# kursawe/OpticalFlow

Measured on AMD Instinct MI355X. Metric: frame-pairs/sec, higher is better.
Workload: dtype f64; 1 GPU; 1024x1024x256 synthetic translating texture (seed 1), speed_alpha=1, remodelling_alpha=1e4, rtol=1e-06, all 255 pairs solved to the stopping rule; frames_per_gpu=256, pairs_in_flight=255, levels=9, coarse_stencils=float8, vcycle_vectors=coarse_float32, w_cycle_level=1, w_cycle_visits=3, warm_start_stride=3, allgather=False, gather_chunks=1, converged=True

## Files before the change

include/vof.h:

```cpp
#ifndef VOF_H
#define VOF_H

#include <stddef.h>
#include <stdint.h>

#ifdef __cplusplus
extern "C" {
#endif

#define VOF_VERSION 202

typedef struct vof_ctx vof_ctx;

typedef struct vof_params {
    uint32_t struct_size;
    uint32_t abi_version;
    double speed_alpha;
    double remodelling_alpha;
    double delta_x;
    double delta_t;
    double initial_v_x;
    double initial_v_y;
    double initial_remodelling;
    double rtol;
    int32_t max_iterations;
    int32_t nu_pre;
    int32_t nu_post;
    int32_t reference_quirks;
    int32_t coarse_precision;
    int32_t vcycle_precision;
    int32_t nu_pre_coarse;
    int32_t nu_post_coarse;
    int32_t w_cycle_level;
    int32_t w_cycle_visits;
    int32_t krylov_method;
    int32_t gmres_restart;
    int32_t fallback_after;
    int32_t warm_start_stride;
    int32_t preconditioner;
    int32_t reserved0;
} vof_params;

typedef struct vof_pair_stats {
    int32_t iterations;
    int32_t converged;
    double relative_residual;
    double L1_functional;
    double speed_functional;
    double remodelling_functional;
    double batch_ms;
    int32_t batch_pairs;
    int32_t reserved;
} vof_pair_stats;

enum vof_kernel_id {
    VOF_K_RHS = 0, VOF_K_APPLY0, VOF_K_GS0, VOF_K_GS, VOF_K_RESIDUAL, VOF_K_RESTRICT, VOF_K_PROLONG,
    VOF_K_GALERKIN0, VOF_K_GALERKIN, VOF_K_COARSE_SETUP, VOF_K_COARSE_SOLVE, VOF_K_VECTOR, VOF_K_REDUCE,
    VOF_K_FINALIZE, VOF_K_FUNCTIONALS, VOF_K_COARSE_TAIL, VOF_K_COUNT
};

int vof_version(void);
size_t vof_params_size(void);
int vof_default_params(vof_params* p, size_t struct_size);


int vof_create(vof_ctx** out, int device_id, int n_i, int n_j, int max_pairs_in_flight, void* stream);
void vof_destroy(vof_ctx* ctx);
const char* vof_last_error(const vof_ctx* ctx);
size_t vof_workspace_bytes(const vof_ctx* ctx);
size_t vof_query_workspace(int n_i, int n_j, int max_pairs_in_flight);
size_t vof_query_workspace_for(int n_i, int n_j, int max_pairs_in_flight, int coarse_precision, int vcycle_precision);
int vof_device_memory(int device_id, size_t* free_bytes, size_t* total_bytes);
int vof_num_levels(const vof_ctx* ctx);

int vof_solve_stack_host(vof_ctx* ctx, const double* movie, int n_frames, const vof_params* p,
                         double* v_x, double* v_y, double* remodelling, double* speed,
                         vof_pair_stats* stats);
int vof_solve_stack_dev(vof_ctx* ctx, const double* movie, int n_frames, const vof_params* p,
                        double* v_x, double* v_y, double* remodelling, double* speed,
                        vof_pair_stats* stats);

int vof_blur_stack_dev(vof_ctx* ctx, const double* in_dev, double* out_dev, int n_frames, const double* weights, int radius);
int vof_blur_stack_host(vof_ctx* ctx, const double* in_host, double* out_host, int n_frames, const double* weights, int radius);

typedef struct vof_variation_stats {
    double speed_mean, speed_variance;
    double remodelling_mean, remodelling_variance;
    double L1_functional, speed_functional, remodelling_functional;
    double max_relative_residual;
    int32_t converged_last;
    int32_t converged_all;
    int32_t max_iterations_used;
    int32_t reserved;
} vof_variation_stats;

int vof_vary_regularisation_host(vof_ctx* ctx, const double* movie, int n_frames, const vof_params* base,
                                 const double* speed_alphas, int n_speed_alphas,
                                 const double* remodelling_alphas, int n_remodelling_alphas,
                                 const double* blur_weights, int blur_radius, vof_variation_stats* out);

int vof_field_moments_dev(vof_ctx* ctx, const double* field_dev, size_t n, double* mean, double* variance);

int vof_subsample_dev(vof_ctx* ctx, const double* field_dev, int n_fields, int box, int offset, double* out_dev);

int vof_texture_stack_dev(vof_ctx* ctx, double* out_dev, int n_frames, const double* mode_params, int n_modes,
                          const double* frame_offsets, double period, double scale);

int vof_set_fused_sweeps(vof_ctx* ctx, int on);

int vof_bench_sweeps_dev(vof_ctx* ctx, const double* movie, int n_pairs, const vof_params* p, int n_sweeps);

int vof_profile_enable(vof_ctx* ctx, int on);
int vof_profile_reset(vof_ctx* ctx);
int vof_profile_filter(vof_ctx* ctx, int kernel_id, int level);
int vof_profile_get(vof_ctx* ctx, int kernel_id, int level, int64_t* launches, double* total_ms);
int vof_profile_get_units(vof_ctx* ctx, int kernel_id, int level, int64_t* pair_launches);
int vof_profile_get_bytes(vof_ctx* ctx, int kernel_id, int level, double* algorithmic_bytes);
int vof_profile_get_moved(vof_ctx* ctx, int kernel_id, int level, double* moved_bytes);
const char* vof_kernel_name(int kernel_id);

int vof_debug_setup(vof_ctx* ctx, const double* movie_host, int n_pairs, const vof_params* p);
int vof_debug_check_canaries(vof_ctx* ctx);
int vof_debug_level_shape(vof_ctx* ctx, int level, int* n_i, int* n_j);
int vof_debug_rhs(vof_ctx* ctx, double* b_host);
int vof_debug_apply(vof_ctx* ctx, int level, const double* x_host, double* y_host);
int vof_debug_gs(vof_ctx* ctx, int level, double* x_host, const double* b_host, int colour);
int vof_debug_sweep(vof_ctx* ctx, int level, double* x_host, const double* b_host, int reverse, int from_zero);
int vof_debug_smooth(vof_ctx* ctx, int level, double* x_host, const double* b_host, int nu, int reverse, int from_zero);
int vof_debug_restrict(vof_ctx* ctx, int level, const double* fine_host, double* coarse_host);
int vof_debug_prolong_add(vof_ctx* ctx, int level, double* fine_host, const double* coarse_host);
int vof_debug_resrestrict_u(vof_ctx* ctx, int level, const double* x_new_host, const double* x_old_host, double* coarse_host);
int vof_debug_stencil(vof_ctx* ctx, int level, double* c_host);
int vof_debug_vcycle(vof_ctx* ctx, const double* r_host, double* e_host);
int vof_debug_coarse_solve(vof_ctx* ctx, const double* r_host, double* e_host);
int vof_debug_vcycle_apply(vof_ctx* ctx, const double* r_host, double* y_host, double* v_host, double* dots_host, int* fused);

#ifdef __cplusplus
}
#endif
#endif
```

opticalflow_amd/_native.py:

```python
from __future__ import annotations

import ctypes as C
import os

import numpy as np

HERE = os.path.dirname(os.path.abspath(__file__))
LIB_PATH = os.environ.get("VOF_LIB") or os.path.join(HERE, "csrc", "libvof.so")

K_NAMES = ["rhs", "apply0", "gs0", "gs", "residual", "restrict", "prolong", "galerkin0", "galerkin",
           "coarse_setup", "coarse_solve", "vector", "reduce", "finalize", "functionals", "coarse_tail"]


class VofParams(C.Structure):
    _fields_ = [("struct_size", C.c_uint32), ("abi_version", C.c_uint32),
                ("speed_alpha", C.c_double), ("remodelling_alpha", C.c_double), ("delta_x", C.c_double),
                ("delta_t", C.c_double), ("initial_v_x", C.c_double), ("initial_v_y", C.c_double),
                ("initial_remodelling", C.c_double), ("rtol", C.c_double), ("max_iterations", C.c_int32),
                ("nu_pre", C.c_int32), ("nu_post", C.c_int32), ("reference_quirks", C.c_int32),
                ("coarse_precision", C.c_int32), ("vcycle_precision", C.c_int32), ("nu_pre_coarse", C.c_int32), ("nu_post_coarse", C.c_int32),
                ("w_cycle_level", C.c_int32), ("w_cycle_visits", C.c_int32), ("krylov_method", C.c_int32),
                ("gmres_restart", C.c_int32), ("fallback_after", C.c_int32), ("warm_start_stride", C.c_int32),
                ("preconditioner", C.c_int32), ("reserved0", C.c_int32)]


class VofPairStats(C.Structure):
    _fields_ = [("iterations", C.c_int32), ("converged", C.c_int32), ("relative_residual", C.c_double),
                ("L1_functional", C.c_double), ("speed_functional", C.c_double),
                ("remodelling_functional", C.c_double), ("batch_ms", C.c_double), ("batch_pairs", C.c_int32),
                ("reserved", C.c_int32)]


STATS_DTYPE = np.dtype([("iterations", np.int32), ("converged", np.int32), ("relative_residual", np.float64),
                        ("L1_functional", np.float64), ("speed_functional", np.float64),
                        ("remodelling_functional", np.float64), ("batch_ms", np.float64), ("batch_pairs", np.int32),
                        ("reserved", np.int32)])
assert STATS_DTYPE.itemsize == C.sizeof(VofPairStats)

VARIATION_DTYPE = np.dtype([("speed_mean", np.float64), ("speed_variance", np.float64), ("remodelling_mean", np.float64),
                            ("remodelling_variance", np.float64), ("L1_functional", np.float64),
                            ("speed_functional", np.float64), ("remodelling_functional", np.float64),
                            ("max_relative_residual", np.float64), ("converged_last", np.int32),
                            ("converged_all", np.int32), ("max_iterations_used", np.int32), ("reserved", np.int32)])
assert VARIATION_DTYPE.itemsize == 80

_dp = C.POINTER(C.c_double)
_vp = C.c_void_p

SIGNATURES = {
    "vof_version": (C.c_int, []),
    "vof_params_size": (C.c_size_t, []),
    "vof_default_params": (C.c_int, [C.POINTER(VofParams), C.c_size_t]),
    "vof_create": (C.c_int, [C.POINTER(_vp), C.c_int, C.c_int, C.c_int, C.c_int, _vp]),
    "vof_destroy": (None, [_vp]),
    "vof_last_error": (C.c_char_p, [_vp]),
    "vof_workspace_bytes": (C.c_size_t, [_vp]),
    "vof_query_workspace": (C.c_size_t, [C.c_int, C.c_int, C.c_int]),
    "vof_query_workspace_for": (C.c_size_t, [C.c_int, C.c_int, C.c_int, C.c_int, C.c_int]),
    "vof_device_memory": (C.c_int, [C.c_int, C.POINTER(C.c_size_t), C.POINTER(C.c_size_t)]),
    "vof_num_levels": (C.c_int, [_vp]),
    "vof_solve_stack_host": (C.c_int, [_vp, _vp, C.c_int, C.POINTER(VofParams), _vp, _vp, _vp, _vp, _vp]),
    "vof_solve_stack_dev": (C.c_int, [_vp, _vp, C.c_int, C.POINTER(VofParams), _vp, _vp, _vp, _vp, _vp]),
    "vof_texture_stack_dev": (C.c_int, [_vp, _vp, C.c_int, _vp, C.c_int, _vp, C.c_double, C.c_double]),
    "vof_bench_sweeps_dev": (C.c_int, [_vp, _vp, C.c_int, C.POINTER(VofParams), C.c_int]),
    "vof_blur_stack_dev": (C.c_int, [_vp, _vp, _vp, C.c_int, _vp, C.c_int]),
    "vof_blur_stack_host": (C.c_int, [_vp, _vp, _vp, C.c_int, _vp, C.c_int]),
    "vof_vary_regularisation_host": (C.c_int, [_vp, _vp, C.c_int, C.POINTER(VofParams), _vp, C.c_int, _vp, C.c_int, _vp, C.c_int, _vp]),
    "vof_field_moments_dev": (C.c_int, [_vp, _vp, C.c_size_t, C.POINTER(C.c_double), C.POINTER(C.c_double)]),
    "vof_subsample_dev": (C.c_int, [_vp, _vp, C.c_int, C.c_int, C.c_int, _vp]),
    "vof_profile_enable": (C.c_int, [_vp, C.c_int]),
    "vof_profile_reset": (C.c_int, [_vp]),
    "vof_profile_filter": (C.c_int, [_vp, C.c_int, C.c_int]),
    "vof_profile_get": (C.c_int, [_vp, C.c_int, C.c_int, C.POINTER(C.c_int64), C.POINTER(C.c_double)]),
    "vof_profile_get_units": (C.c_int, [_vp, C.c_int, C.c_int, C.POINTER(C.c_int64)]),
    "vof_profile_get_bytes": (C.c_int, [_vp, C.c_int, C.c_int, C.POINTER(C.c_double)]),
    "vof_profile_get_moved": (C.c_int, [_vp, C.c_int, C.c_int, C.POINTER(C.c_double)]),
    "vof_kernel_name": (C.c_char_p, [C.c_int]),
    "vof_debug_setup": (C.c_int, [_vp, _vp, C.c_int, C.POINTER(VofParams)]),
    "vof_debug_check_canaries": (C.c_int, [_vp]),
    "vof_debug_level_shape": (C.c_int, [_vp, C.c_int, C.POINTER(C.c_int), C.POINTER(C.c_int)]),
    "vof_debug_rhs": (C.c_int, [_vp, _vp]),
    "vof_debug_apply": (C.c_int, [_vp, C.c_int, _vp, _vp]),
    "vof_debug_gs": (C.c_int, [_vp, C.c_int, _vp, _vp, C.c_int]),
    "vof_debug_sweep": (C.c_int, [_vp, C.c_int, _vp, _vp, C.c_int, C.c_int]),
    "vof_debug_smooth": (C.c_int, [_vp, C.c_int, _vp, _vp, C.c_int, C.c_int, C.c_int]),
    "vof_set_fused_sweeps": (C.c_int, [_vp, C.c_int]),
    "vof_debug_restrict": (C.c_int, [_vp, C.c_int, _vp, _vp]),
    "vof_debug_resrestrict_u": (C.c_int, [_vp, C.c_int, _vp, _vp, _vp]),
    "vof_debug_prolong_add": (C.c_int, [_vp, C.c_int, _vp, _vp]),
    "vof_debug_stencil": (C.c_int, [_vp, C.c_int, _vp]),
    "vof_debug_vcycle": (C.c_int, [_vp, _vp, _vp]),
    "vof_debug_coarse_solve": (C.c_int, [_vp, _vp, _vp]),
    "vof_debug_vcycle_apply": (C.c_int, [_vp, _vp, _vp, _vp, _vp, C.POINTER(C.c_int)]),
}

_lib = None


class VofError(RuntimeError):
    pass


def _share_hip_runtime_with_torch():
    import importlib.util
    import sys
    if "torch" in sys.modules:
        return
    try:
        spec = importlib.util.find_spec("torch")
    except (ImportError, ValueError):
        spec = None
    if spec is None or not spec.origin:
        return
    hip = os.path.join(os.path.dirname(spec.origin), "lib", "libamdhip64.so")
    if os.path.exists(hip):
        C.CDLL(hip, mode=C.RTLD_GLOBAL)


def load_library(path: str | None = None):
    global _lib
    if _lib is not None and path is None:
        return _lib
    p = path or LIB_PATH
    if not os.path.exists(p):
        raise VofError(f"native library {p} not found: build it with `python -m opticalflow_amd.build` "
                       "(hipcc, gfx950). There is no CPU fallback.")
    _share_hip_runtime_with_torch()
    lib = C.CDLL(p)
    for name, (res, args) in SIGNATURES.items():
        fn = getattr(lib, name)
        fn.restype = res
        fn.argtypes = args
    if path is None:
        _lib = lib
    return lib


def default_params(**overrides) -> VofParams:
    lib = load_library()
    p = VofParams()
    if lib.vof_default_params(C.byref(p), C.sizeof(p)) != 0:
        raise VofError(f"vof_params layout mismatch: binding {C.sizeof(p)} bytes, library {lib.vof_params_size()} bytes")
    for k, v in overrides.items():
        if not hasattr(p, k):
            raise TypeError(f"unknown solver parameter {k!r}")
        setattr(p, k, v)
    return p


def _ptr(a):
    if a is None:
        return None
    if isinstance(a, int):
        return C.c_void_p(a)
    if isinstance(a, np.ndarray):
        assert a.flags["C_CONTIGUOUS"]
        return C.c_void_p(a.ctypes.data)
    if hasattr(a, "data_ptr"):
        return C.c_void_p(a.data_ptr())
    raise TypeError(type(a))


class Solver:

    def __init__(self, n_i: int, n_j: int, max_pairs_in_flight: int, device: int = 0, stream: int | None = None):
        self.lib = load_library()
        self.n_i, self.n_j, self.max_pairs = int(n_i), int(n_j), int(max_pairs_in_flight)
        self.device = int(device)
        h = C.c_void_p()
        rc = self.lib.vof_create(C.byref(h), self.device, self.n_i, self.n_j, self.max_pairs,
                                 C.c_void_p(stream) if stream else None)
        if rc != 0:
            raise VofError("vof_create failed: " + self.lib.vof_last_error(None).decode())
        self.h = h

    def check_canaries(self):
        self._check(self.lib.vof_debug_check_canaries(self.h), "vof_debug_check_canaries")

    def close(self):
        if getattr(self, "h", None):
            h, self.h = self.h, None
            rc = self.lib.vof_debug_check_canaries(h)
            msg = self.lib.vof_last_error(h).decode() if rc != 0 else ""
            self.lib.vof_destroy(h)
            if rc != 0:
                raise VofError("device buffer guard regions damaged: " + msg)

    def __del__(self):
        try:
            self.close()
        except Exception:
            pass

    def __enter__(self):
        return self

    def __exit__(self, *a):
        self.close()

    def _check(self, rc, what):
        if rc != 0:
            raise VofError(f"{what} failed ({rc}): " + self.lib.vof_last_error(self.h).decode())

    @property
    def workspace_bytes(self):
        return int(self.lib.vof_workspace_bytes(self.h))

    @property
    def num_levels(self):
        return int(self.lib.vof_num_levels(self.h))

    def level_shape(self, level):
        a, b = C.c_int(), C.c_int()
        self._check(self.lib.vof_debug_level_shape(self.h, level, C.byref(a), C.byref(b)), "level_shape")
        return a.value, b.value

    def solve_host(self, movie: np.ndarray, params: VofParams, want_speed=True):
        movie = np.ascontiguousarray(movie, dtype=np.float64)
        T = movie.shape[0]
        assert movie.shape[1:] == (self.n_i, self.n_j)
        out = [np.empty((T - 1, self.n_i, self.n_j)) for _ in range(4 if want_speed else 3)]
        stats = np.zeros(T - 1, dtype=STATS_DTYPE)
        rc = self.lib.vof_solve_stack_host(self.h, _ptr(movie), T, C.byref(params), _ptr(out[0]), _ptr(out[1]),
                                           _ptr(out[2]), _ptr(out[3]) if want_speed else None, _ptr(stats))
        self._check(rc, "vof_solve_stack_host")
        return (*out, stats) if want_speed else (*out, None, stats)

    def solve_dev(self, movie, n_frames, params: VofParams, v_x, v_y, remodelling, speed=None, stats=True):
        st = np.zeros(n_frames - 1, dtype=STATS_DTYPE) if stats else None
        rc = self.lib.vof_solve_stack_dev(self.h, _ptr(movie), int(n_frames), C.byref(params), _ptr(v_x), _ptr(v_y),
                                          _ptr(remodelling), _ptr(speed), _ptr(st))
        self._check(rc, "vof_solve_stack_dev")
        return st

    def blur_host(self, movie: np.ndarray, weights: np.ndarray):
        movie = np.ascontiguousarray(movie, dtype=np.float64)
        weights = np.ascontiguousarray(weights, dtype=np.float64)
        assert movie.shape[1:] == (self.n_i, self.n_j) and weights.size % 2 == 1
        out = np.empty_like(movie)
        self._check(self.lib.vof_blur_stack_host(self.h, _ptr(movie), _ptr(out), movie.shape[0], _ptr(weights),
                                                 weights.size // 2), "vof_blur_stack_host")
        return out

    def blur_dev(self, movie, out, n_frames, weights: np.ndarray):
        weights = np.ascontiguousarray(weights, dtype=np.float64)
        self._check(self.lib.vof_blur_stack_dev(self.h, _ptr(movie), _ptr(out), int(n_frames), _ptr(weights),
                                                weights.size // 2), "vof_blur_stack_dev")

    def vary_regularisation_host(self, movie: np.ndarray, params: VofParams, speed_alphas, remodelling_alphas, weights=None):
        movie = np.ascontiguousarray(movie, dtype=np.float64)
        assert movie.shape[1:] == (self.n_i, self.n_j)
        sa = np.ascontiguousarray(speed_alphas, dtype=np.float64).ravel()
        ra = np.ascontiguousarray(remodelling_alphas, dtype=np.float64).ravel()
        out = np.zeros((sa.size, ra.size), dtype=VARIATION_DTYPE)
        w = None if weights is None else np.ascontiguousarray(weights, dtype=np.float64)
        rc = self.lib.vof_vary_regularisation_host(self.h, _ptr(movie), movie.shape[0], C.byref(params), _ptr(sa), sa.size,
                                                   _ptr(ra), ra.size, _ptr(w), 0 if w is None else w.size // 2, _ptr(out))
        self._check(rc, "vof_vary_regularisation_host")
        return out

    def field_moments_dev(self, field, n):
        m, v = C.c_double(), C.c_double()
        self._check(self.lib.vof_field_moments_dev(self.h, _ptr(field), int(n), C.byref(m), C.byref(v)), "vof_field_moments_dev")
        return m.value, v.value

    def subsample_dev(self, field, n_fields, box, offset, out):
        self._check(self.lib.vof_subsample_dev(self.h, _ptr(field), int(n_fields), int(box), int(offset), _ptr(out)),
                    "vof_subsample_dev")

    def texture_stack_dev(self, out, n_frames, mode_params, frame_offsets, period, scale):
        mp = np.ascontiguousarray(mode_params, dtype=np.float64)
        fo = np.ascontiguousarray(frame_offsets, dtype=np.float64)
        assert mp.ndim == 2 and mp.shape[0] == 4 and fo.shape == (n_frames, 2)
        self._check(self.lib.vof_texture_stack_dev(self.h, _ptr(out), int(n_frames), _ptr(mp), mp.shape[1], _ptr(fo),
                                                   float(period), float(scale)), "vof_texture_stack_dev")

    def bench_sweeps(self, movie, n_pairs, params, n_sweeps):
        self._check(self.lib.vof_bench_sweeps_dev(self.h, _ptr(movie), n_pairs, C.byref(params), n_sweeps),
                    "vof_bench_sweeps_dev")

    def profile_enable(self, on=True):
        self._check(self.lib.vof_profile_enable(self.h, int(bool(on))), "profile_enable")

    def profile_filter(self, kernel=-1, level=-1):
        kid = K_NAMES.index(kernel) if isinstance(kernel, str) else int(kernel)
        self._check(self.lib.vof_profile_filter(self.h, kid, level), "profile_filter")

    def profile_reset(self):
        self._check(self.lib.vof_profile_reset(self.h), "profile_reset")

    def profile_get(self, kernel: int | str, level: int = -1):
        kid = K_NAMES.index(kernel) if isinstance(kernel, str) else int(kernel)
        n, ms = C.c_int64(), C.c_double()
        self._check(self.lib.vof_profile_get(self.h, kid, level, C.byref(n), C.byref(ms)), "profile_get")
        return n.value, ms.value

    def profile_units(self, kernel: int | str, level: int = -1):
        kid = K_NAMES.index(kernel) if isinstance(kernel, str) else int(kernel)
        u = C.c_int64()
        self._check(self.lib.vof_profile_get_units(self.h, kid, level, C.byref(u)), "profile_get_units")
        return u.value

    def profile_bytes(self, kernel: int | str, level: int = -1):
        kid = K_NAMES.index(kernel) if isinstance(kernel, str) else int(kernel)
        u = C.c_double()
        self._check(self.lib.vof_profile_get_bytes(self.h, kid, level, C.byref(u)), "profile_get_bytes")
        return u.value

    def profile_moved(self, kernel: int | str, level: int = -1):
        kid = K_NAMES.index(kernel) if isinstance(kernel, str) else int(kernel)
        u = C.c_double()
        self._check(self.lib.vof_profile_get_moved(self.h, kid, level, C.byref(u)), "profile_get_moved")
        return u.value

    def profile_table(self):
        rows = []
        for kid, name in enumerate(K_NAMES):
            for lvl in range(16):
                n, ms = self.profile_get(kid, lvl)
                if n:
                    rows.append((name, lvl, n, ms))
        return rows

    def debug_setup(self, movie: np.ndarray, params: VofParams):
        movie = np.ascontiguousarray(movie, dtype=np.float64)
        self._dbg_pairs = movie.shape[0] - 1
        self._check(self.lib.vof_debug_setup(self.h, _ptr(movie), self._dbg_pairs, C.byref(params)), "debug_setup")

    def _vec(self, level):
        ni, nj = self.level_shape(level)
        return (self._dbg_pairs, 3, ni, nj)

    def debug_rhs(self):
        b = np.empty(self._vec(0))
        self._check(self.lib.vof_debug_rhs(self.h, _ptr(b)), "debug_rhs")
        return b

    def debug_apply(self, level, x):
        x = np.ascontiguousarray(x, dtype=np.float64).reshape(self._vec(level))
        y = np.empty_like(x)
        self._check(self.lib.vof_debug_apply(self.h, level, _ptr(x), _ptr(y)), "debug_apply")
        return y

    def debug_gs(self, level, x, b, colour):
        x = np.array(x, dtype=np.float64, copy=True).reshape(self._vec(level))
        b = np.ascontiguousarray(b, dtype=np.float64).reshape(self._vec(level))
        self._check(self.lib.vof_debug_gs(self.h, level, _ptr(x), _ptr(b), colour), "debug_gs")
        return x

    def debug_sweep(self, level, x, b, reverse=False, from_zero=False):
        x = np.array(x, dtype=np.float64, copy=True).reshape(self._vec(level))
        b = np.ascontiguousarray(b, dtype=np.float64).reshape(self._vec(level))
        self._check(self.lib.vof_debug_sweep(self.h, level, _ptr(x), _ptr(b), int(reverse), int(from_zero)), "debug_sweep")
        return x

    def debug_smooth(self, level, x, b, nu, reverse=False, from_zero=False):
        x = np.array(x, dtype=np.float64, copy=True).reshape(self._vec(level))
        b = np.ascontiguousarray(b, dtype=np.float64).reshape(self._vec(level))
        self._check(self.lib.vof_debug_smooth(self.h, level, _ptr(x), _ptr(b), int(nu), int(reverse), int(from_zero)), "debug_smooth")
        return x

    def set_fused_sweeps(self, on=True):
        self._check(self.lib.vof_set_fused_sweeps(self.h, int(bool(on))), "set_fused_sweeps")

    def debug_restrict(self, level, fine):
        fine = np.ascontiguousarray(fine, dtype=np.float64).reshape(self._vec(level))
        coarse = np.empty(self._vec(level + 1))
        self._check(self.lib.vof_debug_restrict(self.h, level, _ptr(fine), _ptr(coarse)), "debug_restrict")
        return coarse

    def debug_resrestrict_u(self, level, x_new, x_old=None):
        x_new = np.ascontiguousarray(x_new, dtype=np.float64).reshape(self._vec(level))
        if x_old is not None:
            x_old = np.ascontiguousarray(x_old, dtype=np.float64).reshape(self._vec(level))
        coarse = np.empty(self._vec(level + 1))
        self._check(self.lib.vof_debug_resrestrict_u(self.h, level, _ptr(x_new), _ptr(x_old) if x_old is not None else None,
                                                     _ptr(coarse)), "debug_resrestrict_u")
        return coarse

    def debug_prolong_add(self, level, fine, coarse):
        fine = np.array(fine, dtype=np.float64, copy=True).reshape(self._vec(level))
        coarse = np.ascontiguousarray(coarse, dtype=np.float64).reshape(self._vec(level + 1))
        self._check(self.lib.vof_debug_prolong_add(self.h, level, _ptr(fine), _ptr(coarse)), "debug_prolong_add")
        return fine

    def debug_stencil(self, level):
        ni, nj = self.level_shape(level)
        c = np.empty((self._dbg_pairs, 3, 3, 3, 3, ni, nj))
        self._check(self.lib.vof_debug_stencil(self.h, level, _ptr(c)), "debug_stencil")
        return c

    def debug_vcycle(self, r):
        r = np.ascontiguousarray(r, dtype=np.float64).reshape(self._vec(0))
        e = np.empty_like(r)
        self._check(self.lib.vof_debug_vcycle(self.h, _ptr(r), _ptr(e)), "debug_vcycle")
        return e

    def debug_vcycle_apply(self, r):
        r = np.ascontiguousarray(r, dtype=np.float64).reshape(self._vec(0))
        y, v = np.empty_like(r), np.empty_like(r)
        dots = np.zeros((r.shape[0], 2))
        fused = C.c_int(0)
        self._check(self.lib.vof_debug_vcycle_apply(self.h, _ptr(r), _ptr(y), _ptr(v), _ptr(dots), C.byref(fused)), "debug_vcycle_apply")
        return y, v, dots, bool(fused.value)

    def debug_coarse_solve(self, r):
        last = self.num_levels - 1
        r = np.ascontiguousarray(r, dtype=np.float64).reshape(self._vec(last))
        e = np.empty_like(r)
        self._check(self.lib.vof_debug_coarse_solve(self.h, _ptr(r), _ptr(e)), "debug_coarse_solve")
        return e


def query_workspace(n_i, n_j, pairs, coarse_precision=None, vcycle_precision=None):
    if coarse_precision is None and vcycle_precision is None:
        return int(load_library().vof_query_workspace(int(n_i), int(n_j), int(pairs)))
    return int(load_library().vof_query_workspace_for(int(n_i), int(n_j), int(pairs), 3 if coarse_precision is None else int(coarse_precision),
                                                      3 if vcycle_precision is None else int(vcycle_precision)))


def device_memory(device=0):
    f, t = C.c_size_t(), C.c_size_t()
    rc = load_library().vof_device_memory(int(device), C.byref(f), C.byref(t))
    if rc != 0:
        raise VofError("no usable HIP device %d (vof_device_memory rc=%d); this package has no CPU fallback" % (device, rc))
    return f.value, t.value
```

opticalflow_amd/csrc/vof.hip:

```cpp
#include "vof_device.hpp"
#include "vof_sweep0r.hpp"
#include "vof_sweep0p.hpp"
#include "vof_direct.hpp"
#include "../../include/vof.h"

#include <dlfcn.h>
#include <fcntl.h>
#include <unistd.h>

#include <algorithm>
#include <atomic>
#include <chrono>
#include <cmath>
#include <condition_variable>
#include <cstdio>
#include <cstdlib>
#include <cstring>
#include <mutex>
#include <string>
#include <thread>
#include <vector>

using namespace vof;

namespace {

constexpr int COARSEST_MAX = 5;
int coarsest_max() {
    if (const char* e = getenv("VOF_COARSEST_MAX")) { int v = atoi(e); if (v >= 3 && v <= 9) return v; }
    return COARSEST_MAX;
}
constexpr int MAX_PROF_RECS = 32768;
constexpr int MAX_LANES = 3;
constexpr int MAX_LANE_GROUPS = 2;
constexpr int AUTO_F64_AFTER = 8;

struct Level {
    int ni = 0, nj = 0;
    size_t npts = 0;
    void* C = nullptr;
    void* x = nullptr;
    void* b = nullptr;
    void* r = nullptr;
    void* x2 = nullptr;
};

struct ProfRec {
    hipEvent_t e0, e1;
    int kid, level, units;
    double bytes;
    double moved;
};

}

struct vof_ctx {
    int device = 0;
    hipStream_t stream = nullptr;
    bool own_stream = false;
    int Ni = 0, Nj = 0, B = 0;
    std::vector<Level> L;
    double *kx = nullptr, *kb = nullptr, *kr = nullptr, *krh = nullptr, *kp = nullptr, *kv = nullptr, *kt = nullptr;
    double* ky = nullptr;
    double* kz = nullptr;
    double* b32 = nullptr;
    bool vfloat = false;
    bool emit64 = false;
    bool vcoarse32 = false;
    bool l0_handoff = true;
    bool h32 = false;
    bool h32_bad = false;
    const PairParam* pp = nullptr;
    PairParam* pp_buf = nullptr;
    double* warm_x = nullptr;
    size_t warm_cap = 0;
    int* warm_src = nullptr;
    const int* guess_src = nullptr;
    double* partials = nullptr;
    int nblk = 0;
    PairScalars* sc = nullptr;
    int* active = nullptr;
    double* func3 = nullptr;
    double *W = nullptr, *invT = nullptr;
    int nd = 0;
    int* h_active = nullptr;
    PairScalars* h_sc = nullptr;
    double* h_func3 = nullptr;
    char* h_bounce = nullptr;
    hipEvent_t ev_batch[2] = {nullptr, nullptr};
    double* st_movie = nullptr;
    double* st_out[4] = {nullptr, nullptr, nullptr, nullptr};
    double* st_out2[4] = {nullptr, nullptr, nullptr, nullptr};
    hipStream_t copy_stream = nullptr;
    hipEvent_t ev_solved[2] = {nullptr, nullptr}, ev_copied[2] = {nullptr, nullptr}, ev_uploaded[2] = {nullptr, nullptr};
    double* st_movie2 = nullptr;
    double *blur_tmp = nullptr, *blur_w = nullptr, *blur_io = nullptr;
    double* tex_tab = nullptr;
    size_t tex_cap = 0;
    double* gm_V = nullptr;
    GmresState* gm_state = nullptr;
    double* gm_partials = nullptr;
    int* gm_cycle = nullptr;
    int gm_m = 0;
    long long gmres_pairs = 0;
    struct Alloc { void* raw; char* user; size_t bytes; const char* name; int line; };
    std::vector<Alloc> allocs;
    int c_bytes_per_point = 0;
    size_t bytes = 0;
    std::string err;
    const double* frames = nullptr;
    int npairs = 0;
    vof_params prm;
    int cfmt = 0;
    bool fused = true;
    bool geo_b_fine = false, geo_b_stored = true;
    bool fuse_prolong = true;
    bool fuse_restrict = true;
    bool sweep_st = true;
    bool skip_colour0 = true;
    bool fold_stored = false;
    bool fuse_resu = true;
    bool stream_apply = true;
    bool sweep0 = true;
    bool direct_on = false;
    int dir_cap = 0;
    double *dir_T = nullptr, *dir_tabs = nullptr, *dir_W = nullptr, *dir_r = nullptr, *dir_y = nullptr, *dir_x = nullptr, *dir_t = nullptr;
    int *dir_ipiv = nullptr, *dir_info = nullptr;
    double *dir_R = nullptr, *dir_C = nullptr, *dir_D = nullptr;
    int dir_ld = 0;
    void* roc_handle = nullptr;
    long long direct_pairs = 0;
    bool trail_enabled = true;
    bool trail_set = false, trail_done = false;
    S0Trail trail_req;
    bool fuse_rr = true;
    void* rr_out = nullptr;
    bool rr_f32 = false, rr_done = false;
    bool fuse_b = true;
    int bf_mode = 0;
    S0BSrc bf{nullptr, nullptr, nullptr, nullptr, nullptr, nullptr};
    int trail_nblk = 0;
    bool sweep0m = true;
    bool sweep0m_pairs = true;
    bool sweep0r = true;
    long sweep0r_min_blocks = 512;
    bool sweep0p = true;
    bool tail_enabled = true;
    int tail_first = -1;
    size_t tail_lds = 0;
    TailArgs tail;
    int tail_key[6] = {-9, -9, -9, -9, -9, -9};
    bool prof = false;
    int prof_kid = -1, prof_level = -1;
    std::vector<ProfRec> recs;
    std::vector<hipEvent_t> free_events;
    long long prof_dropped = 0;
    double prof_ms[VOF_K_COUNT][16];
    long long prof_n[VOF_K_COUNT][16];
    long long prof_units[VOF_K_COUNT][16];
    double prof_bytes[VOF_K_COUNT][16];
    double prof_moved[VOF_K_COUNT][16];
    int cur_units = 0;
    bool pq_hier = true, pq_smooth = true;
    int dbg_sync = 0;
    long long dbg_seq = 0;
    std::string dbg_fault;
    int dbg_fd = -1;
    bool dbg_canary = false;
    bool dbg_alloc_log = false;
    bool dbg_poison = false;
    size_t part_per_pair = 0;
    vof_ctx* lane_parent = nullptr;
    int lane_lo = 0, lane_slots = 0;
    int dir_ok = -1;
    hipStream_t lane_stream[MAX_LANES] = {};
    hipEvent_t lane_ev[MAX_LANES][2] = {};
    hipEvent_t ev_fork = nullptr;
    hipEvent_t group_ev[MAX_LANES * MAX_LANE_GROUPS] = {};
};

static std::string g_create_error;

namespace {

void dbg_sync_check(vof_ctx* c, const char* what, int level) {
    if (!c->dbg_sync) return;
    ++c->dbg_seq;
    char line[256];
    if (c->dbg_fd >= 0) {
        int n = snprintf(line, sizeof line, "in flight: scope #%lld '%s' level %d, %d pairs, grid %dx%d (%d levels)%-40s\n", c->dbg_seq, what, level,
                         c->cur_units, c->Ni, c->Nj, (int)c->L.size(), "");
        if (pwrite(c->dbg_fd, line, (size_t)n, 0) < 0) {  }
    }
    hipError_t e = hipStreamSynchronize(c->stream);
    hipError_t e2 = hipGetLastError();
    if (e == hipSuccess) e = e2;
    if (e != hipSuccess && c->dbg_fault.empty()) {
        snprintf(line, sizeof line, "VOF_DEBUG_SYNC: scope #%lld, kernel class '%s', level %d, %d pairs, image %dx%d: %s", c->dbg_seq, what, level,
                 c->cur_units, c->Ni, c->Nj, hipGetErrorString(e));
        c->dbg_fault = line;
        fprintf(stderr, "%s\n", line);
        fflush(stderr);
    }
}

struct Prof {
    vof_ctx* c;
    bool on;
    int dkid, dlevel;
    ProfRec rec;
    Prof(vof_ctx* c_, int kid, int level, double bytes_per_pair = 0.0, double moved_per_pair = -1.0) : c(c_), on(false), dkid(kid), dlevel(level) {
        if (!c->prof) return;
        if (c->prof_kid >= 0 && kid != c->prof_kid) return;
        if (c->prof_level >= 0 && level != c->prof_level) return;
        if ((int)c->recs.size() >= MAX_PROF_RECS) { c->prof_dropped++; return; }
        if (c->free_events.size() >= 2) {
            rec.e0 = c->free_events.back(); c->free_events.pop_back();
            rec.e1 = c->free_events.back(); c->free_events.pop_back();
        } else {
            if (hipEventCreate(&rec.e0) != hipSuccess || hipEventCreate(&rec.e1) != hipSuccess) return;
        }
        rec.kid = kid; rec.level = level < 0 ? 0 : (level > 15 ? 15 : level);
        rec.units = c->cur_units;
        rec.bytes = bytes_per_pair * c->cur_units;
        rec.moved = (moved_per_pair < 0.0 ? bytes_per_pair : moved_per_pair) * c->cur_units;
        on = true;
        hipEventRecord(rec.e0, c->stream);
    }
    ~Prof() {
        if (on) {
            hipEventRecord(rec.e1, c->stream);
            c->recs.push_back(rec);
        }
        if (c->dbg_sync) dbg_sync_check(c, vof_kernel_name(dkid), dlevel);
    }
};

void prof_collect(vof_ctx* c) {
    if (c->recs.empty()) return;
    hipStreamSynchronize(c->stream);
    for (auto& r : c->recs) {
        float ms = 0.f;
        if (hipEventElapsedTime(&ms, r.e0, r.e1) == hipSuccess) {
            c->prof_ms[r.kid][r.level] += ms;
            c->prof_n[r.kid][r.level] += 1;
            c->prof_units[r.kid][r.level] += r.units;
            c->prof_bytes[r.kid][r.level] += r.bytes;
            c->prof_moved[r.kid][r.level] += r.moved;
        }
        c->free_events.push_back(r.e0);
        c->free_events.push_back(r.e1);
    }
    c->recs.clear();
}

#define HIPCHK(call)                                                                               \
    do {                                                                                           \
        hipError_t e_ = (call);                                                                    \
        if (e_ != hipSuccess) {                                                                    \
            char buf_[512];                                                                        \
            snprintf(buf_, sizeof buf_, "%s failed: %s (%s:%d)", #call, hipGetErrorString(e_), __FILE__, __LINE__); \
            c->err = buf_;                                                                         \
            if (!c->dbg_fault.empty()) c->err += " [" + c->dbg_fault + "]";                        \
            return -2;                                                                             \
        }                                                                                          \
    } while (0)

constexpr size_t DBG_GUARD = 4096;
constexpr int DBG_GUARD_BYTE = 0xC5;

template <typename T>
int dev_alloc_named(vof_ctx* c, T** p, size_t n, const char* name, int line) {
    void* q = nullptr;
    size_t bytes = std::max<size_t>(n * sizeof(T), 256);
    if (c->dbg_canary) {
        HIPCHK(hipMalloc(&q, bytes + 2 * DBG_GUARD));
        HIPCHK(hipMemset(q, DBG_GUARD_BYTE, DBG_GUARD));
        HIPCHK(hipMemset((char*)q + DBG_GUARD + bytes, DBG_GUARD_BYTE, DBG_GUARD));
        c->allocs.push_back({q, (char*)q + DBG_GUARD, bytes, name, line});
        *p = (T*)((char*)q + DBG_GUARD);
    } else {
        HIPCHK(hipMalloc(&q, bytes));
        c->allocs.push_back({q, (char*)q, bytes, name, line});
        *p = (T*)q;
    }
    c->bytes += bytes;
    if (c->dbg_poison) HIPCHK(hipMemset(*p, 0xFF, bytes));
    if (c->dbg_alloc_log)
        fprintf(stderr, "vof alloc ctx=%p %s (vof.hip:%d) base=%p end=%p bytes=%zu\n", (void*)c, name, line, (void*)*p, (void*)((char*)*p + bytes), bytes);
    return 0;
}
#define dev_alloc(c, p, n) dev_alloc_named(c, p, n, #p, __LINE__)

int dev_free(vof_ctx* c, void* user) {
    if (!user) return 0;
    for (size_t i = 0; i < c->allocs.size(); ++i)
        if ((void*)c->allocs[i].user == user) {
            HIPCHK(hipFree(c->allocs[i].raw));
            c->bytes -= c->allocs[i].bytes;
            c->allocs.erase(c->allocs.begin() + (long)i);
            return 0;
        }
    c->err = "internal: dev_free of a pointer the context does not own";
    return -1;
}

constexpr int DEFAULT_COARSE_PRECISION = 3;
inline int vof_params_default_coarse_precision() { return DEFAULT_COARSE_PRECISION; }
inline int coef_bytes_per_point(int fmt) { return fmt == 3 ? 30 * 4 : (fmt == 2 ? 45 * 4 : (fmt == 1 ? 81 * 4 : 81 * 8)); }

int ensure_stencil_storage(vof_ctx* c, int fmt) {
    const int need = coef_bytes_per_point(fmt);
    if (need <= c->c_bytes_per_point || c->L.size() < 2) return 0;
    HIPCHK(hipStreamSynchronize(c->stream));
    for (size_t l = 1; l < c->L.size(); ++l) {
        Level& lv = c->L[l];
        if (int rc = dev_free(c, lv.C)) return rc;
        lv.C = nullptr;
    }
    for (size_t l = 1; l < c->L.size(); ++l) {
        Level& lv = c->L[l];
        uint32_t* C = nullptr;
        if (int rc = dev_alloc(c, &C, (size_t)c->B * (need / 4) * CLay(lv.ni, lv.nj).plane)) return rc;
        lv.C = C;
    }
    c->c_bytes_per_point = need;
    c->frames = nullptr;
    return 0;
}

int ensure_storage(vof_ctx* c) {
    if (int rc = ensure_stencil_storage(c, c->prm.coarse_precision)) return rc;
    if (c->vfloat && !c->b32)
        if (int rc = dev_alloc(c, &c->b32, (size_t)c->B * 3 * c->L[0].npts)) return rc;
    return 0;
}

int dbg_check_canaries(vof_ctx* c, std::string* report) {
    int bad = 0;
    std::vector<unsigned char> h(2 * DBG_GUARD);
    if (!c->dbg_canary) return 0;
    for (const auto& a : c->allocs) {
        if (hipMemcpy(h.data(), a.raw, DBG_GUARD, hipMemcpyDeviceToHost) != hipSuccess ||
            hipMemcpy(h.data() + DBG_GUARD, a.user + a.bytes, DBG_GUARD, hipMemcpyDeviceToHost) != hipSuccess) {
            if (report) *report += "guard pages unreadable; ";
            return -1;
        }
        long first_lo = -1, first_hi = -1;
        for (size_t i = 0; i < DBG_GUARD; ++i) if (h[DBG_GUARD - 1 - i] != DBG_GUARD_BYTE) { first_lo = (long)i + 1; break; }
        for (size_t i = 0; i < DBG_GUARD; ++i) if (h[DBG_GUARD + i] != DBG_GUARD_BYTE) { first_hi = (long)i; break; }
        if (first_lo >= 0 || first_hi >= 0) {
            ++bad;
            char line[256];
            snprintf(line, sizeof line, "buffer %s (vof.hip:%d, %zu bytes at %p): written %s%ld bytes %s; ", a.name, a.line, a.bytes, (void*)a.user,
                     first_hi >= 0 ? "" : "-", first_hi >= 0 ? first_hi : first_lo, first_hi >= 0 ? "past its end" : "before its start");
            if (report) *report += line;
        }
    }
    return bad;
}

inline dim3 grid2d(int ni, int nj, int z) { return dim3((nj + BX - 1) / BX, (ni + BY - 1) / BY, z); }
inline dim3 grid2d_colour(int ni, int nj, int colour, int z) {
    int cp = colour >> 1, cq = colour & 1;
    int mi = (ni - cp + 1) / 2, mj = (nj - cq + 1) / 2;
    return dim3(std::max(1, (mj + BX - 1) / BX), std::max(1, (mi + BY - 1) / BY), z);
}
const dim3 blk2d(BX, BY, 1);

inline size_t frame_stride(const vof_ctx* c) { return (size_t)c->Ni * c->Nj; }

#define VDISPATCH(c, ...)                                   \
    do {                                                    \
        if ((c)->vfloat) { using VT = float; __VA_ARGS__; } \
        else { using VT = double; __VA_ARGS__; }            \
    } while (0)

#define YDISPATCH(c, ...)                                                  \
    do {                                                                   \
        if ((c)->vfloat || (c)->h32) { using VT = float; __VA_ARGS__; }    \
        else { using VT = double; __VA_ARGS__; }                           \
    } while (0)

template <typename T> struct TypeTag { typedef T type; };
#define CDISPATCH(c, l, ...)                                                                        \
    do {                                                                                            \
        const int cf_ = ((l) > 0) ? (c)->cfmt : 0;                                                  \
        if (cf_ == 2) { using CT = CoefB16; using CW = uint32_t; __VA_ARGS__; }                     \
        else if (cf_ == 3) { using CT = CoefF8; using CW = uint32_t; __VA_ARGS__; }                 \
        else if (cf_ == 1) { using CT = float; using CW = float; __VA_ARGS__; }                     \
        else { using CT = double; using CW = double; __VA_ARGS__; }                                 \
    } while (0)
inline double coef_bytes(const vof_ctx* c, int l) { const int f = l > 0 ? c->cfmt : 0; return f == 3 ? 30.0 * 4 : (f == 2 ? 45.0 * 4 : (f == 1 ? 81.0 * 4 : 81.0 * 8)); }

void gs_colour(vof_ctx* c, int l, double* x, const double* b, int colour, int np, const int* active) {
    Level& lv = c->L[l];
    dim3 g = grid2d_colour(lv.ni, lv.nj, colour, np);
    if (l == 0 && c->L.size() > 1) {
        Prof p(c, VOF_K_GS0, 0, 20.0 * lv.npts);
        k_gs0<<<g, blk2d, 0, c->stream>>>(c->frames, frame_stride(c), c->Nj, lv.ni, lv.nj, c->prm.speed_alpha,
                                          c->prm.remodelling_alpha, c->prm.reference_quirks, x, b, colour, active, c->pp);
    } else {
        Prof p(c, VOF_K_GS, l, (coef_bytes(c, l) + 72.0) / 4.0 * lv.npts);
        CDISPATCH(c, l, (k_gs<CT><<<g, blk2d, 0, c->stream>>>((const CW*)lv.C, lv.ni, lv.nj, x, b, colour, active)));
    }
}

int pick_band_height(int rows, int nx, int units) {
    const long blocks128 = (long)nx * ((rows + 127) / 128) * std::max(1, units);
    const int cap = blocks128 < 768 ? 32 : (blocks128 < 1536 ? 64 : 128);
    const int nb = (rows + cap - 1) / cap;
    return std::max(2, (((rows + nb - 1) / nb + 1) / 2) * 2);
}

struct ApplyGrid { int TI, nblk; dim3 grid; };
ApplyGrid apply_grid(const vof_ctx* c, int np) {
    const Level& lv = c->L[0];
    int TI = pick_band_height(lv.ni, (lv.nj + AP_OUT - 1) / AP_OUT, c->cur_units);
    ApplyGrid g;
    g.TI = TI;
    g.grid = dim3((lv.nj + AP_OUT - 1) / AP_OUT, (lv.ni + TI - 1) / TI, np);
    g.nblk = g.grid.x * g.grid.y;
    return g;
}

template <typename XT, typename BT, typename YT>
void apply_fine_t(vof_ctx* c, const XT* x, const BT* b, YT* y, int mode, int np, const int* active,
                  const double* dotvec = nullptr, int want_yy = 0, YT* ycopy = nullptr) {
    Level& lv = c->L[0];
    const double bytes = (8.0 + 3.0 * sizeof(XT) + ((y ? 3.0 : 0.0) + (ycopy ? 3.0 : 0.0)) * sizeof(YT) + (mode ? 3.0 * sizeof(BT) : 0.0) +
                          (dotvec ? 24.0 : 0.0)) * lv.npts;
    Prof p(c, VOF_K_APPLY0, 0, bytes);
    if (c->stream_apply) {
        ApplyGrid ag = apply_grid(c, np);
        double* part = (dotvec || want_yy) ? c->partials : nullptr;
        if (mode)
            k_stream_apply0<1, XT, BT, YT><<<ag.grid, AP_THREADS, 0, c->stream>>>(
                c->frames, frame_stride(c), c->Nj, lv.ni, lv.nj, ag.TI, c->prm.speed_alpha, c->prm.remodelling_alpha,
                c->prm.reference_quirks, x, b, y, dotvec, want_yy, part, ag.nblk, active, c->pp, ycopy);
        else
            k_stream_apply0<0, XT, BT, YT><<<ag.grid, AP_THREADS, 0, c->stream>>>(
                c->frames, frame_stride(c), c->Nj, lv.ni, lv.nj, ag.TI, c->prm.speed_alpha, c->prm.remodelling_alpha,
                c->prm.reference_quirks, x, b, y, dotvec, want_yy, part, ag.nblk, active, c->pp, ycopy);
        return;
    }
    if (ycopy) { c->err = "internal: second output without the streaming operator kernel"; return; }
    dim3 g = grid2d(lv.ni, lv.nj, np);
    if (mode)
        k_apply0<1, XT, BT, YT><<<g, blk2d, 0, c->stream>>>(c->frames, frame_stride(c), c->Nj, lv.ni, lv.nj,
                                                            c->prm.speed_alpha, c->prm.remodelling_alpha,
                                                            c->prm.reference_quirks, x, b, y, active, c->pp);
    else
        k_apply0<0, XT, BT, YT><<<g, blk2d, 0, c->stream>>>(c->frames, frame_stride(c), c->Nj, lv.ni, lv.nj,
                                                            c->prm.speed_alpha, c->prm.remodelling_alpha,
                                                            c->prm.reference_quirks, x, b, y, active, c->pp);
}

template <typename VT>
void apply_stored_t(vof_ctx* c, int l, const VT* x, const VT* b, VT* y, int mode, int np, const int* active) {
    Level& lv = c->L[l];
    dim3 g = grid2d(lv.ni, lv.nj, np);
    Prof p(c, VOF_K_RESIDUAL, l, (coef_bytes(c, l) + (mode ? 9.0 : 6.0) * sizeof(VT)) * lv.npts);
    if (mode) CDISPATCH(c, l, (k_apply<CT, 1, VT><<<g, blk2d, 0, c->stream>>>((const CW*)lv.C, lv.ni, lv.nj, x, b, y, active)));
    else CDISPATCH(c, l, (k_apply<CT, 0, VT><<<g, blk2d, 0, c->stream>>>((const CW*)lv.C, lv.ni, lv.nj, x, b, y, active)));
}

template <typename VT>
void apply_level_t(vof_ctx* c, int l, const VT* x, const VT* b, VT* y, int mode, int np, const int* active) {
    if (l == 0 && c->L[0].C == nullptr) apply_fine_t<VT, VT, VT>(c, x, b, y, mode, np, active);
    else apply_stored_t<VT>(c, l, x, b, y, mode, np, active);
}

int krylov_apply(vof_ctx* c, const void* y, double* out, int np, const int* active, const double* dotvec = nullptr,
                 int want_yy = 0) {
    if (c->L[0].C) { apply_stored_t<double>(c, 0, (const double*)y, nullptr, out, 0, np, active); return 0; }
    const bool fuse = c->stream_apply && (dotvec || want_yy);
    if (c->vfloat || c->h32) apply_fine_t<float, double, double>(c, (const float*)y, nullptr, out, 0, np, active, fuse ? dotvec : nullptr, fuse ? want_yy : 0);
    else apply_fine_t<double, double, double>(c, (const double*)y, nullptr, out, 0, np, active, fuse ? dotvec : nullptr, fuse ? want_yy : 0);
    return fuse ? apply_grid(c, np).nblk : 0;
}
inline bool residual_copy_ok(const vof_ctx* c) { return c->stream_apply && !c->L[0].C; }
// ... 575 lines not shown
    if (c->gm_V) return 0;
    const size_t vec = (size_t)c->B * 3 * c->L[0].npts * sizeof(double);
    size_t free_b = 0, total_b = 0;
    HIPCHK(hipMemGetInfo(&free_b, &total_b));
    const size_t fixed = (size_t)c->B * (sizeof(GmresState) + (GM_NV + 1) * c->nblk * sizeof(double) + sizeof(int));
    const double budget = 0.5 * (double)free_b - (double)fixed;
    int fit = budget > 0 ? (int)std::min<double>(budget / (double)vec, 1e6) - 1 : 0;
    int m = std::min(want_m, fit);
    if (m < 4) { c->err = "not enough device memory for the GMRES fallback (lower max_pairs_in_flight)"; return -3; }
    if (int rc = dev_alloc(c, &c->gm_V, (size_t)(m + 1) * c->B * 3 * c->L[0].npts)) return rc;
    if (int rc = dev_alloc(c, &c->gm_state, (size_t)c->B)) return rc;
    if (int rc = dev_alloc(c, &c->gm_partials, (size_t)c->B * (GM_NV + 1) * c->nblk)) return rc;
    c->gm_m = m;
    return 0;
}

std::mutex g_lane_alloc;
int lane_gmres_attach(vof_ctx* c, bool basis, int want_m) {
    vof_ctx* p = c->lane_parent;
    std::lock_guard<std::mutex> lock(g_lane_alloc);
    int rc = 0;
    if (!p->gm_cycle) rc = dev_alloc(p, &p->gm_cycle, (size_t)p->B);
    if (!rc && basis && !p->gm_V) rc = gmres_buffers(p, want_m);
    if (rc) { c->err = p->err; p->err.clear(); return rc; }
    const size_t lo = (size_t)c->lane_lo;
    c->gm_cycle = p->gm_cycle + lo;
    if (p->gm_V) {
        c->gm_V = p->gm_V + lo * 3 * c->L[0].npts;
        c->gm_state = p->gm_state + lo;
        c->gm_partials = p->gm_partials + lo * (GM_NV + 1) * c->nblk;
        c->gm_m = p->gm_m;
    }
    return 0;
}

int gmres_phase(vof_ctx* c, int np, int* handed_over) {
    const vof_params& P = c->prm;
    hipStream_t s = c->stream;
    const size_t len = 3 * c->L[0].npts;
    const size_t vstride = (size_t)c->B * len;
    if (!c->gm_cycle) {
        if (c->lane_parent) { if (int rc = lane_gmres_attach(c, false, 0)) return rc; }
        else if (int rc = dev_alloc(c, &c->gm_cycle, (size_t)c->B)) return rc;
    }
    k_gm_begin<<<(np + 63) / 64, 64, 0, s>>>(c->sc, c->active, c->gm_cycle, np, P.max_iterations);
    dbg_sync_check(c, "gm_begin", 0);
    int nact = count_active(c, np);
    if (nact < 0) { c->err = "stream synchronize failed"; return -2; }
    if (nact == 0) return 0;
    *handed_over = nact;
    if (!c->gm_V) {
        const int want = P.gmres_restart > 0 ? P.gmres_restart : 100;
        int rc = c->lane_parent ? lane_gmres_attach(c, true, want) : gmres_buffers(c, want);
        if (rc == -3) { c->err.clear(); return 0; }
        if (rc) return rc;
    }
    c->gmres_pairs += nact;
    const int m = std::min(c->gm_m, P.gmres_restart > 0 ? P.gmres_restart : 100);
    c->vfloat = false;
    c->vcoarse32 = false;
    double* V = c->gm_V;
    double* w = c->kt;
    const dim3 rg = rgrid(c, np);
    const int coef_c = (int)(offsetof(GmresState, c) / sizeof(double)), coef_y = (int)(offsetof(GmresState, y) / sizeof(double));
    for (;;) {
        c->cur_units = nact;
        int nb = residual_d(c, c->kx, c->kb, V, np, c->gm_cycle, 1);
        if (!nb) { Prof p(c, VOF_K_REDUCE, 0); k_dot2<<<rg, RBLK, 0, s>>>(V, V, nullptr, nullptr, len, c->partials, c->gm_cycle); nb = c->nblk; }
        { Prof p(c, VOF_K_VECTOR, 0);
          k_gm_init<<<np, 64, 0, s>>>(c->gm_state, c->sc, c->partials, nb, c->active, c->gm_cycle, P.max_iterations); }
        nact = count_active(c, np);
        if (nact < 0) { c->err = "stream synchronize failed"; return -2; }
        if (nact == 0) break;
        c->cur_units = nact;
        { Prof p(c, VOF_K_VECTOR, 0, 16.0 * len); k_gm_scale<<<rg, RBLK, 0, s>>>(V, V, len, c->gm_state, c->active); }
        int jdone = 0;
        for (int j = 0; j < m; ++j) {
            const int* act = c->active;
            vcycle(c, &c->ky, V + (size_t)j * vstride, np, act);
            krylov_apply(c, c->ky, w, np, act);
            for (int pass = 0; pass < 2; ++pass) {
                for (int i0 = 0; i0 <= j; i0 += GM_NV) {
                    int cnt = std::min(GM_NV, j + 1 - i0);
                    Prof p(c, VOF_K_REDUCE, 0, 8.0 * len * (cnt + 1));
                    k_gm_multidot<<<rg, RBLK, 0, s>>>(V + (size_t)i0 * vstride, vstride, cnt, w, len, c->gm_partials, act);
                    k_gm_hcoef<<<np, 64, 0, s>>>(c->gm_state, c->gm_partials, c->nblk, i0, cnt, pass, act);
                }
                for (int i0 = 0; i0 <= j; i0 += GM_NV) {
                    int cnt = std::min(GM_NV, j + 1 - i0);
                    bool last = pass == 1 && i0 + GM_NV > j;
                    Prof p(c, VOF_K_VECTOR, 0, 8.0 * len * (cnt + 2));
                    k_gm_axpy<<<rg, RBLK, 0, s>>>(V + (size_t)i0 * vstride, vstride, i0, cnt, c->gm_state, coef_c, -1.0, w,
                                                  last ? V + (size_t)(j + 1) * vstride : w, len, act, 0,
                                                  last ? c->gm_partials : nullptr);
                }
            }
            { Prof p(c, VOF_K_VECTOR, 0, 16.0 * len);
              k_gm_givens<<<np, 64, 0, s>>>(c->gm_state, c->sc, c->gm_partials, c->nblk, j, c->active, P.max_iterations);
              k_gm_scale<<<rg, RBLK, 0, s>>>(V + (size_t)(j + 1) * vstride, V + (size_t)(j + 1) * vstride, len, c->gm_state, c->active); }
            jdone = j + 1;
            nact = count_active(c, np);
            if (nact < 0) { c->err = "stream synchronize failed"; return -2; }
            if (nact == 0) break;
            c->cur_units = nact;
        }
        { Prof p(c, VOF_K_VECTOR, 0); k_gm_solve_y<<<(np + 63) / 64, 64, 0, s>>>(c->gm_state, c->gm_cycle, np); }
        for (int i0 = 0; i0 < jdone; i0 += GM_NV) {
            int cnt = std::min(GM_NV, jdone - i0);
            Prof p(c, VOF_K_VECTOR, 0, 8.0 * len * (cnt + 2));
            k_gm_axpy<<<rg, RBLK, 0, s>>>(V + (size_t)i0 * vstride, vstride, i0, cnt, c->gm_state, coef_y, 1.0,
                                          i0 ? c->kp : nullptr, c->kp, len, c->gm_cycle, 1, nullptr);
        }
        vcycle(c, &c->ky, c->kp, np, c->gm_cycle);
        { Prof p(c, VOF_K_VECTOR, 0, 24.0 * len); k_gm_xpy<<<rg, RBLK, 0, s>>>(c->kx, c->ky, len, c->gm_cycle); }
        HIPCHK(hipGetLastError());
    }
    HIPCHK(hipGetLastError());
    return 0;
}

struct RocSolverApi {
    void* lib = nullptr;
    int (*create_handle)(void**) = nullptr;
    int (*destroy_handle)(void*) = nullptr;
    int (*set_stream)(void*, hipStream_t) = nullptr;
    int (*getrf)(void*, int, int, double*, int, long long, int*, long long, int*, int) = nullptr;
    int (*getri)(void*, int, double*, int, long long, int*, long long, int*, int) = nullptr;
    std::string err;
    bool resident() {
        if (lib) return true;
        const char* names[] = {"librocsolver.so.0", "librocsolver.so"};
        for (const char* n : names)
            if (void* h = dlopen(n, RTLD_NOLOAD | RTLD_LAZY)) { dlclose(h); return true; }
        return false;
    }
    bool load() {
        if (lib) return true;
        const char* names[] = {getenv("VOF_ROCSOLVER_LIB"), "librocsolver.so.0", "librocsolver.so", "/opt/rocm/lib/librocsolver.so.0"};
        for (const char* n : names) {
            if (!n || !*n) continue;
            lib = dlopen(n, RTLD_NOW | RTLD_GLOBAL);
            if (lib) break;
        }
        if (!lib) {
            const char* e = dlerror();
            err = std::string("cannot load rocSOLVER: ") + (e ? e : "not found");
            return false;
        }
        create_handle = (int (*)(void**))dlsym(lib, "rocblas_create_handle");
        destroy_handle = (int (*)(void*))dlsym(lib, "rocblas_destroy_handle");
        set_stream = (int (*)(void*, hipStream_t))dlsym(lib, "rocblas_set_stream");
        getrf = (int (*)(void*, int, int, double*, int, long long, int*, long long, int*, int))dlsym(lib, "rocsolver_dgetrf_strided_batched");
        getri = (int (*)(void*, int, double*, int, long long, int*, long long, int*, int))dlsym(lib, "rocsolver_dgetri_strided_batched");
        if (!create_handle || !destroy_handle || !set_stream || !getrf || !getri) {
            err = "rocSOLVER / rocBLAS symbols missing";
            dlclose(lib);
            lib = nullptr;
            return false;
        }
        return true;
    }
};
RocSolverApi g_roc;

constexpr int DIRECT_OWN_MAX = 192;
bool direct_uses_rocsolver(const vof_ctx*) {
    const char* e = getenv("VOF_DIRECT_LU");
    return e && e[0] == 'r';
}
bool direct_uses_blocked(const vof_ctx* c) {
    if (const char* e = getenv("VOF_DIRECT_LU")) return e[0] == 'b';
    return 3 * c->L[0].nj > DIRECT_OWN_MAX;
}
int direct_ld(const vof_ctx* c) {
    const int m = 3 * c->L[0].nj;
    return direct_uses_blocked(c) ? ((m + DNB - 1) / DNB) * DNB : m;
}

int direct_capacity(vof_ctx* c, int want);
bool direct_ok_for_fallback(vof_ctx* c) { return c->dir_ok >= 0 ? c->dir_ok != 0 : direct_capacity(c, 1) >= 1; }

size_t direct_bytes_per_pair(const vof_ctx* c) {
    const size_t ni = c->L[0].ni, nj = c->L[0].nj, m = 3 * nj, ld = (size_t)direct_ld(c);
    const size_t panels = direct_uses_blocked(c) ? (2 * ld + DNB) * DNB : 0;
    return (ni * ld * ld + ld * ld + panels + ni * nj * DIR_TAB + (3 * ni + 1) * m) * sizeof(double) + (m + 1) * sizeof(int);
}

int direct_capacity(vof_ctx* c, int want) {
    if (c->dir_cap > 0) return c->dir_cap;
    if (c->L.size() < 2 || c->L[0].C != nullptr) return 0;
    if ((size_t)3 * c->L[0].nj > 8192) return 0;
    size_t free_b = 0, total_b = 0;
    if (hipMemGetInfo(&free_b, &total_b) != hipSuccess) return 0;
    const double per = (double)direct_bytes_per_pair(c);
    int fit = (int)std::min<double>(0.6 * (double)free_b / per, 1e6);
    return std::max(0, std::min(fit, want));
}

int direct_alloc(vof_ctx* c, int pairs) {
    if (c->dir_cap >= pairs) return 0;
    if (c->dir_cap > 0) { c->err = "direct preconditioner buffers already allocated for a smaller batch"; return -3; }
    const bool trace = getenv("VOF_TRACE") != nullptr;
    const size_t ni = c->L[0].ni, nj = c->L[0].nj, m = 3 * nj, P = (size_t)pairs, ld = (size_t)direct_ld(c);
    c->dir_ld = (int)ld;
    if (direct_uses_rocsolver(c)) {
        if (trace) { fprintf(stderr, "[vof] direct_alloc: loading rocSOLVER\n"); fflush(stderr); }
        if (!g_roc.load()) { c->err = g_roc.err; return -3; }
        if (trace) { fprintf(stderr, "[vof] direct_alloc: rocSOLVER loaded, allocating for %d pairs\n", pairs); fflush(stderr); }
    }
    if (int rc = dev_alloc(c, &c->dir_T, P * ni * ld * ld)) return rc;
    if (int rc = dev_alloc(c, &c->dir_W, P * ld * ld)) return rc;
    if (direct_uses_blocked(c)) {
        if (int rc = dev_alloc(c, &c->dir_R, P * ld * DNB)) return rc;
        if (int rc = dev_alloc(c, &c->dir_C, P * ld * DNB)) return rc;
        if (int rc = dev_alloc(c, &c->dir_D, P * DNB * DNB)) return rc;
        const int lds = (DNB * DNB + DNB * DNB_LDB) * (int)sizeof(double);
        HIPCHK(hipFuncSetAttribute((const void*)k_dir_bgj_panel, hipFuncAttributeMaxDynamicSharedMemorySize, lds));
        HIPCHK(hipFuncSetAttribute((const void*)k_dir_bgj_update, hipFuncAttributeMaxDynamicSharedMemorySize, lds));
    }
    if (int rc = dev_alloc(c, &c->dir_tabs, P * ni * nj * DIR_TAB)) return rc;
    if (int rc = dev_alloc(c, &c->dir_r, P * ni * m)) return rc;
    if (int rc = dev_alloc(c, &c->dir_y, P * ni * m)) return rc;
    if (int rc = dev_alloc(c, &c->dir_x, P * ni * m)) return rc;
    if (int rc = dev_alloc(c, &c->dir_t, P * m)) return rc;
    if (int rc = dev_alloc(c, &c->dir_ipiv, P * m)) return rc;
    if (int rc = dev_alloc(c, &c->dir_info, P)) return rc;
    if (direct_uses_rocsolver(c) && !c->roc_handle) {
        if (trace) { fprintf(stderr, "[vof] direct_alloc: rocblas_create_handle\n"); fflush(stderr); }
        if (g_roc.create_handle(&c->roc_handle) != 0) { c->err = "rocblas_create_handle failed"; return -2; }
        if (g_roc.set_stream(c->roc_handle, c->stream) != 0) { c->err = "rocblas_set_stream failed"; return -2; }
        if (trace) { fprintf(stderr, "[vof] direct_alloc: handle ready\n"); fflush(stderr); }
    }
    c->dir_cap = pairs;
    return 0;
}

int direct_setup(vof_ctx* c, int np) {
    const vof_params& P = c->prm;
    const int ni = c->L[0].ni, nj = c->L[0].nj, m = 3 * nj, ld = c->dir_ld;
    const size_t sT = (size_t)ni * ld * ld, sW = (size_t)ld * ld, sTab = (size_t)ni * nj * DIR_TAB, rowTab = (size_t)nj * DIR_TAB;
    hipStream_t s = c->stream;
    Prof pr(c, VOF_K_COARSE_SETUP, 0);
    HIPCHK(hipMemsetAsync(c->dir_info, 0, (size_t)np * sizeof(int), s));
    k_dir_tables<<<dim3((nj + 255) / 256, ni, np), 256, 0, s>>>(c->frames, frame_stride(c), c->Nj, P.speed_alpha, P.remodelling_alpha,
                                                               P.reference_quirks, ni, nj, c->dir_tabs, c->pp);
    const dim3 gm((m + 255) / 256, m, np), gs((ld + 255) / 256, ld, np);
    const bool trace = getenv("VOF_TRACE") != nullptr;
    const bool blocked = direct_uses_blocked(c);
    const int nt = ld / DNB;
    const size_t bgj_lds = (size_t)(DNB * DNB + DNB * DNB_LDB) * sizeof(double);
    for (int p = 0; p < ni; ++p) {
        if (trace && (p < 2 || p == ni - 1)) { HIPCHK(hipStreamSynchronize(s)); fprintf(stderr, "[vof] direct_setup: row %d of %d (m = %d, %d pairs)\n", p, ni, m, np); fflush(stderr); }
        double* Tp = c->dir_T + (size_t)p * ld * ld;
        if (p > 0) k_dir_W<<<gm, 256, 0, s>>>(Tp - (size_t)ld * ld, sT, c->dir_tabs + (size_t)(p - 1) * rowTab, sTab, nj, c->dir_W, sW, ld);
        k_dir_schur<<<gs, 256, 0, s>>>(c->dir_tabs + (size_t)p * rowTab, sTab, nj, p > 0 ? c->dir_W : nullptr, sW, Tp, sT, ld);
        if (blocked) {
            for (int kt = 0; kt < nt; ++kt) {
                k_dir_bgj_panel<<<dim3(nt, 2, np), 256, bgj_lds, s>>>(Tp, sT, ld, kt, c->dir_R, c->dir_C, c->dir_D, c->dir_info);
                k_dir_bgj_update<<<dim3(nt, nt, np), 256, bgj_lds, s>>>(Tp, sT, ld, kt, c->dir_R, c->dir_C, c->dir_D);
            }
        } else if (direct_uses_rocsolver(c)) {
            if (g_roc.getrf(c->roc_handle, m, m, Tp, m, (long long)sT, c->dir_ipiv, (long long)m, c->dir_info, np) != 0 ||
                g_roc.getri(c->roc_handle, m, Tp, m, (long long)sT, c->dir_ipiv, (long long)m, c->dir_info, np) != 0) {
                c->err = "rocSOLVER getrf / getri failed";
                return -2;
            }
        } else {
            k_dir_invert<<<np, 1024, 2 * (size_t)m * sizeof(double), s>>>(Tp, sT, m, c->dir_ipiv, c->dir_info);
        }
    }
    HIPCHK(hipGetLastError());
    if (!direct_uses_rocsolver(c)) {
        std::vector<int> info((size_t)np);
        HIPCHK(hipMemcpyAsync(info.data(), c->dir_info, (size_t)np * sizeof(int), hipMemcpyDeviceToHost, s));
        HIPCHK(hipStreamSynchronize(s));
        for (int k = 0; k < np; ++k)
            if (info[k] != 0) { c->err = "direct preconditioner: a Schur block of pair " + std::to_string(k) + " of the batch is singular"; return -2; }
    }
    return 0;
}

template <typename VT>
int direct_apply_t(vof_ctx* c, VT* z, const VT* r, int np) {
    const int ni = c->L[0].ni, nj = c->L[0].nj, m = 3 * nj, ld = c->dir_ld;
    const size_t sT = (size_t)ni * ld * ld, sTab = (size_t)ni * nj * DIR_TAB, rowTab = (size_t)nj * DIR_TAB, sV = (size_t)ni * m;
    hipStream_t s = c->stream;
    Prof pr(c, VOF_K_COARSE_SOLVE, 0);
    const dim3 gp(64, np), gv((m + 255) / 256, np), gg((m + 63) / 64, np);
    k_dir_permute<const VT, true><<<gp, 256, 0, s>>>(r, c->dir_r, ni, nj);
    for (int p = 0; p < ni; ++p) {
        if (p > 0) k_dir_gemv<<<gg, 256, 0, s>>>(c->dir_T + (size_t)(p - 1) * ld * ld, sT, m, c->dir_y + (size_t)(p - 1) * m, sV, c->dir_t, (size_t)m, ld);
        k_dir_rowupdate<<<gv, 256, 0, s>>>(c->dir_tabs + (size_t)p * rowTab, sTab, nj, -1, c->dir_r + (size_t)p * m, sV,
                                          p > 0 ? c->dir_t : nullptr, (size_t)m, c->dir_y + (size_t)p * m, sV);
    }
    for (int p = ni - 1; p >= 0; --p) {
        k_dir_rowupdate<<<gv, 256, 0, s>>>(c->dir_tabs + (size_t)p * rowTab, sTab, nj, +1, c->dir_y + (size_t)p * m, sV,
                                          p + 1 < ni ? c->dir_x + (size_t)(p + 1) * m : nullptr, sV, c->dir_t, (size_t)m);
        k_dir_gemv<<<gg, 256, 0, s>>>(c->dir_T + (size_t)p * ld * ld, sT, m, c->dir_t, (size_t)m, c->dir_x + (size_t)p * m, sV, ld);
    }
    k_dir_permute<VT, false><<<gp, 256, 0, s>>>(z, c->dir_x, ni, nj);
    return 0;
}

int solve_batch(vof_ctx* c, const double* frames_dev, int np, double* vx, double* vy, double* gm, double* speed,
                vof_pair_stats* stats) {
    const vof_params& P = c->prm;
    struct MaxItGuard { vof_params& p; int saved; ~MaxItGuard() { p.max_iterations = saved; } } max_it_guard{c->prm, c->prm.max_iterations};
    constexpr int MG_ATTEMPT_CAP = 150;
    if (P.preconditioner == 2 && !c->direct_on && c->L.size() > 1 && P.max_iterations > MG_ATTEMPT_CAP && 3 * c->L[0].nj <= 3100 &&
        direct_ok_for_fallback(c))
        c->prm.max_iterations = MG_ATTEMPT_CAP;
    if (stats) HIPCHK(hipEventRecord(c->ev_batch[0], c->stream));
    c->vfloat = (P.vcycle_precision == 1 || P.vcycle_precision == 2) && c->fused && c->L.size() > 1 && !c->direct_on;
    c->vcoarse32 = P.vcycle_precision == 3 && !c->direct_on;
    c->h32 = c->h32_bad = false;
    if (c->direct_on) {
        if (np > c->dir_cap) { c->err = "batch larger than the direct preconditioner's buffers"; return -1; }
        c->frames = frames_dev;
        c->npairs = np;
        c->cur_units = np;
        if (int rc = direct_setup(c, np)) return rc;
        c->direct_pairs += np;
    } else if (int rc = setup_batch(c, frames_dev, np)) return rc;
    Level& f = c->L[0];
    const size_t len = 3 * f.npts;
    hipStream_t s = c->stream;
    double sx = P.delta_t / P.delta_x;
    const bool zero_guess = !c->guess_src && (P.initial_v_x == 0.0 && P.initial_v_y == 0.0 && P.initial_remodelling == 0.0);
    double* rh = c->krh;
    {
        Prof p(c, VOF_K_RHS, 0);
        k_rhs_norm<<<rgrid(c, np), RBLK, 0, s>>>(frames_dev, frame_stride(c), c->Nj, f.ni, f.nj, c->kb, zero_guess ? c->kr : nullptr,
                                                c->partials, c->pp);
    }
    { Prof p(c, VOF_K_VECTOR, 0); k_scalar<S_BNORM><<<np, 64, 0, s>>>(c->sc, c->partials, c->nblk, c->active, P.rtol, P.max_iterations); }
    int nb0 = c->nblk;
    if (zero_guess) {
        HIPCHK(hipMemsetAsync(c->kx, 0, (size_t)np * len * sizeof(double), s));
        rh = c->kb;
    } else {
        if (c->guess_src) {
            Prof p(c, VOF_K_VECTOR, 0, 16.0 * len);
            k_gather_guess<<<rgrid(c, np), RBLK, 0, s>>>(c->kx, c->warm_x, c->guess_src, len, f.npts, P.initial_v_x * sx, P.initial_v_y * sx,
                                                        P.initial_remodelling);
        } else {
            Prof p(c, VOF_K_VECTOR, 0); k_fill<<<dim3(c->nblk, np), 256, 0, s>>>(c->kx, f.npts, P.initial_v_x * sx, P.initial_v_y * sx, P.initial_remodelling);
        }
        const bool two = residual_copy_ok(c);
        nb0 = residual_d(c, c->kx, c->kb, c->kr, np, nullptr, 1, two ? c->krh : nullptr);
        if (!two) HIPCHK(hipMemcpyAsync(c->krh, c->kr, (size_t)np * len * sizeof(double), hipMemcpyDeviceToDevice, s));
    }
    if (!nb0) {
        Prof p(c, VOF_K_REDUCE, 0); k_dot2<<<rgrid(c, np), RBLK, 0, s>>>(c->kr, c->kr, nullptr, nullptr, len, c->partials, nullptr);
        nb0 = c->nblk;
    }
    { Prof p(c, VOF_K_VECTOR, 0); k_scalar<S_R0><<<np, 64, 0, s>>>(c->sc, c->partials, nb0, c->active, P.rtol, P.max_iterations); }

    const int bicg_limit = P.krylov_method == 1 ? 0 : (P.krylov_method == 2 ? std::min(P.max_iterations, P.fallback_after) : P.max_iterations);
    int it_total = 0;
    auto bicg_loop = [&](int limit) -> int {
    bool ran_on_r = false;
    for (int it = 0; it < limit; ++it, ++it_total) {
        HIPCHK(hipMemcpyAsync(c->h_active, c->active, np * sizeof(int), hipMemcpyDeviceToHost, s));
        HIPCHK(hipStreamSynchronize(s));
        int nact = 0;
        for (int k = 0; k < np; ++k) nact += c->h_active[k] != 0;
        if (nact == 0) break;
        if (it_total == AUTO_F64_AFTER) { if (P.vcycle_precision == 2) c->vfloat = false; c->vcoarse32 = false; }
        c->cur_units = nact;
        c->h32 = handoff32_ok(c);
        const int* act = c->active;
        void* vrhs_p = c->vfloat ? (void*)c->b32 : (void*)c->kp;
        void* vrhs_s = c->vfloat ? (void*)c->b32 : (void*)c->kr;
        const double vsz = (c->vfloat || c->h32) ? 4.0 : 8.0;
        const bool on_r = it == 0 && !c->vfloat;
        const bool fold_b = fold_b_usable(c);
        if (on_r) vrhs_p = (void*)c->kr;
        else if (fold_b && it > 0) {
            const double* p_old = (it == 1 && ran_on_r) ? rh : c->kp;
            c->bf = S0BSrc{c->kr, c->kv, p_old, c->kt, c->sc, nullptr};
            c->bf_mode = 2;
            std::swap(c->kp, c->kt);
            vrhs_p = (void*)c->kp;
        } else {
            Prof p(c, VOF_K_VECTOR, 0, 8.0 * len * (it == 0 ? 2 : 4) + (c->vfloat ? 4.0 * len : 0.0));
            const double* p_old = (it == 1 && ran_on_r) ? rh : c->kp;
            VDISPATCH(c, (k_update_p<VT><<<rgrid(c, np), RBLK, 0, s>>>(c->kp, p_old, c->kr, c->kv, len, c->sc, act,
                                                                     c->vfloat ? (VT*)c->b32 : (VT*)nullptr, it == 0 ? 1 : 0)));
        }
        if (it == 0) ran_on_r = on_r;
        c->trail_req = S0Trail{c->kv, rh, 0, c->partials};
        c->trail_set = true; c->trail_done = false;
        vcycle(c, &c->ky, vrhs_p, np, act);
        c->trail_set = false;
        if (c->bf_mode) { if (c->err.empty()) c->err = "folded vector update (p): not consumed by the cycle"; c->bf_mode = 0; return -1; }
        if (c->h32_bad) { c->h32_bad = c->h32 = false; return -1; }
        int nb1 = c->trail_done ? c->trail_nblk : krylov_apply(c, c->ky, c->kv, np, act, rh, 0);
        if (!nb1) { Prof p(c, VOF_K_REDUCE, 0, 16.0 * len); k_dot2<<<rgrid(c, np), RBLK, 0, s>>>(rh, c->kv, nullptr, nullptr, len, c->partials, act); nb1 = c->nblk; }
        { Prof p(c, VOF_K_VECTOR, 0); k_scalar<S_ALPHA><<<np, 64, 0, s>>>(c->sc, c->partials, nb1, c->active, P.rtol, P.max_iterations); }
        if (fold_b) {
            c->bf = S0BSrc{c->kr, c->kv, nullptr, c->kt, c->sc, c->partials};
            c->bf_mode = 1;
            std::swap(c->kr, c->kt);
            vrhs_s = (void*)c->kr;
        } else {
        { Prof p(c, VOF_K_VECTOR, 0, 8.0 * len * 3 + (c->vfloat ? 4.0 * len : 0.0));
          VDISPATCH(c, (k_update_s<VT><<<rgrid(c, np), RBLK, 0, s>>>(c->kr, c->kv, len, c->sc, c->partials, act, c->vfloat ? (VT*)c->b32 : (VT*)nullptr))); }
        { Prof p(c, VOF_K_VECTOR, 0); k_scalar<S_S><<<np, 64, 0, s>>>(c->sc, c->partials, c->nblk, c->active, P.rtol, P.max_iterations); }
        { Prof p(c, VOF_K_VECTOR, 0);
          YDISPATCH(c, (k_fix_half<VT><<<dim3(64, np), RBLK, 0, s>>>(c->kx, (const VT*)c->ky, len, c->sc)));
          k_clear_half<<<(np + 255) / 256, 256, 0, s>>>(c->sc, np); }
        }
        c->trail_req = S0Trail{c->kt, c->kr, 1, c->partials};
        c->trail_set = true; c->trail_done = false;
        vcycle(c, &c->kz, vrhs_s, np, act);
        c->trail_set = false;
        if (c->bf_mode) { if (c->err.empty()) c->err = "folded vector update (s): not consumed by the cycle"; c->bf_mode = 0; return -1; }
        if (c->h32_bad) { c->h32_bad = c->h32 = false; return -1; }
        int nb2 = c->trail_done ? c->trail_nblk : krylov_apply(c, c->kz, c->kt, np, act, c->kr, 1);
        if (!nb2) { Prof p(c, VOF_K_REDUCE, 0, 16.0 * len); k_dot2<<<rgrid(c, np), RBLK, 0, s>>>(c->kt, c->kr, c->kt, c->kt, len, c->partials, act); nb2 = c->nblk; }
        { Prof p(c, VOF_K_VECTOR, 0); k_scalar<S_OMEGA><<<np, 64, 0, s>>>(c->sc, c->partials, nb2, c->active, P.rtol, P.max_iterations); }
        { Prof p(c, VOF_K_VECTOR, 0, 8.0 * len * 6 + 2.0 * vsz * len);
          YDISPATCH(c, (k_update_xr<VT><<<rgrid(c, np), RBLK, 0, s>>>(c->kx, (const VT*)c->ky, (const VT*)c->kz, c->kr, c->kt, rh, len, c->sc, c->partials, act))); }
        { Prof p(c, VOF_K_VECTOR, 0); k_scalar<S_R><<<np, 64, 0, s>>>(c->sc, c->partials, c->nblk, c->active, P.rtol, P.max_iterations); }
    }
    c->h32 = false;
    return 0;
    };
    if (int rc = bicg_loop(bicg_limit)) return rc;
    auto independent_residual = [&](bool keep) -> int {
        c->cur_units = np;
        int nb3 = keep ? 0 : residual_d(c, c->kx, c->kb, nullptr, np, nullptr, 1);
        if (!nb3) nb3 = residual_d(c, c->kx, c->kb, c->kt, np, nullptr, 1);
        if (!nb3) { Prof p(c, VOF_K_REDUCE, 0); k_dot2<<<rgrid(c, np), RBLK, 0, s>>>(c->kt, c->kt, nullptr, nullptr, len, c->partials, nullptr); nb3 = c->nblk; }
        { Prof p(c, VOF_K_VECTOR, 0); k_scalar<S_FINAL><<<np, 64, 0, s>>>(c->sc, c->partials, nb3, c->active, P.rtol, P.max_iterations); }
        HIPCHK(hipGetLastError());
        return 0;
    };
    if (int rc = independent_residual(false)) return rc;
    if (bicg_limit > 0) {
        for (int round = 0; round < 3; ++round) {
            { Prof p(c, VOF_K_VECTOR, 0); k_bicg_restart<<<(np + 63) / 64, 64, 0, s>>>(c->sc, c->active, np, P.max_iterations); }
            int nact = count_active(c, np);
            if (nact < 0) { c->err = "stream synchronize failed"; return -2; }
            if (nact == 0) break;
            if (int rc = independent_residual(true)) return rc;
            c->cur_units = nact;
            rh = c->krh;
            { Prof p(c, VOF_K_VECTOR, 0, 8.0 * len * 3);
              k_restart_vectors<<<rgrid(c, np), RBLK, 0, s>>>(c->kr, rh, c->kt, len, c->active); }
            if (int rc = bicg_loop(std::min(bicg_limit, 8))) return rc;
            if (int rc = independent_residual(false)) return rc;
        }
    }
    if (P.krylov_method != 0) {
        int handed_over = 0;
        if (int rc = gmres_phase(c, np, &handed_over)) return rc;
        if (handed_over)
            if (int rc = independent_residual(false)) return rc;
    }
    { Prof p(c, VOF_K_FINALIZE, 0);
      k_finalize_functionals<<<rgrid(c, np), RBLK, 0, s>>>(frames_dev, frame_stride(c), f.ni, f.nj, P.speed_alpha, P.remodelling_alpha,
                                                           P.reference_quirks, c->kx, P.delta_x / P.delta_t, vx, vy, gm, speed,
                                                           c->partials, c->pp);
      k_sum3<<<np, 64, 0, s>>>(c->partials, c->nblk, c->func3); }
    HIPCHK(hipGetLastError());
    if (stats) {
        HIPCHK(hipMemcpyAsync(c->h_sc, c->sc, np * sizeof(PairScalars), hipMemcpyDeviceToHost, s));
        HIPCHK(hipMemcpyAsync(c->h_func3, c->func3, np * 3 * sizeof(double), hipMemcpyDeviceToHost, s));
        HIPCHK(hipEventRecord(c->ev_batch[1], s));
        HIPCHK(hipStreamSynchronize(s));
        float batch_ms = 0.f;
        HIPCHK(hipEventElapsedTime(&batch_ms, c->ev_batch[0], c->ev_batch[1]));
        for (int k = 0; k < np; ++k) {
            const PairScalars& q = c->h_sc[k];
            stats[k].iterations = q.iterations;
            stats[k].relative_residual = q.bnorm2 > 0 ? std::sqrt(q.rnorm2 / q.bnorm2) : 0.0;
            stats[k].converged = (q.rnorm2 <= q.tol2) ? 1 : 0;
            stats[k].L1_functional = c->h_func3[3 * k];
            stats[k].speed_functional = c->h_func3[3 * k + 1];
            stats[k].remodelling_functional = c->h_func3[3 * k + 2];
            stats[k].batch_ms = batch_ms;
            stats[k].batch_pairs = np;
            stats[k].reserved = 0;
        }
    }
    return 0;
}

int check_params(vof_ctx* c, const vof_params* p) {
    if (!p) { c->err = "params is NULL"; return -1; }
    if (p->struct_size != sizeof(vof_params) || p->abi_version != VOF_VERSION) {
        char buf[256];
        snprintf(buf, sizeof buf, "vof_params ABI mismatch: caller has struct_size %u / version %u, library has %zu / %d "
                 "(fill the struct with vof_default_params(p, sizeof *p) of the matching include/vof.h)",
                 p->struct_size, p->abi_version, sizeof(vof_params), VOF_VERSION);
        c->err = buf;
        return -4;
    }
    if (!(p->delta_x != 0.0) || !(p->delta_t != 0.0)) { c->err = "delta_x and delta_t must be non-zero"; return -1; }
    if (p->nu_pre < 0 || p->nu_post < 0 || p->nu_pre + p->nu_post == 0) { c->err = "nu_pre + nu_post must be > 0"; return -1; }
    if (p->nu_pre_coarse < 0 || p->nu_post_coarse < 0) { c->err = "nu_*_coarse must be >= 0"; return -1; }
    if (p->w_cycle_level < -1 || p->w_cycle_level > 15) { c->err = "w_cycle_level must be -1 or a level index"; return -1; }
    if (p->w_cycle_visits < 0 || p->w_cycle_visits > 8) { c->err = "w_cycle_visits must be in [0, 8]"; return -1; }
    if (!(p->rtol > 0.0)) { c->err = "rtol must be > 0"; return -1; }
    if (p->coarse_precision < 0 || p->coarse_precision > 3) { c->err = "coarse_precision must be 0, 1, 2 or 3"; return -1; }
    if (p->vcycle_precision < 0 || p->vcycle_precision > 3) { c->err = "vcycle_precision must be 0, 1, 2 or 3"; return -1; }
    if (p->krylov_method < 0 || p->krylov_method > 2) { c->err = "krylov_method must be 0, 1 or 2"; return -1; }
    if (p->gmres_restart < 0 || p->gmres_restart > GM_MAXM) { c->err = "gmres_restart must be in [0, 128]"; return -1; }
    if (p->fallback_after < 0) { c->err = "fallback_after must be >= 0"; return -1; }
    if (p->warm_start_stride < 0) { c->err = "warm_start_stride must be >= 0"; return -1; }
    if (p->preconditioner < 0 || p->preconditioner > 2) { c->err = "preconditioner must be 0, 1 or 2"; return -1; }
    c->prm = *p;
    c->vfloat = (p->vcycle_precision == 1 || p->vcycle_precision == 2) && c->fused && c->L.size() > 1;
    c->vcoarse32 = false;
    return ensure_storage(c);
}

}

extern "C" {

int vof_version(void) { return VOF_VERSION; }

size_t vof_params_size(void) { return sizeof(vof_params); }

int vof_default_params(vof_params* p, size_t struct_size) {
    if (!p || struct_size != sizeof(vof_params)) return -1;
    memset(p, 0, sizeof *p);
    p->struct_size = (uint32_t)sizeof(vof_params);
    p->abi_version = VOF_VERSION;
    p->speed_alpha = 1.0;
    p->remodelling_alpha = 1000.0;
    p->delta_x = 1.0;
    p->delta_t = 1.0;
    p->rtol = 1e-6;
    p->max_iterations = 1000;
    p->nu_pre = 2;
    p->nu_post = 2;
    p->nu_pre_coarse = 1;
    p->nu_post_coarse = 1;
    p->w_cycle_level = 1;
    p->w_cycle_visits = 3;
    p->reference_quirks = 1;
    p->coarse_precision = 3;
    p->vcycle_precision = 3;
    p->krylov_method = 2;
    p->gmres_restart = 100;
    p->warm_start_stride = 3;
    p->fallback_after = 25;
    p->preconditioner = 2;
    return 0;
}

const char* vof_last_error(const vof_ctx* ctx) { return ctx ? ctx->err.c_str() : g_create_error.c_str(); }
size_t vof_workspace_bytes(const vof_ctx* ctx) { return ctx ? ctx->bytes : 0; }
int vof_num_levels(const vof_ctx* ctx) { return ctx ? (int)ctx->L.size() : 0; }

size_t vof_query_workspace(int n_i, int n_j, int B) { return vof_query_workspace_for(n_i, n_j, B, DEFAULT_COARSE_PRECISION, 3); }

size_t vof_query_workspace_for(int n_i, int n_j, int B, int coarse_precision, int vcycle_precision) {
    if (n_i < 4 || n_j < 4 || B < 1 || coarse_precision < 0 || coarse_precision > 3) return 0;
    size_t ni = n_i - 2, nj = n_j - 2, total = 0, b = (size_t)B;
    std::vector<std::pair<size_t, size_t>> lv{{ni, nj}};
    while (std::max(lv.back().first, lv.back().second) > (size_t)coarsest_max())
        lv.push_back({(lv.back().first + 1) / 2, (lv.back().second + 1) / 2});
    size_t words = 0;
    total += (9 + ((vcycle_precision == 1 || vcycle_precision == 2) && lv.size() > 1 ? 1 : 0)) * b * 3 * ni * nj;
    for (size_t l = 0; l < lv.size(); ++l) {
        size_t npts = lv[l].first * lv[l].second;
        if (l + 1 < lv.size()) total += (l > 0 ? 2 : 1) * b * 3 * npts;
        if (l > 0) total += 2 * b * 3 * npts;
        const size_t plane = CLay((int)lv[l].first, (int)lv[l].second).plane;
        if (lv.size() == 1) total += b * 81 * plane;
        else if (l > 0) words += b * (size_t)(coef_bytes_per_point(coarse_precision) / 4) * plane;
    }
    size_t nd = 3 * lv.back().first * lv.back().second;
    total += b * nd * 2 * nd + b * nd * nd;
    return total * sizeof(double) + words * 4 + (size_t)B * 3 * 256 * sizeof(double) + 4096;
}

int vof_device_memory(int device_id, size_t* free_bytes, size_t* total_bytes) {
    size_t f = 0, t = 0;
    if (hipSetDevice(device_id) != hipSuccess) return -1;
    if (hipMemGetInfo(&f, &t) != hipSuccess) return -2;
    if (free_bytes) *free_bytes = f;
    if (total_bytes) *total_bytes = t;
    return 0;
}

const char* vof_kernel_name(int k) {
    static const char* names[VOF_K_COUNT] = {"rhs", "apply0", "gs0", "gs", "residual", "restrict", "prolong",
                                             "galerkin0", "galerkin", "coarse_setup", "coarse_solve", "vector",
                                             "reduce", "finalize", "functionals", "coarse_tail"};
    return (k >= 0 && k < VOF_K_COUNT) ? names[k] : "?";
}

void vof_destroy(vof_ctx* c) {
    if (!c) return;
    hipSetDevice(c->device);
    if (c->stream) {
        const hipError_t e = hipStreamSynchronize(c->stream);
        if (e != hipSuccess && (c->dbg_sync || c->dbg_canary))
            fprintf(stderr, "vof_destroy: the context's stream ends with an error: %s\n", hipGetErrorString(e));
    }
    if (c->dbg_canary) {
        std::string rep;
        if (dbg_check_canaries(c, &rep) != 0) { fprintf(stderr, "vof_destroy: VOF_DEBUG_CANARY: %s\n", rep.c_str()); fflush(stderr); }
    }
    if (c->dbg_fd >= 0) close(c->dbg_fd);
    prof_collect(c);
    for (auto e : c->free_events) hipEventDestroy(e);
    for (const auto& a : c->allocs) hipFree(a.raw);
    if (c->h_active) hipHostFree(c->h_active);
    if (c->h_sc) hipHostFree(c->h_sc);
    if (c->h_func3) hipHostFree(c->h_func3);
    if (c->h_bounce) hipHostFree(c->h_bounce);
    for (int i = 0; i < 2; ++i) if (c->ev_batch[i]) hipEventDestroy(c->ev_batch[i]);
    for (int i = 0; i < 2; ++i) {
        if (c->ev_solved[i]) hipEventDestroy(c->ev_solved[i]);
        if (c->ev_copied[i]) hipEventDestroy(c->ev_copied[i]);
        if (c->ev_uploaded[i]) hipEventDestroy(c->ev_uploaded[i]);
    }
    if (c->copy_stream) hipStreamDestroy(c->copy_stream);
    for (int i = 0; i < MAX_LANES; ++i) {
        if (c->lane_stream[i]) hipStreamDestroy(c->lane_stream[i]);
        for (int j = 0; j < 2; ++j) if (c->lane_ev[i][j]) hipEventDestroy(c->lane_ev[i][j]);
    }
    if (c->ev_fork) hipEventDestroy(c->ev_fork);
    for (hipEvent_t e : c->group_ev) if (e) hipEventDestroy(e);
    if (c->own_stream && c->stream) hipStreamDestroy(c->stream);
    delete c;
}

static int create_impl(vof_ctx* c, int device_id, int n_i, int n_j, int B, void* stream) {
    if (n_i < 4 || n_j < 4) { c->err = "image must be at least 4x4 (the mirror boundary rows need N >= 4)"; return -1; }
    if (B < 1) { c->err = "max_pairs_in_flight must be >= 1"; return -1; }
    int ndev = 0;
    HIPCHK(hipGetDeviceCount(&ndev));
    if (device_id < 0 || device_id >= ndev) { c->err = "no such HIP device"; return -1; }
    HIPCHK(hipSetDevice(device_id));
    c->device = device_id;
    c->Ni = n_i; c->Nj = n_j; c->B = B;
    if (stream) { c->stream = (hipStream_t)stream; c->own_stream = false; }
    else { HIPCHK(hipStreamCreate(&c->stream)); c->own_stream = true; }
    memset(c->prof_ms, 0, sizeof c->prof_ms);
    memset(c->prof_n, 0, sizeof c->prof_n);
    memset(c->prof_units, 0, sizeof c->prof_units);
    memset(c->prof_bytes, 0, sizeof c->prof_bytes);
    memset(c->prof_moved, 0, sizeof c->prof_moved);
    vof_default_params(&c->prm, sizeof c->prm);
    if (const char* e = getenv("VOF_DEBUG_SYNC")) c->dbg_sync = atoi(e);
    if (const char* e = getenv("VOF_DEBUG_CANARY")) c->dbg_canary = e[0] != '0';
    if (const char* e = getenv("VOF_DEBUG_ALLOC_LOG")) c->dbg_alloc_log = e[0] != '0';
    if (const char* e = getenv("VOF_DEBUG_POISON")) c->dbg_poison = e[0] != '0';
    if (c->dbg_sync)
        if (const char* e = getenv("VOF_DEBUG_SYNC_FILE")) c->dbg_fd = open(e, O_WRONLY | O_CREAT, 0644);
    if (const char* e = getenv("VOF_PRECOND_QUIRKS")) { c->pq_hier = e[0] != '0'; c->pq_smooth = e[0] && e[1] != '0'; }
    if (!c->pq_smooth) c->trail_enabled = false;
    if (const char* e = getenv("VOF_SWEEP_GEO")) {
        c->geo_b_fine = e[0] == 'B';
        c->geo_b_stored = e[0] && e[1] == 'B';
    }
    if (const char* e = getenv("VOF_STREAM_APPLY")) c->stream_apply = e[0] != '0';
    if (const char* e = getenv("VOF_FUSE_RESTRICT")) c->fuse_restrict = e[0] != '0';
    if (const char* e = getenv("VOF_FUSE_PROLONG")) c->fuse_prolong = e[0] != '0';
    if (const char* e = getenv("VOF_FUSE_RESU")) c->fuse_resu = e[0] != '0';
    if (const char* e = getenv("VOF_SWEEP_ST")) c->sweep_st = e[0] != '0';
    if (const char* e = getenv("VOF_FOLD_STORED")) c->fold_stored = e[0] != '0';
    if (const char* e = getenv("VOF_SKIP_COLOUR0")) c->skip_colour0 = e[0] != '0';
    if (const char* e = getenv("VOF_COARSE_TAIL")) c->tail_enabled = e[0] != '0';
    if (const char* e = getenv("VOF_SWEEP0")) c->sweep0 = e[0] != '0';
    if (const char* e = getenv("VOF_FUSE_APPLY")) c->trail_enabled = e[0] != '0';
    if (const char* e = getenv("VOF_SWEEP0R")) c->sweep0r = e[0] != '0';
    if (const char* e = getenv("VOF_L0_HANDOFF")) c->l0_handoff = e[0] != '0';
    if (const char* e = getenv("VOF_SWEEP0P")) c->sweep0p = e[0] != '0';
    if (const char* e = getenv("VOF_SWEEP0R_MIN_BLOCKS")) c->sweep0r_min_blocks = atol(e);
    if (const char* e = getenv("VOF_FUSE_B")) c->fuse_b = e[0] != '0';
    if (const char* e = getenv("VOF_FUSE_RR")) c->fuse_rr = e[0] != '0';
    if (const char* e = getenv("VOF_SWEEP0M")) { c->sweep0m = e[0] != '0'; c->sweep0m_pairs = e[0] != '0' && e[0] != '1'; }
    Level l0; l0.ni = n_i - 2; l0.nj = n_j - 2; l0.npts = (size_t)l0.ni * l0.nj;
    c->L.push_back(l0);
    while (std::max(c->L.back().ni, c->L.back().nj) > coarsest_max()) {
        Level k; k.ni = (c->L.back().ni + 1) / 2; k.nj = (c->L.back().nj + 1) / 2; k.npts = (size_t)k.ni * k.nj;
        c->L.push_back(k);
    }
    int nl = (int)c->L.size();
    if (nl > 16) { c->err = "too many levels"; return -1; }
    size_t len0 = 3 * l0.npts;
    for (double** v : {&c->kx, &c->kb, &c->kr, &c->krh, &c->kp, &c->kv, &c->kt, &c->ky, &c->kz})
        if (int rc = dev_alloc(c, v, (size_t)B * len0)) return rc;
    for (int l = 0; l < nl; ++l) {
        Level& lv = c->L[l];
        auto valloc = [&](void** q) { double* t = nullptr; int rc = dev_alloc(c, &t, (size_t)B * 3 * lv.npts); *q = t; return rc; };
        if (l + 1 < nl && (l > 0 || !(c->stream_apply && c->fuse_restrict))) if (int rc = valloc(&lv.r)) return rc;
        if (l + 1 < nl) if (int rc = valloc(&lv.x2)) return rc;
        if (l > 0) {
            if (int rc = valloc(&lv.x)) return rc;
            if (int rc = valloc(&lv.b)) return rc;
        }
        if (nl == 1) {
            double* C = nullptr;
            if (int rc = dev_alloc(c, &C, (size_t)B * 81 * CLay(lv.ni, lv.nj).plane)) return rc;
            lv.C = C;
        }
    }
    if (int rc = ensure_stencil_storage(c, vof_params_default_coarse_precision())) return rc;
    c->nd = 3 * (int)c->L.back().npts;
    {
        int first = -1;
        for (int l = 1; l < nl; ++l) {
            const CLay lay(c->L[l].ni, c->L[l].nj);
            if (c->L[l].npts <= (size_t)TAIL_MAX_PTS && lay.sub <= (size_t)TAIL_MAX_SUB) { first = l; break; }
        }
        if (first >= 0) first = std::max(first, nl - TAIL_MAX_LEVELS);
        if (first >= 1 && first < nl - 1) {
            memset(&c->tail, 0, sizeof c->tail);
            int off = 0;
            for (int l = first; l < nl; ++l) {
                TailLevel& t = c->tail.L[l - first];
                const CLay lay(c->L[l].ni, c->L[l].nj);
                t.ni = c->L[l].ni; t.nj = c->L[l].nj; t.hj = lay.hj; t.sub = (int)lay.sub; t.plane = lay.plane;
                t.xo = off; off += 3 * (t.ni + 2) * (t.nj + 2);
                t.bo = off; off += 3 * t.ni * t.nj;
            }
            c->tail.ro = off; off += 3 * (int)c->L[first].npts;
            c->tail.nl = nl - first;
            c->tail.nd = c->nd;
            c->tail.n_ops = 0;
            c->tail_lds = (size_t)off * sizeof(double);
            if (c->tail_lds <= (size_t)150 * 1024) {
                c->tail_first = first;
                const int lds = (int)c->tail_lds;
                HIPCHK(hipFuncSetAttribute((const void*)k_tail_cycle<CoefB16, double>, hipFuncAttributeMaxDynamicSharedMemorySize, lds));
                HIPCHK(hipFuncSetAttribute((const void*)k_tail_cycle<CoefB16, float>, hipFuncAttributeMaxDynamicSharedMemorySize, lds));
                HIPCHK(hipFuncSetAttribute((const void*)k_tail_cycle<CoefF8, double>, hipFuncAttributeMaxDynamicSharedMemorySize, lds));
                HIPCHK(hipFuncSetAttribute((const void*)k_tail_cycle<CoefF8, float>, hipFuncAttributeMaxDynamicSharedMemorySize, lds));
                HIPCHK(hipFuncSetAttribute((const void*)k_tail_cycle<float, double>, hipFuncAttributeMaxDynamicSharedMemorySize, lds));
                HIPCHK(hipFuncSetAttribute((const void*)k_tail_cycle<float, float>, hipFuncAttributeMaxDynamicSharedMemorySize, lds));
                HIPCHK(hipFuncSetAttribute((const void*)k_tail_cycle<double, double>, hipFuncAttributeMaxDynamicSharedMemorySize, lds));
                HIPCHK(hipFuncSetAttribute((const void*)k_tail_cycle<double, float>, hipFuncAttributeMaxDynamicSharedMemorySize, lds));
            }
        }
    }
    if (int rc = dev_alloc(c, &c->W, (size_t)B * c->nd * 2 * c->nd)) return rc;
    if (int rc = dev_alloc(c, &c->invT, (size_t)B * c->nd * c->nd)) return rc;
    {
        const int lds = 18 * s0_row_bytes(8) + 9 * (S0_W / 2 + 2) * 8;
        HIPCHK(hipFuncSetAttribute((const void*)k_sweep0m<2, true, false, 1>, hipFuncAttributeMaxDynamicSharedMemorySize, lds));
        HIPCHK(hipFuncSetAttribute((const void*)k_sweep0m<2, false, false, 1>, hipFuncAttributeMaxDynamicSharedMemorySize, lds));
        HIPCHK(hipFuncSetAttribute((const void*)k_sweep0m<1, true, false, 1>, hipFuncAttributeMaxDynamicSharedMemorySize, lds));
        HIPCHK(hipFuncSetAttribute((const void*)k_sweep0m<1, false, false, 1>, hipFuncAttributeMaxDynamicSharedMemorySize, lds));
    }
    c->nblk = (int)std::min<size_t>(256, std::max<size_t>(1, (len0 + 4 * RBLK - 1) / (4 * RBLK)));
    {
        int nblk_apply = ((l0.nj + AP_OUT - 1) / AP_OUT) * ((l0.ni + 31) / 32 + 1);
        nblk_apply = std::max(nblk_apply, ((l0.nj + 99) / 100) * ((l0.ni + 1 + 31) / 32 + 1));
        c->part_per_pair = (size_t)3 * std::max(c->nblk, nblk_apply);
        if (int rc = dev_alloc(c, &c->partials, (size_t)B * c->part_per_pair)) return rc;
    }
    if (int rc = dev_alloc(c, &c->sc, (size_t)B)) return rc;
    if (int rc = dev_alloc(c, &c->active, (size_t)B)) return rc;
    if (int rc = dev_alloc(c, &c->func3, (size_t)B * 3)) return rc;
    HIPCHK(hipHostMalloc((void**)&c->h_active, B * sizeof(int)));
    HIPCHK(hipHostMalloc((void**)&c->h_sc, B * sizeof(PairScalars)));
    HIPCHK(hipHostMalloc((void**)&c->h_func3, B * 3 * sizeof(double)));
    for (int i = 0; i < 2; ++i) HIPCHK(hipEventCreate(&c->ev_batch[i]));
    return 0;
}

int vof_create(vof_ctx** out, int device_id, int n_i, int n_j, int max_pairs_in_flight, void* stream) {
    if (!out) { g_create_error = "out is NULL"; return -1; }
    *out = nullptr;
    vof_ctx* c = new (std::nothrow) vof_ctx();
    if (!c) { g_create_error = "out of host memory"; return -1; }
    int rc = create_impl(c, device_id, n_i, n_j, max_pairs_in_flight, stream);
    if (rc) {
        g_create_error = c->err;
        vof_destroy(c);
        return rc;
    }
    *out = c;
    return 0;
}

}

namespace {

double lanes_min_pixels() {
    double mpix = 16.0;
    if (const char* e = getenv("VOF_LANES_MIN_MPIX")) { const double v = atof(e); if (v >= 0.0) mpix = v; }
    return mpix * 1e6;
}

int lanes_for(const vof_ctx* c, int pairs_per_phase) {
    if (c->prof || c->dbg_sync) return 1;
    int n = 3;
    if (const char* e = getenv("VOF_LANES")) { const int v = atoi(e); if (v >= 1 && v <= MAX_LANES) n = v; }
    const double minpix = lanes_min_pixels();
    n = std::min(n, c->B);
    while (n > 1 && (pairs_per_phase < n || (double)pairs_per_phase / n * c->Ni * c->Nj < minpix)) --n;
    return n;
}

struct LaneGroup { int lo, hi, lane; };

int lane_groups_wanted() {
    int g = 1;
    if (const char* e = getenv("VOF_LANE_GROUPS")) { const int v = atoi(e); if (v >= 1 && v <= MAX_LANE_GROUPS) g = v; }
    return g;
}

std::vector<LaneGroup> plan_groups(const vof_ctx* c, int n1, int L, int G) {
    const int min_pairs = std::max(1, (int)std::ceil(lanes_min_pixels() / ((double)c->Ni * c->Nj)));
    std::vector<int> share((size_t)L), head((size_t)L);
    for (int i = 0; i < L; ++i) {
        share[i] = (int)((long)n1 * (i + 1) / L - (long)n1 * i / L);
        if (G < 2 || share[i] < 2 * min_pairs) G = 1;
    }
    std::vector<LaneGroup> g;
    int at = 0;
    if (G == 2) {
        for (int i = 0; i < L; ++i)
            head[i] = std::min(std::max((int)std::lround((double)share[i] * (L - i) / (L + 1)), min_pairs), share[i] - min_pairs);
        for (int i = 0; i < L; ++i) { g.push_back({at, at + share[i] - head[i], i}); at += share[i] - head[i]; }
        for (int i = 0; i < L; ++i) { g.push_back({at, at + head[i], i}); at += head[i]; }
    } else {
        for (int i = 0; i < L; ++i) { g.push_back({at, at + share[i], i}); at += share[i]; }
    }
    return g;
}

struct GroupSync {
    std::mutex m;
    std::condition_variable cv;
    std::vector<char> usable;
    std::vector<int> state;
};

inline int batch_slots(const vof_ctx* c) { return c->lane_parent ? c->lane_slots : c->B; }

int make_lane(vof_ctx* c, int i, int n, vof_ctx* L) {
    if (!c->lane_stream[i]) {
        HIPCHK(hipStreamCreate(&c->lane_stream[i]));
        for (int j = 0; j < 2; ++j) HIPCHK(hipEventCreate(&c->lane_ev[i][j]));
    }
    *L = *c;
    const size_t lo = (size_t)c->B * i / n;
    L->lane_parent = c;
    L->lane_lo = (int)lo;
    L->lane_slots = (int)((size_t)c->B * (i + 1) / n - lo);
    for (int j = 0; j < MAX_LANES; ++j) { L->lane_stream[j] = nullptr; L->lane_ev[j][0] = L->lane_ev[j][1] = nullptr; }
    L->ev_fork = nullptr;
    L->stream = c->lane_stream[i];
    L->own_stream = false;
    L->ev_batch[0] = c->lane_ev[i][0];
    L->ev_batch[1] = c->lane_ev[i][1];
    L->allocs.clear();
    L->recs.clear();
    L->free_events.clear();
    L->prof = false;
    L->err.clear();
    L->h_bounce = nullptr;
    L->pp = nullptr;
    L->guess_src = nullptr;
    L->gmres_pairs = 0;
    L->dir_ok = direct_ok_for_fallback(c) ? 1 : 0;
    const size_t len0 = 3 * c->L[0].npts;
    for (double** v : {&L->kx, &L->kb, &L->kr, &L->krh, &L->kp, &L->kv, &L->kt, &L->ky, &L->kz, &L->b32, &L->gm_V})
        if (*v) *v += lo * len0;
    const int nl = (int)c->L.size();
    for (int l = 0; l < nl; ++l) {
        Level& lv = L->L[l];
        const size_t vb = 3 * lv.npts * sizeof(double);
        const size_t cb = (size_t)(nl == 1 ? 81 * 8 : c->c_bytes_per_point) * CLay(lv.ni, lv.nj).plane;
        for (void** q : {&lv.x, &lv.b, &lv.r, &lv.x2}) if (*q) *q = (char*)*q + lo * vb;
        if (lv.C) lv.C = (char*)lv.C + lo * cb;
    }
    L->W += lo * c->nd * 2 * c->nd;
    L->invT += lo * c->nd * c->nd;
    L->partials += lo * c->part_per_pair;
    L->sc += lo; L->h_sc += lo;
    L->active += lo; L->h_active += lo;
    L->func3 += 3 * lo; L->h_func3 += 3 * lo;
    if (L->pp_buf) L->pp_buf += lo;
    if (L->warm_src) L->warm_src += lo;
    if (L->gm_cycle) L->gm_cycle += lo;
    if (L->gm_state) L->gm_state += lo;
    if (L->gm_partials) L->gm_partials += lo * (GM_NV + 1) * c->nblk;
    return 0;
}

constexpr int LANES_NO_THREAD = -100;
template <typename F>
int run_lanes(vof_ctx* c, int n, F&& fn, bool concurrent_only = false) {
    std::vector<vof_ctx> lanes((size_t)n);
    for (int i = 0; i < n; ++i)
        if (int rc = make_lane(c, i, n, &lanes[i])) return rc;
    if (!c->ev_fork) HIPCHK(hipEventCreateWithFlags(&c->ev_fork, hipEventDisableTiming));
    HIPCHK(hipEventRecord(c->ev_fork, c->stream));
    for (int i = 0; i < n; ++i) HIPCHK(hipStreamWaitEvent(lanes[i].stream, c->ev_fork, 0));
    std::vector<int> rc((size_t)n, 0);
    std::vector<std::thread> th;
    auto body = [&](int i) {
        vof_ctx* L = &lanes[i];
        if (hipSetDevice(c->device) != hipSuccess) { L->err = "hipSetDevice failed"; rc[i] = -2; return; }
        rc[i] = fn(L, i);
        const hipError_t e = hipStreamSynchronize(L->stream);
        if (!rc[i] && e != hipSuccess) { L->err = std::string("stream synchronize failed: ") + hipGetErrorString(e); rc[i] = -2; }
    };
    try {
        for (int i = n - 1; i >= 0; --i) th.emplace_back(body, i);
    } catch (...) {
        if (th.empty() && concurrent_only) return LANES_NO_THREAD;
        for (int i = n - 1 - (int)th.size(); i >= 0; --i) body(i);
    }
    for (auto& t : th) t.join();
    for (int i = 0; i < n; ++i) c->gmres_pairs += lanes[i].gmres_pairs;
    for (int i = 0; i < n; ++i)
        if (rc[i]) { c->err = "lane " + std::to_string(i) + ": " + lanes[i].err; return rc[i]; }
    return 0;
}

}

extern "C" {

static int two_phase_part(vof_ctx* c, const double* movie, const std::vector<int>& list, size_t a, size_t b, bool phase2, int stride,
                          GroupSync& sync, double* v_x, double* v_y, double* remodelling, double* speed, vof_pair_stats* stats) {
    const vof_params prm = c->prm;
    const size_t len = 3 * c->L[0].npts;
    const int cap = batch_slots(c);
    const int n1 = (int)sync.usable.size();
    std::vector<PairParam> hp((size_t)cap);
    std::vector<int> hsrc((size_t)cap);
    std::vector<vof_pair_stats> st((size_t)cap);
    for (size_t o = a; o < b; o += (size_t)cap) {
        const int np = (int)std::min<size_t>((size_t)cap, b - o);
        {
            std::lock_guard<std::mutex> lk(sync.m);
            for (int i = 0; i < np; ++i) {
                const int k = list[o + i];
                hp[i] = PairParam{prm.speed_alpha, prm.remodelling_alpha, k, k};
                const int src = std::min((k + stride / 2) / stride, n1 - 1);
                hsrc[i] = phase2 && sync.usable[src] ? src : -1;
            }
        }
        HIPCHK(hipStreamSynchronize(c->stream));
        HIPCHK(hipMemcpyAsync(c->pp_buf, hp.data(), (size_t)np * sizeof(PairParam), hipMemcpyHostToDevice, c->stream));
        if (phase2) HIPCHK(hipMemcpyAsync(c->warm_src, hsrc.data(), (size_t)np * sizeof(int), hipMemcpyHostToDevice, c->stream));
        c->pp = c->pp_buf;
        c->guess_src = phase2 ? c->warm_src : nullptr;
        int rc = solve_batch(c, movie, np, v_x, v_y, remodelling, speed, st.data());
        c->pp = nullptr;
        c->guess_src = nullptr;
        if (rc) return rc;
        if (!phase2) {
            HIPCHK(hipMemcpyAsync(c->warm_x + o * len, c->kx, (size_t)np * len * sizeof(double), hipMemcpyDeviceToDevice, c->stream));
            std::lock_guard<std::mutex> lk(sync.m);
            for (int i = 0; i < np; ++i) sync.usable[o + i] = st[i].converged && std::isfinite(st[i].relative_residual);
        }
        if (stats)
            for (int i = 0; i < np; ++i) stats[list[o + i]] = st[i];
    }
    return 0;
}

static int two_phase_lane(vof_ctx* c, int lane, const std::vector<LaneGroup>& groups, hipEvent_t* ev, GroupSync& sync, const double* movie,
                          const std::vector<int>& first, const std::vector<int>& rest, int stride, double* v_x, double* v_y,
                          double* remodelling, double* speed, vof_pair_stats* stats) {
    const int ng = (int)groups.size();
    auto publish = [&](int g, bool ok) {
        {
            std::lock_guard<std::mutex> lk(sync.m);
            if (sync.state[g]) return;
            if (!ok) for (int o = groups[g].lo; o < groups[g].hi; ++o) sync.usable[o] = 0;
            sync.state[g] = ok ? 1 : -1;
        }
        sync.cv.notify_all();
    };
    auto run_group = [&](int g) -> int {
        const LaneGroup& G = groups[g];
        if (int rc = two_phase_part(c, movie, first, (size_t)G.lo, (size_t)G.hi, false, stride, sync, v_x, v_y, remodelling, speed, stats)) return rc;
        HIPCHK(hipEventRecord(ev[g], c->stream));
        publish(g, true);
        if (g + 1 < ng) {
            int state;
            {
                std::unique_lock<std::mutex> lk(sync.m);
                if (!sync.cv.wait_for(lk, std::chrono::seconds(60), [&] { return sync.state[g + 1] != 0; })) {
                    c->err = "timed out waiting for the phase-1 solutions of the next pair group";
                    return -2;
                }
                state = sync.state[g + 1];
            }
            if (state > 0) HIPCHK(hipStreamWaitEvent(c->stream, ev[g + 1], 0));
        }
        const size_t ra = (size_t)(std::lower_bound(rest.begin(), rest.end(), G.lo * stride) - rest.begin());
        const size_t rb = g + 1 < ng ? (size_t)(std::lower_bound(rest.begin(), rest.end(), G.hi * stride) - rest.begin()) : rest.size();
        return two_phase_part(c, movie, rest, ra, rb, true, stride, sync, v_x, v_y, remodelling, speed, stats);
    };
    int rc = 0;
    for (int g = ng - 1; g >= 0 && !rc; --g)
        if (groups[g].lane == lane) rc = run_group(g);
    for (int g = 0; g < ng; ++g)
        if (groups[g].lane == lane) publish(g, false);
    return rc;
}

static int solve_stack_two_phase(vof_ctx* c, const double* movie, int P, double* v_x, double* v_y, double* remodelling,
                                 double* speed, vof_pair_stats* stats, int stride, int lanes) {
    const size_t len = 3 * c->L[0].npts;
    const int B = c->B;
    std::vector<int> first, rest;
    for (int k = 0; k < P; ++k) (k % stride == 0 ? first : rest).push_back(k);
    const int n1 = (int)first.size();
    if (!c->pp_buf) { if (int rc = dev_alloc(c, &c->pp_buf, (size_t)B)) return rc; }
    if (!c->warm_src) { if (int rc = dev_alloc(c, &c->warm_src, (size_t)B)) return rc; }
    if (c->warm_cap < (size_t)n1 * len) {
        if (int rc = dev_free(c, c->warm_x)) return rc;
        c->warm_x = nullptr; c->warm_cap = 0;
        if (int rc = dev_alloc(c, &c->warm_x, (size_t)n1 * len)) return rc;
        c->warm_cap = (size_t)n1 * len;
    }
    GroupSync sync;
    sync.usable.assign((size_t)n1, 0);
    int rc = LANES_NO_THREAD;
    if (lanes > 1) {
        const std::vector<LaneGroup> groups = plan_groups(c, n1, lanes, lane_groups_wanted());
        sync.state.assign(groups.size(), 0);
        for (size_t g = 0; g < groups.size(); ++g)
            if (!c->group_ev[g]) HIPCHK(hipEventCreateWithFlags(&c->group_ev[g], hipEventDisableTiming));
        rc = run_lanes(c, lanes, [&](vof_ctx* L, int i) {
            return two_phase_lane(L, i, groups, c->group_ev, sync, movie, first, rest, stride, v_x, v_y, remodelling, speed, stats);
        }, true);
    }
    if (rc == LANES_NO_THREAD) {
        for (int phase = 0; phase < 2; ++phase) {
            const std::vector<int>& list = phase ? rest : first;
            if ((rc = two_phase_part(c, movie, list, 0, list.size(), phase == 1, stride, sync, v_x, v_y, remodelling, speed, stats))) return rc;
        }
    }
    if (rc) return rc;
    HIPCHK(hipStreamSynchronize(c->stream));
    return 0;
}

static int direct_solve_list(vof_ctx* c, const double* frames, const std::vector<PairParam>& items, double* v_x, double* v_y,
                             double* remodelling, double* speed, vof_pair_stats* stats) {
    if (items.empty()) return 0;
    const int cap = direct_capacity(c, std::min<int>(c->B, (int)items.size()));
    if (cap < 1) { c->err = "the direct preconditioner does not fit into the free device memory (3 n_j x 3 n_j doubles per image row and pair)"; return -3; }
    if (int rc = direct_alloc(c, cap)) return rc;
    if (!c->pp_buf) { if (int rc = dev_alloc(c, &c->pp_buf, (size_t)c->B)) return rc; }
    std::vector<vof_pair_stats> st((size_t)c->dir_cap);
    for (size_t o = 0; o < items.size(); o += (size_t)c->dir_cap) {
        const int np = (int)std::min<size_t>((size_t)c->dir_cap, items.size() - o);
        HIPCHK(hipStreamSynchronize(c->stream));
        HIPCHK(hipMemcpyAsync(c->pp_buf, items.data() + o, (size_t)np * sizeof(PairParam), hipMemcpyHostToDevice, c->stream));
        c->pp = c->pp_buf;
        c->direct_on = true;
        int rc = solve_batch(c, frames, np, v_x, v_y, remodelling, speed, st.data());
        c->direct_on = false;
        c->pp = nullptr;
        if (rc) return rc;
        if (stats)
            for (int i = 0; i < np; ++i) stats[o + i] = st[i];
    }
    return 0;
}

static int solve_range_dev(vof_ctx* c, const double* frames, int P, double* v_x, double* v_y, double* remodelling,
                           double* speed, vof_pair_stats* stats, bool allow_lanes) {
    const vof_params prm = c->prm;
    const int stride = prm.warm_start_stride;
    const size_t fs = frame_stride(c);
    if (prm.preconditioner == 1 && c->L.size() > 1) {
        std::vector<PairParam> items((size_t)P);
        for (int k = 0; k < P; ++k) items[k] = PairParam{prm.speed_alpha, prm.remodelling_alpha, k, k};
        return direct_solve_list(c, frames, items, v_x, v_y, remodelling, speed, stats);
    }
    std::vector<vof_pair_stats> local;
    if (!stats && prm.preconditioner == 2) { local.resize((size_t)P); stats = local.data(); }
    if (stride > 1 && P >= 2 * stride && (double)(P / stride) * (double)c->Ni * (double)c->Nj >= 16e6) {
        const int lanes = allow_lanes ? lanes_for(c, (P + stride - 1) / stride) : 1;
        if (int rc = solve_stack_two_phase(c, frames, P, v_x, v_y, remodelling, speed, stats, stride, lanes)) return rc;
    } else {
        auto plain = [&](vof_ctx* L, int a, int b) -> int {
            for (int k0 = a; k0 < b; k0 += batch_slots(L)) {
                int np = std::min(batch_slots(L), b - k0);
                int rc = solve_batch(L, frames + (size_t)k0 * fs, np, v_x + (size_t)k0 * fs, v_y + (size_t)k0 * fs,
                                     remodelling + (size_t)k0 * fs, speed ? speed + (size_t)k0 * fs : nullptr,
                                     stats ? stats + k0 : nullptr);
                if (rc) return rc;
            }
            return 0;
        };
        const int lanes = allow_lanes ? lanes_for(c, P) : 1;
        if (lanes <= 1) {
            if (int rc = plain(c, 0, P)) return rc;
        } else if (int rc = run_lanes(c, lanes, [&](vof_ctx* L, int i) { return plain(L, (int)((long)P * i / lanes), (int)((long)P * (i + 1) / lanes)); })) {
            return rc;
        }
    }
    if (prm.preconditioner == 2 && stats) {
        std::vector<PairParam> items;
        std::vector<int> which;
        for (int k = 0; k < P; ++k)
            if (!stats[k].converged && std::isfinite(stats[k].relative_residual)) {
                items.push_back(PairParam{prm.speed_alpha, prm.remodelling_alpha, k, k});
                which.push_back(k);
            }
        if (!items.empty() && direct_ok_for_fallback(c)) {
            std::vector<vof_pair_stats> st(items.size());
            if (int rc = direct_solve_list(c, frames, items, v_x, v_y, remodelling, speed, st.data())) {
                if (rc != -3) return rc;
                c->err.clear();
            } else {
                for (size_t i = 0; i < which.size(); ++i) {
                    st[i].iterations += stats[which[i]].iterations;
                    st[i].batch_ms += stats[which[i]].batch_ms / std::max(1, stats[which[i]].batch_pairs) * st[i].batch_pairs;
                    stats[which[i]] = st[i];
                }
            }
        }
    }
    return 0;
}

int vof_solve_stack_dev(vof_ctx* c, const double* movie, int n_frames, const vof_params* p, double* v_x, double* v_y,
                        double* remodelling, double* speed, vof_pair_stats* stats) {
    if (!c) return -1;
    if (!movie || !v_x || !v_y || !remodelling) { c->err = "NULL array pointer"; return -1; }
    if (n_frames < 2) { c->err = "need at least two frames"; return -1; }
    if (int rc = check_params(c, p)) return rc;
    HIPCHK(hipSetDevice(c->device));
    if (int rc = solve_range_dev(c, movie, n_frames - 1, v_x, v_y, remodelling, speed, stats, true)) return rc;
    HIPCHK(hipStreamSynchronize(c->stream));
    return 0;
}

static int ensure_staging(vof_ctx* c, bool double_buffer) {
    const size_t fs = frame_stride(c);
    if (!c->st_movie) {
        if (int rc = dev_alloc(c, &c->st_movie, (size_t)(c->B + 1) * fs)) return rc;
        for (int i = 0; i < 4; ++i)
            if (int rc = dev_alloc(c, &c->st_out[i], (size_t)c->B * fs)) return rc;
    }
    if (double_buffer && !c->st_out2[0]) {
        for (int i = 0; i < 4; ++i)
            if (int rc = dev_alloc(c, &c->st_out2[i], (size_t)c->B * fs)) return rc;
        if (int rc = dev_alloc(c, &c->st_movie2, (size_t)(c->B + 1) * fs)) return rc;
        HIPCHK(hipStreamCreateWithFlags(&c->copy_stream, hipStreamNonBlocking));
        for (int i = 0; i < 2; ++i) {
            HIPCHK(hipEventCreateWithFlags(&c->ev_solved[i], hipEventDisableTiming));
            HIPCHK(hipEventCreateWithFlags(&c->ev_copied[i], hipEventDisableTiming));
            HIPCHK(hipEventCreateWithFlags(&c->ev_uploaded[i], hipEventDisableTiming));
        }
    }
    return 0;
}

int vof_solve_stack_host(vof_ctx* c, const double* movie, int n_frames, const vof_params* p, double* v_x,
                         double* v_y, double* remodelling, double* speed, vof_pair_stats* stats) {
    if (!c) return -1;
    if (!movie || !v_x || !v_y || !remodelling) { c->err = "NULL array pointer"; return -1; }
    if (n_frames < 2) { c->err = "need at least two frames"; return -1; }
    if (int rc = check_params(c, p)) return rc;
    HIPCHK(hipSetDevice(c->device));
    const size_t fs = frame_stride(c);
    const int P = n_frames - 1;
    const bool multi = P > c->B;
    if (int rc = ensure_staging(c, multi)) return rc;
    struct Batch { int k0, np; };
    std::vector<Batch> batches;
    for (int k0 = 0; k0 < P;) {
        int np = std::min(c->B, P - k0);
        const int rest = P - k0;
        if (multi && rest <= c->B && rest > 48) np = rest - std::max(16, rest / 4);
        batches.push_back({k0, np});
        k0 += np;
    }
    const int nb = (int)batches.size();
    const char* mbase = (const char*)movie;
    const size_t movie_bytes = (size_t)n_frames * fs * sizeof(double);
    size_t split = movie_bytes;
    if (nb > 1) {
        size_t want = (size_t)(batches[0].np + 1) * fs * sizeof(double);
        size_t addr = ((size_t)(uintptr_t)mbase + want + 4095) & ~(size_t)4095;
        split = std::min(movie_bytes, addr - (size_t)(uintptr_t)mbase);
    }
    const bool htrace = getenv("VOF_TRACE_HOST") != nullptr;
    const auto ht0 = std::chrono::steady_clock::now();
    auto hmark = [&](const char* what) {
        if (htrace) fprintf(stderr, "[vof host] %8.1f ms  %s\n", std::chrono::duration<double, std::milli>(std::chrono::steady_clock::now() - ht0).count(), what);
    };
    const bool pinned_a = hipHostRegister((void*)mbase, split, hipHostRegisterDefault) == hipSuccess;
    if (!pinned_a) (void)hipGetLastError();
    hmark("first movie part pinned");
    bool pinned_b = false;
    double* outs[4] = {v_x, v_y, remodelling, speed};
    const size_t out_bytes = (size_t)P * fs * sizeof(double);
    std::vector<std::thread> helpers;
    std::thread movie_helper;
    if (split < movie_bytes)
        movie_helper = std::thread([&pinned_b, mbase, split, movie_bytes, dev = c->device]() {
            if (hipSetDevice(dev) == hipSuccess &&
                hipHostRegister((void*)(mbase + split), movie_bytes - split, hipHostRegisterDefault) == hipSuccess) pinned_b = true;
        });
    const bool pin_outputs = out_bytes >= ((size_t)1 << 20);
    std::vector<size_t> bound((size_t)nb + 1);
    struct Region { char* ptr; size_t bytes; bool pinned; };
    std::vector<Region> regions((size_t)nb * 4, Region{nullptr, 0, false});
    std::vector<std::atomic<int>> batch_ready((size_t)nb);
    for (auto& a : batch_ready) a.store(0);
    int n_outs = 0;
    for (int i = 0; i < 4; ++i) if (outs[i]) ++n_outs;
    for (int i = 0; i < 4; ++i) {
        if (!outs[i]) continue;
        const uintptr_t base = (uintptr_t)outs[i];
        for (int bi = 0; bi <= nb; ++bi) {
            size_t o = bi == nb ? out_bytes : (size_t)batches[bi].k0 * fs * sizeof(double);
            if (bi > 0 && bi < nb) o = std::min(out_bytes, (size_t)(((base + o + 4095) & ~(uintptr_t)4095) - base));
            bound[(size_t)bi] = o;
            if (bi > 0) regions[(size_t)(bi - 1) * 4 + i].bytes = o;
        }
        size_t prev = 0;
        for (int bi = 0; bi < nb; ++bi) {
            Region& r = regions[(size_t)bi * 4 + i];
            const size_t end = r.bytes;
            r.ptr = (char*)outs[i] + prev;
            r.bytes = end - prev;
            prev = end;
        }
    }
    std::atomic<int> next_task{0};
    const int n_tasks = nb * 4;
    auto helper_body = [&regions, &batch_ready, &next_task, n_tasks]() {
        for (;;) {
            const int t = next_task.fetch_add(1);
            if (t >= n_tasks) return;
            Region& r = regions[(size_t)t];
            if (r.ptr && r.bytes) {
                volatile char* q = (volatile char*)r.ptr;
                for (size_t o = 0; o < r.bytes; o += 4096) q[o] = 0;
                q[r.bytes - 1] = 0;
            }
            batch_ready[(size_t)(t / 4)].fetch_add(1);
        }
    };
    {
        const unsigned hw = std::max(1u, std::thread::hardware_concurrency());
        const int n_helpers = (int)std::min<unsigned>(std::min<unsigned>(8u, hw), (unsigned)n_tasks);
        for (int t = 0; t < n_helpers; ++t) helpers.emplace_back(helper_body);
    }
    int regions_pinned_upto = 0;
    auto wait_batch_regions = [&](int bi) {
        for (int b = 0; b <= bi; ++b)
            while (batch_ready[(size_t)b].load() < 4) std::this_thread::yield();
        for (; regions_pinned_upto <= bi; ++regions_pinned_upto)
            for (int i = 0; i < 4 && pin_outputs; ++i) {
                Region& r = regions[(size_t)regions_pinned_upto * 4 + i];
                if (!r.ptr || !r.bytes) continue;
                if (hipHostRegister((void*)r.ptr, r.bytes, hipHostRegisterDefault) == hipSuccess) r.pinned = true;
                else (void)hipGetLastError();
            }
    };
    auto join_helpers = [&]() { for (auto& t : helpers) if (t.joinable()) t.join(); };
    auto fail_msg = [&](const char* what, hipError_t e) { c->err = std::string(what) + ": " + hipGetErrorString(e); return -2; };
    int rc_all = 0;
    double* frames_buf[2] = {c->st_movie, multi ? c->st_movie2 : c->st_movie};
    auto upload = [&](int bi, hipStream_t st) {
        const Batch& bt = batches[bi];
        const size_t o0 = (size_t)bt.k0 * fs * sizeof(double), o1 = o0 + (size_t)(bt.np + 1) * fs * sizeof(double);
        char* dst = (char*)frames_buf[bi & 1];
        hipError_t e = hipSuccess;
        if (o0 < split) e = hipMemcpyAsync(dst, mbase + o0, std::min(o1, split) - o0, hipMemcpyHostToDevice, st);
        if (e == hipSuccess && o1 > split) {
            const size_t a = std::max(o0, split);
            e = hipMemcpyAsync(dst + (a - o0), mbase + a, o1 - a, hipMemcpyHostToDevice, st);
        }
        return e;
    };
    {
        hipError_t e = upload(0, c->stream);
        if (e != hipSuccess) rc_all = fail_msg("H2D copy failed", e);
    }
    for (int bi = 0; bi < nb && !rc_all; ++bi) {
        const Batch& bt = batches[bi];
        const int set = bi & 1;
        double** so = (multi && set) ? c->st_out2 : c->st_out;
        hipError_t e;
        if (bi + 1 < nb) {
            if (movie_helper.joinable()) movie_helper.join();
            if (bi >= 1 && (e = hipStreamWaitEvent(c->copy_stream, c->ev_solved[(bi + 1) & 1], 0)) != hipSuccess) { rc_all = fail_msg("stream wait failed", e); break; }
            if ((e = upload(bi + 1, c->copy_stream)) != hipSuccess ||
                (e = hipEventRecord(c->ev_uploaded[(bi + 1) & 1], c->copy_stream)) != hipSuccess) { rc_all = fail_msg("H2D copy failed", e); break; }
        }
        if (bi > 0 && (e = hipStreamWaitEvent(c->stream, c->ev_uploaded[set], 0)) != hipSuccess) { rc_all = fail_msg("stream wait failed", e); break; }
        if (multi && bi >= 2 && (e = hipStreamWaitEvent(c->stream, c->ev_copied[set], 0)) != hipSuccess) {
            rc_all = fail_msg("stream wait failed", e);
            break;
        }
        int rc = solve_range_dev(c, frames_buf[set], bt.np, so[0], so[1], so[2], so[3], stats ? stats + bt.k0 : nullptr, false);
        if (rc) { rc_all = rc; break; }
        hmark("batch solved");
        wait_batch_regions(bi);
        hmark("output regions of the batch ready");
        hipStream_t cs = multi ? c->copy_stream : c->stream;
        if (multi) {
            if ((e = hipEventRecord(c->ev_solved[set], c->stream)) != hipSuccess ||
                (e = hipStreamWaitEvent(cs, c->ev_solved[set], 0)) != hipSuccess) { rc_all = fail_msg("event record failed", e); break; }
        }
        for (int i = 0; i < 4 && !rc_all; ++i)
            if (outs[i]) {
                const size_t o0 = (size_t)bt.k0 * fs * sizeof(double), o1 = o0 + (size_t)bt.np * fs * sizeof(double);
                const size_t r0 = (size_t)(regions[(size_t)bi * 4 + i].ptr - (char*)outs[i]);
                const size_t cut = std::min(std::max(r0, o0), o1);
                if (cut > o0) {
                    e = hipMemcpyAsync((char*)outs[i] + o0, (const char*)so[i], cut - o0, hipMemcpyDeviceToHost, cs);
                    if (e != hipSuccess) { rc_all = fail_msg("D2H copy failed", e); break; }
                }
                if (o1 > cut) {
                    e = hipMemcpyAsync((char*)outs[i] + cut, (const char*)so[i] + (cut - o0), o1 - cut, hipMemcpyDeviceToHost, cs);
                    if (e != hipSuccess) rc_all = fail_msg("D2H copy failed", e);
                }
            }
        if (multi) {
            if (!rc_all && (e = hipEventRecord(c->ev_copied[set], cs)) != hipSuccess) rc_all = fail_msg("event record failed", e);
        } else if ((e = hipStreamSynchronize(c->stream)) != hipSuccess && !rc_all) rc_all = fail_msg("stream synchronize failed", e);
    }
    join_helpers();
    if (movie_helper.joinable()) movie_helper.join();
    hmark("all batches enqueued");
    if (multi && hipStreamSynchronize(c->copy_stream) != hipSuccess && !rc_all) { c->err = "copy stream synchronize failed"; rc_all = -2; }
    if (hipStreamSynchronize(c->stream) != hipSuccess && !rc_all) { c->err = "stream synchronize failed"; rc_all = -2; }
    hmark("copies done");
    for (auto& r : regions)
        if (r.pinned) (void)hipHostUnregister((void*)r.ptr);
    if (pinned_a) (void)hipHostUnregister((void*)mbase);
    if (pinned_b) (void)hipHostUnregister((void*)(mbase + split));
    hmark("unpinned");
    return rc_all;
}

int vof_blur_stack_dev(vof_ctx* c, const double* in, double* out, int n_frames, const double* weights, int radius) {
    if (!c) return -1;
    if (!in || !out || !weights) { c->err = "NULL pointer"; return -1; }
    if (n_frames < 1 || radius < 0 || radius > 4096) { c->err = "bad n_frames / radius"; return -1; }
    HIPCHK(hipSetDevice(c->device));
    size_t fs = frame_stride(c);
    const int chunk = std::min(n_frames, 16);
    if (!c->blur_tmp) {
        if (int rc = dev_alloc(c, &c->blur_tmp, (size_t)16 * fs)) return rc;
        if (int rc = dev_alloc(c, &c->blur_w, (size_t)2 * 4096 + 1)) return rc;
    }
    HIPCHK(hipMemcpyAsync(c->blur_w, weights, (size_t)(2 * radius + 1) * sizeof(double), hipMemcpyHostToDevice, c->stream));
    for (int f0 = 0; f0 < n_frames; f0 += chunk) {
        int nf = std::min(chunk, n_frames - f0);
        dim3 g = grid2d(c->Ni, c->Nj, nf);
        Prof p(c, VOF_K_RHS, 0);
        k_blur1d<0><<<g, blk2d, 0, c->stream>>>(in + (size_t)f0 * fs, c->blur_tmp, c->Ni, c->Nj, c->blur_w, radius);
        k_blur1d<1><<<g, blk2d, 0, c->stream>>>(c->blur_tmp, out + (size_t)f0 * fs, c->Ni, c->Nj, c->blur_w, radius);
    }
    HIPCHK(hipGetLastError());
    HIPCHK(hipStreamSynchronize(c->stream));
    return 0;
}

int vof_blur_stack_host(vof_ctx* c, const double* in, double* out, int n_frames, const double* weights, int radius) {
    if (!c) return -1;
    if (!in || !out || !weights) { c->err = "NULL pointer"; return -1; }
    HIPCHK(hipSetDevice(c->device));
    size_t fs = frame_stride(c);
    if (!c->blur_io) { if (int rc = dev_alloc(c, &c->blur_io, (size_t)2 * 16 * fs)) return rc; }
    for (int f0 = 0; f0 < n_frames; f0 += 16) {
        int nf = std::min(16, n_frames - f0);
        HIPCHK(hipMemcpyAsync(c->blur_io, in + (size_t)f0 * fs, (size_t)nf * fs * sizeof(double), hipMemcpyHostToDevice, c->stream));
        if (int rc = vof_blur_stack_dev(c, c->blur_io, c->blur_io + (size_t)16 * fs, nf, weights, radius)) return rc;
        HIPCHK(hipMemcpyAsync(out + (size_t)f0 * fs, c->blur_io + (size_t)16 * fs, (size_t)nf * fs * sizeof(double), hipMemcpyDeviceToHost, c->stream));
        HIPCHK(hipStreamSynchronize(c->stream));
    }
    return 0;
}

static int moments_pass(vof_ctx* c, const double* x, size_t n, double shift, double* out2) {
    const int nb = c->nblk;
    Prof p(c, VOF_K_REDUCE, 0, 8.0 * n);
    k_moments<<<nb, RBLK, 0, c->stream>>>(x, n, shift, c->partials);
    k_sum3<<<1, 64, 0, c->stream>>>(c->partials, nb, c->func3);
    HIPCHK(hipGetLastError());
    HIPCHK(hipMemcpyAsync(c->h_func3, c->func3, 3 * sizeof(double), hipMemcpyDeviceToHost, c->stream));
    HIPCHK(hipStreamSynchronize(c->stream));
    out2[0] = c->h_func3[0];
    out2[1] = c->h_func3[1];
    return 0;
}

struct Moments {
    double n = 0, mean = 0, m2 = 0;
    void merge(double nb, double meanb, double m2b) {
        if (nb == 0) return;
        double nt = n + nb, d = meanb - mean;
        m2 += m2b + d * d * n * nb / nt;
        mean += d * nb / nt;
        n = nt;
    }
};

static int chunk_moments(vof_ctx* c, const double* x, size_t n, Moments* acc) {
    double s[2];
    if (int rc = moments_pass(c, x, n, 0.0, s)) return rc;
    double mean = s[0] / (double)n;
    if (int rc = moments_pass(c, x, n, mean, s)) return rc;
    mean += s[0] / (double)n;
    acc->merge((double)n, mean, s[1] - s[0] * s[0] / (double)n);
    return 0;
}

int vof_field_moments_dev(vof_ctx* c, const double* field, size_t n, double* mean, double* variance) {
    if (!c) return -1;
    if (!field || n == 0) { c->err = "empty field"; return -1; }
    HIPCHK(hipSetDevice(c->device));
    Moments m;
    if (int rc = chunk_moments(c, field, n, &m)) return rc;
    if (mean) *mean = m.mean;
    if (variance) *variance = m.m2 / m.n;
    return 0;
}

int vof_subsample_dev(vof_ctx* c, const double* field, int n_fields, int box, int offset, double* out) {
    if (!c) return -1;
    if (!field || !out) { c->err = "NULL pointer"; return -1; }
    if (n_fields < 1 || box < 1 || offset < 0 || offset >= box) { c->err = "bad n_fields / box / offset"; return -1; }
    HIPCHK(hipSetDevice(c->device));
    int nbx = c->Ni / box, nby = c->Nj / box;
    if (nbx < 1 || nby < 1) return 0;
    k_subsample<<<grid2d(nbx, nby, n_fields), blk2d, 0, c->stream>>>(field, c->Ni, c->Nj, box, offset, nbx, nby, out);
    HIPCHK(hipGetLastError());
    HIPCHK(hipStreamSynchronize(c->stream));
    return 0;
}

static int solve_virtual_pairs(vof_ctx* c, const double* dmovie, const std::vector<PairParam>& hp, int np, double* const* outs,
                               vof_pair_stats* st) {
    if (c->prm.preconditioner == 1 && c->L.size() > 1) {
        std::vector<PairParam> items(hp.begin(), hp.begin() + np);
        return direct_solve_list(c, dmovie, items, outs[0], outs[1], outs[2], outs[3], st);
    }
    if (!c->pp_buf) { if (int rc = dev_alloc(c, &c->pp_buf, (size_t)c->B)) return rc; }
    HIPCHK(hipStreamSynchronize(c->stream));
    HIPCHK(hipMemcpyAsync(c->pp_buf, hp.data(), (size_t)np * sizeof(PairParam), hipMemcpyHostToDevice, c->stream));
    c->pp = c->pp_buf;
    int rc = solve_batch(c, dmovie, np, outs[0], outs[1], outs[2], outs[3], st);
    c->pp = nullptr;
    if (rc) return rc;
    if (c->prm.preconditioner == 2) {
        std::vector<PairParam> items;
        std::vector<int> which;
        for (int i = 0; i < np; ++i)
            if (!st[i].converged && std::isfinite(st[i].relative_residual)) { items.push_back(hp[i]); which.push_back(i); }
        if (!items.empty() && direct_ok_for_fallback(c)) {
            std::vector<vof_pair_stats> s2(items.size());
            int rc2 = direct_solve_list(c, dmovie, items, outs[0], outs[1], outs[2], outs[3], s2.data());
            if (rc2 == 0) {
                for (size_t i = 0; i < which.size(); ++i) { s2[i].iterations += st[which[i]].iterations; st[which[i]] = s2[i]; }
            } else if (rc2 != -3) {
                return rc2;
            } else {
                c->err.clear();
            }
        }
    }
    return 0;
}

int vof_vary_regularisation_host(vof_ctx* c, const double* movie, int n_frames, const vof_params* base,
                                 const double* speed_alphas, int n_sa, const double* remodelling_alphas, int n_ra,
                                 const double* blur_weights, int blur_radius, vof_variation_stats* out) {
    if (!c) return -1;
    if (!movie || !base || !out || !speed_alphas || !remodelling_alphas) { c->err = "NULL pointer"; return -1; }
    if (n_frames < 2) { c->err = "need at least two frames"; return -1; }
    if (n_sa < 0 || n_ra < 0) { c->err = "negative grid size"; return -1; }
    if (int rc = check_params(c, base)) return rc;
    HIPCHK(hipSetDevice(c->device));
    const size_t fs = frame_stride(c);
    const int P = n_frames - 1;
    if (int rc = ensure_staging(c, false)) return rc;
    double* dmovie = nullptr;
    HIPCHK(hipMalloc((void**)&dmovie, (size_t)n_frames * fs * sizeof(double)));
    auto fail = [&](int rc) { (void)hipFree(dmovie); return rc; };
    {
        const size_t movie_bytes = (size_t)n_frames * fs * sizeof(double);
        const bool pinned = hipHostRegister((void*)movie, movie_bytes, hipHostRegisterDefault) == hipSuccess;
        if (!pinned) (void)hipGetLastError();
        hipError_t e = hipMemcpyAsync(dmovie, movie, movie_bytes, hipMemcpyHostToDevice, c->stream);
        if (e == hipSuccess) e = hipStreamSynchronize(c->stream);
        if (pinned) (void)hipHostUnregister((void*)movie);
        if (e != hipSuccess) { c->err = std::string("H2D copy failed: ") + hipGetErrorString(e); return fail(-2); }
    }
    if (blur_weights)
        if (int rc = vof_blur_stack_dev(c, dmovie, dmovie, n_frames, blur_weights, blur_radius)) return fail(rc);
    auto summarise = [&](vof_variation_stats& o, const vof_pair_stats* st, const Moments& ms, const Moments& mr) {
        memset(&o, 0, sizeof o);
        o.speed_mean = ms.mean; o.speed_variance = ms.m2 / ms.n;
        o.remodelling_mean = mr.mean; o.remodelling_variance = mr.m2 / mr.n;
        o.converged_all = 1;
        for (int k = 0; k < P; ++k) {
            o.L1_functional += st[k].L1_functional;
            o.speed_functional += st[k].speed_functional;
            o.remodelling_functional += st[k].remodelling_functional;
            o.max_relative_residual = std::max(o.max_relative_residual, st[k].relative_residual);
            o.max_iterations_used = std::max(o.max_iterations_used, st[k].iterations);
            o.converged_all &= st[k].converged;
        }
        o.converged_last = st[P - 1].converged;
    };
    const int n_comb = n_sa * n_ra;
    for (int t = 0; t < n_comb; ++t) {
        vof_params q = *base;
        q.speed_alpha = speed_alphas[t / n_ra];
        q.remodelling_alpha = remodelling_alphas[t % n_ra];
        if (int rc = check_params(c, &q)) return fail(rc);
    }
    if (int rc = check_params(c, base)) return fail(rc);
    if (P <= c->B) {
        const int G = std::max(1, c->B / P);
        if (!c->pp_buf) { if (int rc = dev_alloc(c, &c->pp_buf, (size_t)c->B)) return fail(rc); }
        std::vector<PairParam> hp((size_t)G * P);
        std::vector<vof_pair_stats> st((size_t)G * P);
        for (int t0 = 0; t0 < n_comb; t0 += G) {
            const int g = std::min(G, n_comb - t0), np = g * P;
            for (int u = 0; u < g; ++u)
                for (int k = 0; k < P; ++k)
                    hp[(size_t)u * P + k] = PairParam{speed_alphas[(t0 + u) / n_ra], remodelling_alphas[(t0 + u) % n_ra], k, u * P + k};
            if (int rc = solve_virtual_pairs(c, dmovie, hp, np, c->st_out, st.data())) return fail(rc);
            for (int u = 0; u < g; ++u) {
                Moments ms, mr;
                if (int rc2 = chunk_moments(c, c->st_out[3] + (size_t)u * P * fs, (size_t)P * fs, &ms)) return fail(rc2);
                if (int rc2 = chunk_moments(c, c->st_out[2] + (size_t)u * P * fs, (size_t)P * fs, &mr)) return fail(rc2);
                summarise(out[t0 + u], st.data() + (size_t)u * P, ms, mr);
            }
        }
    } else {
        std::vector<vof_pair_stats> st((size_t)P);
        for (int t = 0; t < n_comb; ++t) {
            vof_params q = *base;
            q.speed_alpha = speed_alphas[t / n_ra];
            q.remodelling_alpha = remodelling_alphas[t % n_ra];
            if (int rc = check_params(c, &q)) return fail(rc);
            Moments ms, mr;
            std::vector<PairParam> hp2((size_t)c->B);
            for (int k0 = 0; k0 < P; k0 += c->B) {
                int np = std::min(c->B, P - k0);
                for (int i = 0; i < np; ++i) hp2[i] = PairParam{q.speed_alpha, q.remodelling_alpha, k0 + i, i};
                if (int rc = solve_virtual_pairs(c, dmovie, hp2, np, c->st_out, st.data() + k0)) return fail(rc);
                if (int rc = chunk_moments(c, c->st_out[3], (size_t)np * fs, &ms)) return fail(rc);
                if (int rc = chunk_moments(c, c->st_out[2], (size_t)np * fs, &mr)) return fail(rc);
            }
            summarise(out[t], st.data(), ms, mr);
        }
    }
    if (hipStreamSynchronize(c->stream) != hipSuccess) { c->err = "stream synchronize failed"; return fail(-2); }
    return fail(0);
}

int vof_texture_stack_dev(vof_ctx* c, double* out, int n_frames, const double* mode_params, int n_modes,
                          const double* frame_offsets, double period, double scale) {
    if (!c) return -1;
    if (!out || !mode_params || !frame_offsets) { c->err = "NULL pointer"; return -1; }
    if (n_frames < 1 || n_modes < 1 || n_modes > 4096 || !(period > 0.0)) { c->err = "bad n_frames / n_modes / period"; return -1; }
    HIPCHK(hipSetDevice(c->device));
    const int width = std::max(c->Ni, c->Nj);
    const int chunk = std::max(1, std::min(n_frames, (int)(((size_t)64 << 20) / ((size_t)4 * n_modes * width * sizeof(double)))));
    const size_t need = (size_t)chunk * 4 * n_modes * width + (size_t)4 * n_modes + (size_t)2 * chunk;
    if (c->tex_cap < need) {
        if (int rc = dev_alloc(c, &c->tex_tab, need)) return rc;
        c->tex_cap = need;
    }
    double* prm = c->tex_tab + (size_t)chunk * 4 * n_modes * width;
    double* offs = prm + (size_t)4 * n_modes;
    HIPCHK(hipMemcpyAsync(prm, mode_params, (size_t)4 * n_modes * sizeof(double), hipMemcpyHostToDevice, c->stream));
    for (int t0 = 0; t0 < n_frames; t0 += chunk) {
        const int nf = std::min(chunk, n_frames - t0);
        HIPCHK(hipMemcpyAsync(offs, frame_offsets + (size_t)2 * t0, (size_t)2 * nf * sizeof(double), hipMemcpyHostToDevice, c->stream));
        k_texture_tables<<<dim3((width + 255) / 256, n_modes, nf), 256, 0, c->stream>>>(c->tex_tab, width, c->Ni, c->Nj, n_modes, prm,
                                                                                       offs, period);
        k_texture_sum<<<dim3((c->Nj + BX - 1) / BX, (c->Ni + BY * TEX_ROWS - 1) / (BY * TEX_ROWS), nf), blk2d, 0, c->stream>>>(
            c->tex_tab, width, c->Ni, c->Nj, n_modes, scale, out + (size_t)t0 * frame_stride(c));
        HIPCHK(hipGetLastError());
        HIPCHK(hipStreamSynchronize(c->stream));
    }
    return 0;
}

int vof_bench_sweeps_dev(vof_ctx* c, const double* movie, int n_pairs, const vof_params* p, int n_sweeps) {
    if (!c) return -1;
    if (!movie) { c->err = "NULL movie"; return -1; }
    if (n_pairs < 1 || n_pairs > c->B) { c->err = "n_pairs must be in [1, max_pairs_in_flight]"; return -1; }
    if (c->L.size() < 2) { c->err = "grid too small for the sweep benchmark"; return -1; }
    if (int rc = check_params(c, p)) return rc;
    HIPCHK(hipSetDevice(c->device));
    c->frames = movie;
    c->npairs = n_pairs;
    c->cur_units = n_pairs;
    Level& f = c->L[0];
    {
        Prof pr(c, VOF_K_RHS, 0);
        k_rhs<<<grid2d(f.ni, f.nj, n_pairs), blk2d, 0, c->stream>>>(movie, frame_stride(c), c->Nj, f.ni, f.nj, c->kb, nullptr);
    }
    HIPCHK(hipMemsetAsync(c->kx, 0, (size_t)n_pairs * 3 * f.npts * sizeof(double), c->stream));
    if (c->vfloat) {
        size_t n = (size_t)n_pairs * 3 * f.npts;
        k_convert<double, float><<<1024, 256, 0, c->stream>>>(c->kb, (float*)c->b32, n);
        smooth_level_t<float>(c, 0, (float*)c->ky, (float*)f.x2, (const float*)c->b32, n_sweeps, true, false, n_pairs, nullptr);
    } else {
        smooth_level_t<double>(c, 0, c->kx, (double*)f.x2, c->kb, n_sweeps, true, false, n_pairs, nullptr);
    }
    HIPCHK(hipGetLastError());
    HIPCHK(hipStreamSynchronize(c->stream));
    return 0;
}

int vof_profile_enable(vof_ctx* c, int on) {
    if (!c) return -1;
    if (!on) prof_collect(c);
    c->prof = on != 0;
    return 0;
}

int vof_profile_filter(vof_ctx* c, int kid, int level) {
    if (!c) return -1;
    if (kid >= VOF_K_COUNT || level > 15) { c->err = "bad kernel id / level"; return -1; }
    c->prof_kid = kid;
    c->prof_level = level;
    return 0;
}

int vof_profile_get_units(vof_ctx* c, int kid, int level, int64_t* pair_launches) {
    if (!c) return -1;
    if (kid < 0 || kid >= VOF_K_COUNT || level > 15) { c->err = "bad kernel id / level"; return -1; }
    prof_collect(c);
    long long u = 0;
    for (int l = 0; l < 16; ++l)
        if (level < 0 || l == level) u += c->prof_units[kid][l];
    if (pair_launches) *pair_launches = u;
    return 0;
}

int vof_profile_get_bytes(vof_ctx* c, int kid, int level, double* algorithmic_bytes) {
    if (!c) return -1;
    if (kid < 0 || kid >= VOF_K_COUNT || level > 15) { c->err = "bad kernel id / level"; return -1; }
    prof_collect(c);
    double u = 0;
    for (int l = 0; l < 16; ++l)
        if (level < 0 || l == level) u += c->prof_bytes[kid][l];
    if (algorithmic_bytes) *algorithmic_bytes = u;
    return 0;
}

int vof_profile_get_moved(vof_ctx* c, int kid, int level, double* moved_bytes) {
    if (!c) return -1;
    if (kid < 0 || kid >= VOF_K_COUNT || level > 15) { c->err = "bad kernel id / level"; return -1; }
    prof_collect(c);
    double u = 0;
    for (int l = 0; l < 16; ++l)
        if (level < 0 || l == level) u += c->prof_moved[kid][l];
    if (moved_bytes) *moved_bytes = u;
    return 0;
}

int vof_profile_reset(vof_ctx* c) {
    if (!c) return -1;
    prof_collect(c);
    memset(c->prof_ms, 0, sizeof c->prof_ms);
    memset(c->prof_n, 0, sizeof c->prof_n);
    memset(c->prof_units, 0, sizeof c->prof_units);
    memset(c->prof_bytes, 0, sizeof c->prof_bytes);
    memset(c->prof_moved, 0, sizeof c->prof_moved);
    c->prof_dropped = 0;
    return 0;
}

int vof_profile_get(vof_ctx* c, int kid, int level, int64_t* launches, double* total_ms) {
    if (!c) return -1;
    if (kid < 0 || kid >= VOF_K_COUNT || level > 15) { c->err = "bad kernel id / level"; return -1; }
    prof_collect(c);
    long long n = 0; double ms = 0;
    for (int l = 0; l < 16; ++l)
        if (level < 0 || l == level) { n += c->prof_n[kid][l]; ms += c->prof_ms[kid][l]; }
    if (launches) *launches = n;
    if (total_ms) *total_ms = ms;
    return 0;
}

static int dbg_ready(vof_ctx* c) {
    if (!c) return -1;
    if (!c->frames || c->npairs < 1) { c->err = "call vof_debug_setup first"; return -1; }
    return 0;
}

int vof_debug_setup(vof_ctx* c, const double* movie_host, int n_pairs, const vof_params* p) {
    if (!c) return -1;
    if (!movie_host) { c->err = "NULL movie"; return -1; }
    if (n_pairs < 1 || n_pairs > c->B) { c->err = "n_pairs must be in [1, max_pairs_in_flight]"; return -1; }
    if (int rc = check_params(c, p)) return rc;
    HIPCHK(hipSetDevice(c->device));
    size_t fs = frame_stride(c);
    if (int rc = ensure_staging(c, false)) return rc;
    HIPCHK(hipMemcpyAsync(c->st_movie, movie_host, (size_t)(n_pairs + 1) * fs * sizeof(double), hipMemcpyHostToDevice,
                          c->stream));
    if (int rc = setup_batch(c, c->st_movie, n_pairs)) return rc;
    c->vcoarse32 = p->vcycle_precision == 3;
    HIPCHK(hipStreamSynchronize(c->stream));
    return 0;
}

int vof_debug_check_canaries(vof_ctx* c) {
    if (!c) return -1;
    if (!c->dbg_canary) return 0;
    HIPCHK(hipStreamSynchronize(c->stream));
    std::string rep;
    const int bad = dbg_check_canaries(c, &rep);
    if (bad != 0) { c->err = "VOF_DEBUG_CANARY: " + rep; return -5; }
    return 0;
}

int vof_debug_level_shape(vof_ctx* c, int level, int* n_i, int* n_j) {
    if (!c) return -1;
    if (level < 0 || level >= (int)c->L.size()) { c->err = "bad level"; return -1; }
    if (n_i) *n_i = c->L[level].ni;
    if (n_j) *n_j = c->L[level].nj;
    return 0;
}

#define DBG_LEVEL(level)                                                              \
    if (int rc_ = dbg_ready(c)) return rc_;                                           \
    if (level < 0 || level >= (int)c->L.size()) { c->err = "bad level"; return -1; } \
    Level& lv = c->L[level];                                                          \
    size_t nbytes = (size_t)c->npairs * 3 * lv.npts * sizeof(double);                 \
    (void)nbytes;

constexpr size_t BOUNCE_BYTES = (size_t)8 << 20;
static int d2h_bounced(vof_ctx* c, void* host, const void* dev, size_t bytes) {
    if (!c->h_bounce) HIPCHK(hipHostMalloc((void**)&c->h_bounce, BOUNCE_BYTES));
    for (size_t off = 0; off < bytes; off += BOUNCE_BYTES) {
        const size_t n = std::min(BOUNCE_BYTES, bytes - off);
        HIPCHK(hipMemcpyAsync(c->h_bounce, (const char*)dev + off, n, hipMemcpyDeviceToHost, c->stream));
        HIPCHK(hipStreamSynchronize(c->stream));
        memcpy((char*)host + off, c->h_bounce, n);
    }
    HIPCHK(hipGetLastError());
    return 0;
}

static int dbg_up(vof_ctx* c, void* dst_v, const double* host, size_t n) {
    if (c->vfloat) {
        HIPCHK(hipMemcpyAsync(c->krh, host, n * sizeof(double), hipMemcpyHostToDevice, c->stream));
        k_convert<double, float><<<256, 256, 0, c->stream>>>(c->krh, (float*)dst_v, n);
    } else {
        HIPCHK(hipMemcpyAsync(dst_v, host, n * sizeof(double), hipMemcpyHostToDevice, c->stream));
    }
    return 0;
}
static int dbg_down(vof_ctx* c, double* host, const void* src_v, size_t n) {
    if (c->vfloat || c->h32) {
        k_convert<float, double><<<256, 256, 0, c->stream>>>((const float*)src_v, c->krh, n);
        HIPCHK(hipMemcpyAsync(host, c->krh, n * sizeof(double), hipMemcpyDeviceToHost, c->stream));
    } else {
        HIPCHK(hipMemcpyAsync(host, src_v, n * sizeof(double), hipMemcpyDeviceToHost, c->stream));
    }
    HIPCHK(hipStreamSynchronize(c->stream));
    HIPCHK(hipGetLastError());
    return 0;
}

int vof_debug_rhs(vof_ctx* c, double* b_host) {
    DBG_LEVEL(0)
    k_rhs<<<grid2d(lv.ni, lv.nj, c->npairs), blk2d, 0, c->stream>>>(c->frames, frame_stride(c), c->Nj, lv.ni, lv.nj, c->kb, nullptr);
    HIPCHK(hipMemcpyAsync(b_host, c->kb, nbytes, hipMemcpyDeviceToHost, c->stream));
    HIPCHK(hipStreamSynchronize(c->stream));
    return 0;
}

int vof_debug_apply(vof_ctx* c, int level, const double* x_host, double* y_host) {
    DBG_LEVEL(level)
    size_t n = nbytes / sizeof(double);
    if (int rc = dbg_up(c, c->kp, x_host, n)) return rc;
    if (level == 0) {
        krylov_apply(c, c->kp, c->kv, c->npairs, nullptr);
        HIPCHK(hipMemcpyAsync(y_host, c->kv, nbytes, hipMemcpyDeviceToHost, c->stream));
        HIPCHK(hipStreamSynchronize(c->stream));
        HIPCHK(hipGetLastError());
        return 0;
    }
    VDISPATCH(c, apply_level_t<VT>(c, level, (const VT*)c->kp, (const VT*)nullptr, (VT*)c->kv, 0, c->npairs, nullptr));
    return dbg_down(c, y_host, c->kv, n);
}

int vof_debug_gs(vof_ctx* c, int level, double* x_host, const double* b_host, int colour) {
    DBG_LEVEL(level)
    if (colour < 0 || colour > 3) { c->err = "bad colour"; return -1; }
    if (c->vfloat) { c->err = "the per-colour reference smoother works on float64 vectors only"; return -1; }
    HIPCHK(hipMemcpyAsync(c->kp, x_host, nbytes, hipMemcpyHostToDevice, c->stream));
    HIPCHK(hipMemcpyAsync(c->kv, b_host, nbytes, hipMemcpyHostToDevice, c->stream));
    gs_colour(c, level, c->kp, c->kv, colour, c->npairs, nullptr);
    HIPCHK(hipMemcpyAsync(x_host, c->kp, nbytes, hipMemcpyDeviceToHost, c->stream));
    HIPCHK(hipStreamSynchronize(c->stream));
    HIPCHK(hipGetLastError());
    return 0;
}

int vof_debug_sweep(vof_ctx* c, int level, double* x_host, const double* b_host, int reverse, int from_zero) {
    DBG_LEVEL(level)
    if (level + 1 >= (int)c->L.size()) { c->err = "coarsest level has no smoother"; return -1; }
    size_t n = nbytes / sizeof(double);
    if (int rc = dbg_up(c, c->kp, x_host, n)) return rc;
    if (int rc = dbg_up(c, c->kv, b_host, n)) return rc;
    VDISPATCH(c, sweep_level_t<VT>(c, level, from_zero ? (const VT*)nullptr : (const VT*)c->kp, (VT*)c->kt,
                                   (const VT*)c->kv, reverse != 0, c->npairs, nullptr));
    return dbg_down(c, x_host, c->kt, n);
}

int vof_debug_smooth(vof_ctx* c, int level, double* x_host, const double* b_host, int nu, int reverse, int from_zero) {
    DBG_LEVEL(level)
    if (level + 1 >= (int)c->L.size()) { c->err = "coarsest level has no smoother"; return -1; }
    if (nu < 1) { c->err = "nu must be >= 1"; return -1; }
    size_t n = nbytes / sizeof(double);
    if (int rc = dbg_up(c, c->kp, x_host, n)) return rc;
    if (int rc = dbg_up(c, c->kv, b_host, n)) return rc;
    VDISPATCH(c, smooth_level_t<VT>(c, level, (VT*)c->kp, (VT*)c->kt, (const VT*)c->kv, nu, from_zero != 0, reverse != 0, c->npairs, nullptr));
    return dbg_down(c, x_host, c->kp, n);
}

int vof_set_fused_sweeps(vof_ctx* c, int on) {
    if (!c) return -1;
    c->fused = on != 0;
    if (!c->fused) c->vfloat = false;
    return 0;
}

int vof_debug_restrict(vof_ctx* c, int level, const double* fine_host, double* coarse_host) {
    DBG_LEVEL(level)
    if (level + 1 >= (int)c->L.size()) { c->err = "no coarser level"; return -1; }
    Level& k = c->L[level + 1];
    if (int rc = dbg_up(c, c->kp, fine_host, nbytes / sizeof(double))) return rc;
    VDISPATCH(c, restrict_level_t<VT>(c, level, (const VT*)c->kp, (VT*)c->kv, c->npairs, nullptr));
    return dbg_down(c, coarse_host, c->kv, (size_t)c->npairs * 3 * k.npts);
}

int vof_debug_resrestrict_u(vof_ctx* c, int level, const double* x_new_host, const double* x_old_host, double* coarse_host) {
    DBG_LEVEL(level)
    if (level < 1 || level + 1 >= (int)c->L.size() || !lv.C) { c->err = "a stored level with a coarser level is needed"; return -1; }
    Level& k = c->L[level + 1];
    if (int rc = dbg_up(c, c->kp, x_new_host, nbytes / sizeof(double))) return rc;
    if (x_old_host)
        if (int rc = dbg_up(c, c->kt, x_old_host, nbytes / sizeof(double))) return rc;
    VDISPATCH(c, resrestrict_u_t<VT>(c, level, (const VT*)c->kp, x_old_host ? (const VT*)c->kt : (const VT*)nullptr, (VT*)c->kv, c->npairs, nullptr));
    return dbg_down(c, coarse_host, c->kv, (size_t)c->npairs * 3 * k.npts);
}

int vof_debug_prolong_add(vof_ctx* c, int level, double* fine_host, const double* coarse_host) {
    DBG_LEVEL(level)
    if (level + 1 >= (int)c->L.size()) { c->err = "no coarser level"; return -1; }
    Level& k = c->L[level + 1];
    if (int rc = dbg_up(c, c->kp, fine_host, nbytes / sizeof(double))) return rc;
    if (int rc = dbg_up(c, c->kv, coarse_host, (size_t)c->npairs * 3 * k.npts)) return rc;
    VDISPATCH(c, prolong_add_level_t<VT>(c, level, (VT*)c->kp, (const VT*)c->kv, c->npairs, nullptr));
    return dbg_down(c, fine_host, c->kp, nbytes / sizeof(double));
}

int vof_debug_stencil(vof_ctx* c, int level, double* c_host) {
    DBG_LEVEL(level)
    if (!lv.C) { c->err = "level has no stored stencil"; return -1; }
    const CLay L(lv.ni, lv.nj);
    const int fmt = level > 0 ? c->cfmt : 0;
    const int planes = fmt == 3 ? 30 : (fmt == 2 ? 45 : 81);
    const size_t n = (size_t)c->npairs * planes * L.plane;
    auto unpack = [&](auto get) {
        for (int k = 0; k < c->npairs; ++k)
            for (int pl = 0; pl < 81; ++pl)
                for (int p = 0; p < lv.ni; ++p)
                    for (int q = 0; q < lv.nj; ++q)
                        c_host[((size_t)k * 81 + pl) * lv.npts + (size_t)p * lv.nj + q] = get((size_t)k * planes * L.plane, pl, L.idx(p, q));
    };
    if (fmt == 2) {
        std::vector<uint32_t> tw(n);
        if (int rc = d2h_bounced(c, tw.data(), lv.C, n * sizeof(uint32_t))) return rc;
        unpack([&](size_t base, int pl, size_t idx) -> double {
            const int d = pl / 9, e = pl % 9;
            uint32_t bits;
            if (d == 4) bits = tw[base + (size_t)(36 + e) * L.plane + idx];
            else {
                const int j = (d < 4 ? d : d - 1) * 9 + e;
                const uint32_t v = tw[base + (size_t)(j >> 1) * L.plane + idx];
                bits = (j & 1) ? (v & 0xFFFF0000u) : (v << 16);
            }
            float f;
            memcpy(&f, &bits, 4);
            return f;
        });
    } else if (fmt == 3) {
        std::vector<uint32_t> tw(n);
        if (int rc = d2h_bounced(c, tw.data(), lv.C, n * sizeof(uint32_t))) return rc;
        unpack([&](size_t base, int pl, size_t idx) -> double {
            const int d = pl / 9, e = pl % 9;
            if (d == 4) {
                float f;
                memcpy(&f, &tw[base + (size_t)(18 + e) * L.plane + idx], 4);
                return f;
            }
            const int j = (d < 4 ? d : d - 1) * 9 + e;
            const uint32_t v = (tw[base + (size_t)(j >> 2) * L.plane + idx] >> (8 * (j & 3))) & 0xFFu;
            const int ex = (int)((v >> 3) & 0xFu), m = (int)(v & 7u);
            const double mag = ex ? std::ldexp(1.0 + m / 8.0, ex - 7) : std::ldexp(m / 8.0, -6);
            const int eb = (int)((tw[base + (size_t)(27 + e / 3) * L.plane + idx] >> (8 * (e % 3))) & 0xFFu);
            return ((v & 0x80u) ? -mag : mag) * std::ldexp(1.0, eb - 127);
        });
    } else if (fmt == 1) {
        std::vector<float> tf(n);
        if (int rc = d2h_bounced(c, tf.data(), lv.C, n * sizeof(float))) return rc;
        unpack([&](size_t base, int pl, size_t idx) -> double { return tf[base + (size_t)pl * L.plane + idx]; });
    } else {
        std::vector<double> tmp(n);
        if (int rc = d2h_bounced(c, tmp.data(), lv.C, n * sizeof(double))) return rc;
        unpack([&](size_t base, int pl, size_t idx) -> double { return tmp[base + (size_t)pl * L.plane + idx]; });
    }
    return 0;
}

int vof_debug_vcycle(vof_ctx* c, const double* r_host, double* e_host) {
    DBG_LEVEL(0)
    size_t n = nbytes / sizeof(double);
    if (int rc = dbg_up(c, c->kp, r_host, n)) return rc;
    c->h32 = handoff32_ok(c);
    vcycle(c, &c->ky, c->kp, c->npairs, nullptr);
    const int rc = c->h32_bad ? -1 : dbg_down(c, e_host, c->ky, n);
    c->h32 = c->h32_bad = false;
    return rc;
}

int vof_debug_vcycle_apply(vof_ctx* c, const double* r_host, double* y_host, double* v_host, double* dots_host, int* fused) {
    DBG_LEVEL(0)
    size_t n = nbytes / sizeof(double);
    if (int rc = dbg_up(c, c->kp, r_host, n)) return rc;
    const int np = c->npairs;
    c->cur_units = np;
    HIPCHK(hipMemcpyAsync(c->krh, r_host, nbytes, hipMemcpyHostToDevice, c->stream));
    c->trail_req = S0Trail{c->kv, c->krh, 1, c->partials};
    c->trail_set = true; c->trail_done = false;
    c->h32 = handoff32_ok(c);
    vcycle(c, &c->ky, c->kp, np, nullptr);
    c->trail_set = false;
    if (c->h32_bad) { c->h32 = c->h32_bad = false; return -1; }
    int nb = c->trail_done ? c->trail_nblk : krylov_apply(c, c->ky, c->kv, np, nullptr, c->krh, 1);
    if (fused) *fused = c->trail_done ? 1 : 0;
    if (!nb) { c->h32 = false; c->err = "the operator kernel did not fuse the dot products"; return -1; }
    std::vector<double> part((size_t)np * 3 * nb);
    HIPCHK(hipMemcpyAsync(part.data(), c->partials, part.size() * sizeof(double), hipMemcpyDeviceToHost, c->stream));
    const int rcd = dbg_down(c, y_host, c->ky, n);
    c->h32 = false;
    if (rcd) return rcd;
    if (int rc = d2h_bounced(c, v_host, c->kv, nbytes)) return rc;
    for (int k = 0; k < np; ++k)
        for (int sl = 0; sl < 2; ++sl) {
            double a = 0;
            for (int i = 0; i < nb; ++i) a += part[((size_t)k * 3 + sl) * nb + i];
            dots_host[2 * k + sl] = a;
        }
    return 0;
}

int vof_debug_coarse_solve(vof_ctx* c, const double* r_host, double* e_host) {
    int last = c ? (int)c->L.size() - 1 : 0;
    DBG_LEVEL(last)
    size_t n = nbytes / sizeof(double);
    if (int rc = dbg_up(c, c->kp, r_host, n)) return rc;
    VDISPATCH(c, coarse_solve_t<VT>(c, (const VT*)c->kp, (VT*)c->kv, c->npairs, nullptr));
    return dbg_down(c, e_host, c->kv, n);
}

}
```

profiles/round_overlap.py:

```python
#!/usr/bin/env python3
import argparse
import csv
from collections import defaultdict


def rounds_of(kernels):
    out, cur = [], []
    for s, e, name in kernels:
        cur.append((s, e))
        if "k_update_xr" in name:
            out.append({"iv": cur, "upd": e - s})
            cur = []
    if cur:
        out.append({"iv": cur, "upd": None})
    for r in out:
        r["start"] = min(s for s, _ in r["iv"])
        r["end"] = max(e for _, e in r["iv"])
        r["sum"] = sum(e - s for s, e in r["iv"])
    return out


def merged(iv):
    out = []
    for s, e in sorted(iv):
        if out and s <= out[-1][1]:
            out[-1][1] = max(out[-1][1], e)
        else:
            out.append([s, e])
    return out


def overlap(s, e, cover):
    return sum(max(0, min(e, b) - max(s, a)) for a, b in cover)


def main():
    ap = argparse.ArgumentParser()
    ap.add_argument("trace")
    ap.add_argument("--steps", type=int, default=2)
    ap.add_argument("--straggler", type=float, default=0.10)
    ap.add_argument("--quiet", action="store_true", help="totals only, no per-round table")
    a = ap.parse_args()
    per_queue = defaultdict(list)
    with open(a.trace) as f:
        for r in csv.DictReader(f):
            name = r["Kernel_Name"]
            if "vof::" not in name or "k_texture" in name:
                continue
            per_queue[r.get("Queue_Id", "?")].append((int(r["Start_Timestamp"]), int(r["End_Timestamp"]), name))
    t0 = min(k[0] for ks in per_queue.values() for k in ks)
    rounds = {}
    for q, ks in per_queue.items():
        ks.sort()
        rs = rounds_of(ks)
        longest = max((r["upd"] for r in rs if r["upd"] is not None), default=1)
        for r in rs:
            r["share"] = None if r["upd"] is None else r["upd"] / longest
            r["straggler"] = r["share"] is not None and r["share"] < a.straggler
        rounds[q] = rs
    dense = {q: merged([(r["start"], r["end"]) for r in rs if r["share"] is not None and not r["straggler"]])
             for q, rs in rounds.items()}
    tot_span = tot_sum = tot_cov = 0
    n_str = 0
    if not a.quiet:
        print("| queue | round | start ms | wall span ms | summed kernel ms | launches | k_update_xr ms | share of the queue's longest | straggler | covered ms |")
        print("|---|---:|---:|---:|---:|---:|---:|---:|---|---:|")
    for q in sorted(rounds):
        cover = merged([iv for p, ivs in dense.items() if p != q for iv in ivs])
        for i, r in enumerate(rounds[q]):
            span = r["end"] - r["start"]
            cov = overlap(r["start"], r["end"], cover) if r["straggler"] else 0
            if r["straggler"]:
                tot_span += span; tot_sum += r["sum"]; tot_cov += cov; n_str += 1
            if not a.quiet:
                upd = "tail" if r["upd"] is None else f"{r['upd'] / 1e6:.3f}"
                share = "" if r["share"] is None else f"{100 * r['share']:.1f} %"
                tail = f"yes | {cov / 1e6:.2f}" if r["straggler"] else " | "
                print(f"| {q} | {i} | {(r['start'] - t0) / 1e6:.1f} | {span / 1e6:.2f} | {r['sum'] / 1e6:.2f} | {len(r['iv'])} | {upd} | {share} | {tail} |")
    k = a.steps
    all_iv = [(s, e) for ks in per_queue.values() for s, e, _ in ks]
    span_all = max(e for _, e in all_iv) - min(s for s, _ in all_iv)
    print(f"\n| per step ({k} steps in the trace) | |\n|---|---:|")
    print(f"| queues with solver kernels | {len(rounds)} |")
    print(f"| rounds | {sum(len(rs) for rs in rounds.values()) / k:.1f} |")
    print(f"| straggler rounds (k_update_xr below {100 * a.straggler:.0f} % of the queue's longest) | {n_str / k:.1f} |")
    print(f"| wall span of the straggler rounds, ms | {tot_span / 1e6 / k:.2f} |")
    print(f"| summed kernel time of the straggler rounds, ms | {tot_sum / 1e6 / k:.2f} |")
    print(f"| of the wall span: covered by a dense round of another queue, ms | {tot_cov / 1e6 / k:.2f} |")
    print(f"| of the wall span: not covered, ms | {(tot_span - tot_cov) / 1e6 / k:.2f} |")
    print(f"| first to last solver kernel, ms (all steps, with the gaps between them) | {span_all / 1e6:.1f} |")


if __name__ == "__main__":
    main()
```

Baseline: 1359 frame-pairs/s.

## Overlap second-phase batch setup with first-phase solver tail on a side stream

Splits solve_batch into a prelude (setup, RHS and norm) and the iterative rest. In the two-phase warm-start scheme, the second phase's prelude is queued on a side stream while the first phase's BiCG loop is still in its straggler tail, either early once fewer than 10% of pairs stay active or right after that loop. The aim is to hide the setup and Galerkin work of the rest batch behind the sparse tail iterations. It adds side streams and events, sizes lane slots so both phases fit in one batch, and is on by default unless profiling or VOF_TAIL_OVERLAP=0; the two phases now share buffers and depend on correct event ordering.

```diff
diff --git a/include/vof.h b/include/vof.h
--- a/include/vof.h
+++ b/include/vof.h
@@ -118,6 +118,7 @@
 int vof_profile_get_bytes(vof_ctx* ctx, int kernel_id, int level, double* algorithmic_bytes);
 int vof_profile_get_moved(vof_ctx* ctx, int kernel_id, int level, double* moved_bytes);
 const char* vof_kernel_name(int kernel_id);
+int vof_debug_tail_overlap(vof_ctx* ctx, int64_t* groups_overlapped, int64_t* queued_early);
 
 int vof_debug_setup(vof_ctx* ctx, const double* movie_host, int n_pairs, const vof_params* p);
 int vof_debug_check_canaries(vof_ctx* ctx);
diff --git a/opticalflow_amd/_native.py b/opticalflow_amd/_native.py
--- a/opticalflow_amd/_native.py
+++ b/opticalflow_amd/_native.py
@@ -76,6 +76,7 @@
     "vof_profile_get_bytes": (C.c_int, [_vp, C.c_int, C.c_int, C.POINTER(C.c_double)]),
     "vof_profile_get_moved": (C.c_int, [_vp, C.c_int, C.c_int, C.POINTER(C.c_double)]),
     "vof_kernel_name": (C.c_char_p, [C.c_int]),
+    "vof_debug_tail_overlap": (C.c_int, [_vp, C.POINTER(C.c_int64), C.POINTER(C.c_int64)]),
     "vof_debug_setup": (C.c_int, [_vp, _vp, C.c_int, C.POINTER(VofParams)]),
     "vof_debug_check_canaries": (C.c_int, [_vp]),
     "vof_debug_level_shape": (C.c_int, [_vp, C.c_int, C.POINTER(C.c_int), C.POINTER(C.c_int)]),
@@ -94,6 +95,8 @@
     "vof_debug_vcycle_apply": (C.c_int, [_vp, _vp, _vp, _vp, _vp, C.POINTER(C.c_int)]),
 }
 
+_NEWER_SYMBOLS = {"vof_debug_tail_overlap"}
+
 _lib = None
 
 
@@ -128,6 +131,8 @@
     _share_hip_runtime_with_torch()
     lib = C.CDLL(p)
     for name, (res, args) in SIGNATURES.items():
+        if name in _NEWER_SYMBOLS and path is None and os.environ.get("VOF_LIB") and not hasattr(lib, name):
+            continue
         fn = getattr(lib, name)
         fn.restype = res
         fn.argtypes = args
@@ -282,6 +287,11 @@
     def profile_enable(self, on=True):
         self._check(self.lib.vof_profile_enable(self.h, int(bool(on))), "profile_enable")
 
+    def tail_overlap(self):
+        n, early = C.c_int64(), C.c_int64()
+        self._check(self.lib.vof_debug_tail_overlap(self.h, C.byref(n), C.byref(early)), "debug_tail_overlap")
+        return n.value, early.value
+
     def profile_filter(self, kernel=-1, level=-1):
         kid = K_NAMES.index(kernel) if isinstance(kernel, str) else int(kernel)
         self._check(self.lib.vof_profile_filter(self.h, kid, level), "profile_filter")
diff --git a/opticalflow_amd/csrc/vof.hip b/opticalflow_amd/csrc/vof.hip
--- a/opticalflow_amd/csrc/vof.hip
+++ b/opticalflow_amd/csrc/vof.hip
@@ -16,6 +16,7 @@
 #include <cstdio>
 #include <cstdlib>
 #include <cstring>
+#include <functional>
 #include <mutex>
 #include <string>
 #include <thread>
@@ -177,6 +178,11 @@
     hipEvent_t lane_ev[MAX_LANES][2] = {};
     hipEvent_t ev_fork = nullptr;
     hipEvent_t group_ev[MAX_LANES * MAX_LANE_GROUPS] = {};
+    hipStream_t side_stream[MAX_LANES] = {};
+    hipEvent_t side_ev[MAX_LANES][4] = {};
+    std::function<int()> tail_hook;
+    bool tail_hook_early = false;
+    long long tail_preludes = 0, tail_early = 0;
 };
 
 static std::string g_create_error;
@@ -1358,14 +1364,28 @@
     return 0;
 }
 
-int solve_batch(vof_ctx* c, const double* frames_dev, int np, double* vx, double* vy, double* gm, double* speed,
-                vof_pair_stats* stats) {
+int fire_tail_hook(vof_ctx* c, bool early) {
+    const std::function<int()> hook = std::move(c->tail_hook);
+    c->tail_hook = nullptr;
+    c->tail_hook_early = early;
+    return hook();
+}
+
+struct MaxItGuard {
+    vof_params& p;
+    int saved;
+    explicit MaxItGuard(vof_ctx* c) : p(c->prm), saved(c->prm.max_iterations) {
+        constexpr int MG_ATTEMPT_CAP = 150;
+        if (p.preconditioner == 2 && !c->direct_on && c->L.size() > 1 && p.max_iterations > MG_ATTEMPT_CAP && 3 * c->L[0].nj <= 3100 &&
+            direct_ok_for_fallback(c))
+            p.max_iterations = MG_ATTEMPT_CAP;
+    }
+    ~MaxItGuard() { p.max_iterations = saved; }
+};
+
+int solve_batch_prelude(vof_ctx* c, const double* frames_dev, int np, bool stats) {
     const vof_params& P = c->prm;
-    struct MaxItGuard { vof_params& p; int saved; ~MaxItGuard() { p.max_iterations = saved; } } max_it_guard{c->prm, c->prm.max_iterations};
-    constexpr int MG_ATTEMPT_CAP = 150;
-    if (P.preconditioner == 2 && !c->direct_on && c->L.size() > 1 && P.max_iterations > MG_ATTEMPT_CAP && 3 * c->L[0].nj <= 3100 &&
-        direct_ok_for_fallback(c))
-        c->prm.max_iterations = MG_ATTEMPT_CAP;
+    MaxItGuard max_it_guard(c);
     if (stats) HIPCHK(hipEventRecord(c->ev_batch[0], c->stream));
     c->vfloat = (P.vcycle_precision == 1 || P.vcycle_precision == 2) && c->fused && c->L.size() > 1 && !c->direct_on;
     c->vcoarse32 = P.vcycle_precision == 3 && !c->direct_on;
@@ -1379,17 +1399,28 @@
         c->direct_pairs += np;
     } else if (int rc = setup_batch(c, frames_dev, np)) return rc;
     Level& f = c->L[0];
+    hipStream_t s = c->stream;
+    const bool zero_guess = !c->guess_src && (P.initial_v_x == 0.0 && P.initial_v_y == 0.0 && P.initial_remodelling == 0.0);
+    {
+        Prof p(c, VOF_K_RHS, 0);
+        k_rhs_norm<<<rgrid(c, np), RBLK, 0, s>>>(frames_dev, frame_stride(c), c->Nj, f.ni, f.nj, c->kb, zero_guess ? c->kr : nullptr,
+                                                c->partials, c->pp);
+    }
+    { Prof p(c, VOF_K_VECTOR, 0); k_scalar<S_BNORM><<<np, 64, 0, s>>>(c->sc, c->partials, c->nblk, c->active, P.rtol, P.max_iterations); }
+    HIPCHK(hipGetLastError());
+    return 0;
+}
+
+int solve_batch_rest(vof_ctx* c, const double* frames_dev, int np, double* vx, double* vy, double* gm, double* speed,
+                     vof_pair_stats* stats) {
+    const vof_params& P = c->prm;
+    MaxItGuard max_it_guard(c);
+    Level& f = c->L[0];
     const size_t len = 3 * f.npts;
     hipStream_t s = c->stream;
     double sx = P.delta_t / P.delta_x;
     const bool zero_guess = !c->guess_src && (P.initial_v_x == 0.0 && P.initial_v_y == 0.0 && P.initial_remodelling == 0.0);
     double* rh = c->krh;
-    {
-        Prof p(c, VOF_K_RHS, 0);
-        k_rhs_norm<<<rgrid(c, np), RBLK, 0, s>>>(frames_dev, frame_stride(c), c->Nj, f.ni, f.nj, c->kb, zero_guess ? c->kr : nullptr,
-                                                c->partials, c->pp);
-    }
-    { Prof p(c, VOF_K_VECTOR, 0); k_scalar<S_BNORM><<<np, 64, 0, s>>>(c->sc, c->partials, c->nblk, c->active, P.rtol, P.max_iterations); }
     int nb0 = c->nblk;
     if (zero_guess) {
         HIPCHK(hipMemsetAsync(c->kx, 0, (size_t)np * len * sizeof(double), s));
@@ -1422,6 +1453,8 @@
         int nact = 0;
         for (int k = 0; k < np; ++k) nact += c->h_active[k] != 0;
         if (nact == 0) break;
+        if (c->tail_hook && nact * 10 < np)
+            if (int rc = fire_tail_hook(c, true)) return rc;
         if (it_total == AUTO_F64_AFTER) { if (P.vcycle_precision == 2) c->vfloat = false; c->vcoarse32 = false; }
         c->cur_units = nact;
         c->h32 = handoff32_ok(c);
@@ -1484,6 +1517,8 @@
     return 0;
     };
     if (int rc = bicg_loop(bicg_limit)) return rc;
+    if (c->tail_hook)
+        if (int rc = fire_tail_hook(c, false)) return rc;
     auto independent_residual = [&](bool keep) -> int {
         c->cur_units = np;
         int nb3 = keep ? 0 : residual_d(c, c->kx, c->kb, nullptr, np, nullptr, 1);
@@ -1542,6 +1577,12 @@
         }
     }
     return 0;
+}
+
+int solve_batch(vof_ctx* c, const double* frames_dev, int np, double* vx, double* vy, double* gm, double* speed,
+                vof_pair_stats* stats) {
+    if (int rc = solve_batch_prelude(c, frames_dev, np, stats != nullptr)) return rc;
+    return solve_batch_rest(c, frames_dev, np, vx, vy, gm, speed, stats);
 }
 
 int check_params(vof_ctx* c, const vof_params* p) {
@@ -1682,6 +1723,10 @@
     for (int i = 0; i < MAX_LANES; ++i) {
         if (c->lane_stream[i]) hipStreamDestroy(c->lane_stream[i]);
         for (int j = 0; j < 2; ++j) if (c->lane_ev[i][j]) hipEventDestroy(c->lane_ev[i][j]);
+    }
+    for (int i = 0; i < MAX_LANES; ++i) {
+        if (c->side_stream[i]) hipStreamDestroy(c->side_stream[i]);
+        for (hipEvent_t e : c->side_ev[i]) if (e) hipEventDestroy(e);
     }
     if (c->ev_fork) hipEventDestroy(c->ev_fork);
     for (hipEvent_t e : c->group_ev) if (e) hipEventDestroy(e);
@@ -1897,63 +1942,79 @@
 
 inline int batch_slots(const vof_ctx* c) { return c->lane_parent ? c->lane_slots : c->B; }
 
-int make_lane(vof_ctx* c, int i, int n, vof_ctx* L) {
-    if (!c->lane_stream[i]) {
-        HIPCHK(hipStreamCreate(&c->lane_stream[i]));
-        for (int j = 0; j < 2; ++j) HIPCHK(hipEventCreate(&c->lane_ev[i][j]));
-    }
-    *L = *c;
-    const size_t lo = (size_t)c->B * i / n;
-    L->lane_parent = c;
-    L->lane_lo = (int)lo;
-    L->lane_slots = (int)((size_t)c->B * (i + 1) / n - lo);
-    for (int j = 0; j < MAX_LANES; ++j) { L->lane_stream[j] = nullptr; L->lane_ev[j][0] = L->lane_ev[j][1] = nullptr; }
-    L->ev_fork = nullptr;
-    L->stream = c->lane_stream[i];
-    L->own_stream = false;
-    L->ev_batch[0] = c->lane_ev[i][0];
-    L->ev_batch[1] = c->lane_ev[i][1];
-    L->allocs.clear();
-    L->recs.clear();
-    L->free_events.clear();
-    L->prof = false;
-    L->err.clear();
-    L->h_bounce = nullptr;
-    L->pp = nullptr;
-    L->guess_src = nullptr;
-    L->gmres_pairs = 0;
-    L->dir_ok = direct_ok_for_fallback(c) ? 1 : 0;
+void make_view(vof_ctx* src, int lo_slot, int slots, vof_ctx* V) {
+    *V = *src;
+    vof_ctx* c = src->lane_parent ? src->lane_parent : src;
+    const size_t lo = (size_t)lo_slot;
+    V->lane_parent = c;
+    V->lane_lo = (src->lane_parent ? src->lane_lo : 0) + lo_slot;
+    V->lane_slots = slots;
+    for (int j = 0; j < MAX_LANES; ++j) {
+        V->lane_stream[j] = nullptr; V->lane_ev[j][0] = V->lane_ev[j][1] = nullptr;
+        V->side_stream[j] = nullptr;
+        for (hipEvent_t& e : V->side_ev[j]) e = nullptr;
+    }
+    for (hipEvent_t& e : V->group_ev) e = nullptr;
+    V->ev_fork = nullptr;
+    V->own_stream = false;
+    V->allocs.clear();
+    V->recs.clear();
+    V->free_events.clear();
+    V->prof = false;
+    V->err.clear();
+    V->h_bounce = nullptr;
+    V->pp = nullptr;
+    V->guess_src = nullptr;
+    V->tail_hook = nullptr;
+    V->gmres_pairs = 0;
+    V->tail_preludes = V->tail_early = 0;
+    V->dir_ok = direct_ok_for_fallback(src) ? 1 : 0;
     const size_t len0 = 3 * c->L[0].npts;
-    for (double** v : {&L->kx, &L->kb, &L->kr, &L->krh, &L->kp, &L->kv, &L->kt, &L->ky, &L->kz, &L->b32, &L->gm_V})
+    for (double** v : {&V->kx, &V->kb, &V->kr, &V->krh, &V->kp, &V->kv, &V->kt, &V->ky, &V->kz, &V->b32, &V->gm_V})
         if (*v) *v += lo * len0;
     const int nl = (int)c->L.size();
     for (int l = 0; l < nl; ++l) {
-        Level& lv = L->L[l];
+        Level& lv = V->L[l];
         const size_t vb = 3 * lv.npts * sizeof(double);
         const size_t cb = (size_t)(nl == 1 ? 81 * 8 : c->c_bytes_per_point) * CLay(lv.ni, lv.nj).plane;
         for (void** q : {&lv.x, &lv.b, &lv.r, &lv.x2}) if (*q) *q = (char*)*q + lo * vb;
         if (lv.C) lv.C = (char*)lv.C + lo * cb;
     }
-    L->W += lo * c->nd * 2 * c->nd;
-    L->invT += lo * c->nd * c->nd;
-    L->partials += lo * c->part_per_pair;
-    L->sc += lo; L->h_sc += lo;
-    L->active += lo; L->h_active += lo;
-    L->func3 += 3 * lo; L->h_func3 += 3 * lo;
-    if (L->pp_buf) L->pp_buf += lo;
-    if (L->warm_src) L->warm_src += lo;
-    if (L->gm_cycle) L->gm_cycle += lo;
-    if (L->gm_state) L->gm_state += lo;
-    if (L->gm_partials) L->gm_partials += lo * (GM_NV + 1) * c->nblk;
+    V->W += lo * c->nd * 2 * c->nd;
+    V->invT += lo * c->nd * c->nd;
+    V->partials += lo * c->part_per_pair;
+    V->sc += lo; V->h_sc += lo;
+    V->active += lo; V->h_active += lo;
+    V->func3 += 3 * lo; V->h_func3 += 3 * lo;
+    if (V->pp_buf) V->pp_buf += lo;
+    if (V->warm_src) V->warm_src += lo;
+    if (V->gm_cycle) V->gm_cycle += lo;
+    if (V->gm_state) V->gm_state += lo;
+    if (V->gm_partials) V->gm_partials += lo * (GM_NV + 1) * c->nblk;
+}
+
+int make_lane(vof_ctx* c, int i, int lo, int slots, vof_ctx* L) {
+    if (!c->lane_stream[i]) {
+        HIPCHK(hipStreamCreate(&c->lane_stream[i]));
+        for (int j = 0; j < 2; ++j) HIPCHK(hipEventCreate(&c->lane_ev[i][j]));
+    }
+    make_view(c, lo, slots, L);
+    L->stream = c->lane_stream[i];
+    L->ev_batch[0] = c->lane_ev[i][0];
+    L->ev_batch[1] = c->lane_ev[i][1];
     return 0;
 }
 
 constexpr int LANES_NO_THREAD = -100;
 template <typename F>
-int run_lanes(vof_ctx* c, int n, F&& fn, bool concurrent_only = false) {
+int run_lanes(vof_ctx* c, int n, F&& fn, bool concurrent_only = false, const std::vector<int>* slots = nullptr) {
     std::vector<vof_ctx> lanes((size_t)n);
-    for (int i = 0; i < n; ++i)
-        if (int rc = make_lane(c, i, n, &lanes[i])) return rc;
+    for (int i = 0, at = 0; i < n; ++i) {
+        const int lo = slots ? at : (int)((size_t)c->B * i / n);
+        const int cnt = slots ? (*slots)[i] : (int)((size_t)c->B * (i + 1) / n) - lo;
+        if (int rc = make_lane(c, i, lo, cnt, &lanes[i])) return rc;
+        at += cnt;
+    }
     if (!c->ev_fork) HIPCHK(hipEventCreateWithFlags(&c->ev_fork, hipEventDisableTiming));
     HIPCHK(hipEventRecord(c->ev_fork, c->stream));
     for (int i = 0; i < n; ++i) HIPCHK(hipStreamWaitEvent(lanes[i].stream, c->ev_fork, 0));
@@ -1973,7 +2034,11 @@
         for (int i = n - 1 - (int)th.size(); i >= 0; --i) body(i);
     }
     for (auto& t : th) t.join();
-    for (int i = 0; i < n; ++i) c->gmres_pairs += lanes[i].gmres_pairs;
+    for (int i = 0; i < n; ++i) {
+        c->gmres_pairs += lanes[i].gmres_pairs;
+        c->tail_preludes += lanes[i].tail_preludes;
+        c->tail_early += lanes[i].tail_early;
+    }
     for (int i = 0; i < n; ++i)
         if (rc[i]) { c->err = "lane " + std::to_string(i) + ": " + lanes[i].err; return rc[i]; }
     return 0;
@@ -2023,8 +2088,82 @@
     return 0;
 }
 
+static bool tail_overlap_wanted(const vof_ctx* c) {
+    if (c->prof || c->dbg_sync) return false;
+    const char* e = getenv("VOF_TAIL_OVERLAP");
+    return !(e && e[0] == '0');
+}
+
+static int two_phase_group_overlapped(vof_ctx* c, int side, const double* movie, const std::vector<int>& first, int lo, int hi,
+                                      const std::vector<int>& rest, size_t ra, size_t rb, int stride, GroupSync& sync,
+                                      const std::function<int()>& between, double* v_x, double* v_y, double* remodelling,
+                                      double* speed, vof_pair_stats* stats) {
+    vof_ctx* root = c->lane_parent ? c->lane_parent : c;
+    const vof_params prm = c->prm;
+    const int n1 = hi - lo, n2 = (int)(rb - ra), n1_all = (int)sync.usable.size();
+    if (!root->side_stream[side]) {
+        HIPCHK(hipStreamCreate(&root->side_stream[side]));
+        for (int j = 0; j < 4; ++j) HIPCHK(hipEventCreateWithFlags(&root->side_ev[side][j], j < 2 ? hipEventDisableTiming : hipEventDefault));
+    }
+    const hipStream_t side_stream = root->side_stream[side];
+    hipEvent_t* const ev = root->side_ev[side];
+    vof_ctx sub;
+    make_view(c, n1, n2, &sub);
+    sub.stream = side_stream;
+    sub.ev_batch[0] = ev[2];
+    sub.ev_batch[1] = ev[3];
+    std::vector<PairParam> hp((size_t)n2);
+    std::vector<int> hsrc((size_t)n2);
+    for (int i = 0; i < n2; ++i) {
+        const int k = rest[ra + (size_t)i];
+        hp[i] = PairParam{prm.speed_alpha, prm.remodelling_alpha, k, k};
+    }
+    HIPCHK(hipEventRecord(ev[0], c->stream));
+    HIPCHK(hipStreamWaitEvent(side_stream, ev[0], 0));
+    bool queued = false;
+    const std::function<int()> queue_prelude = [&]() -> int {
+        queued = true;
+        HIPCHK(hipMemcpyAsync(sub.pp_buf, hp.data(), (size_t)n2 * sizeof(PairParam), hipMemcpyHostToDevice, side_stream));
+        sub.pp = sub.pp_buf;
+        sub.guess_src = sub.warm_src;
+        if (int rc = solve_batch_prelude(&sub, movie, n2, true)) { c->err = sub.err; return rc; }
+        HIPCHK(hipEventRecord(ev[1], side_stream));
+        return 0;
+    };
+    c->tail_hook = queue_prelude;
+    c->tail_hook_early = false;
+    int rc = two_phase_part(c, movie, first, (size_t)lo, (size_t)hi, false, stride, sync, v_x, v_y, remodelling, speed, stats);
+    c->tail_hook = nullptr;
+    const bool early = queued && c->tail_hook_early;
+    if (!rc) rc = between();
+    if (!rc && !queued) rc = queue_prelude();
+    if (rc) {
+        if (queued) hipStreamSynchronize(side_stream);
+        return rc;
+    }
+    {
+        std::lock_guard<std::mutex> lk(sync.m);
+        for (int i = 0; i < n2; ++i) {
+            const int src = std::min((rest[ra + (size_t)i] + stride / 2) / stride, n1_all - 1);
+            hsrc[i] = sync.usable[src] ? src : -1;
+        }
+    }
+    sub.stream = c->stream;
+    HIPCHK(hipMemcpyAsync(sub.warm_src, hsrc.data(), (size_t)n2 * sizeof(int), hipMemcpyHostToDevice, c->stream));
+    HIPCHK(hipStreamWaitEvent(c->stream, ev[1], 0));
+    std::vector<vof_pair_stats> st((size_t)n2);
+    rc = solve_batch_rest(&sub, movie, n2, v_x, v_y, remodelling, speed, st.data());
+    c->gmres_pairs += sub.gmres_pairs;
+    if (rc) { c->err = sub.err; return rc; }
+    c->tail_preludes += 1;
+    c->tail_early += early ? 1 : 0;
+    if (stats)
+        for (int i = 0; i < n2; ++i) stats[rest[ra + (size_t)i]] = st[i];
+    return 0;
+}
+
 static int two_phase_lane(vof_ctx* c, int lane, const std::vector<LaneGroup>& groups, hipEvent_t* ev, GroupSync& sync, const double* movie,
-                          const std::vector<int>& first, const std::vector<int>& rest, int stride, double* v_x, double* v_y,
+                          const std::vector<int>& first, const std::vector<int>& rest, int stride, bool overlap, double* v_x, double* v_y,
                           double* remodelling, double* speed, vof_pair_stats* stats) {
     const int ng = (int)groups.size();
     auto publish = [&](int g, bool ok) {
@@ -2038,7 +2177,9 @@
     };
     auto run_group = [&](int g) -> int {
         const LaneGroup& G = groups[g];
-        if (int rc = two_phase_part(c, movie, first, (size_t)G.lo, (size_t)G.hi, false, stride, sync, v_x, v_y, remodelling, speed, stats)) return rc;
+        const size_t ra = (size_t)(std::lower_bound(rest.begin(), rest.end(), G.lo * stride) - rest.begin());
+        const size_t rb = g + 1 < ng ? (size_t)(std::lower_bound(rest.begin(), rest.end(), G.hi * stride) - rest.begin()) : rest.size();
+        const std::function<int()> between = [&]() -> int {
         HIPCHK(hipEventRecord(ev[g], c->stream));
         publish(g, true);
         if (g + 1 < ng) {
@@ -2053,8 +2194,13 @@
             }
             if (state > 0) HIPCHK(hipStreamWaitEvent(c->stream, ev[g + 1], 0));
         }
-        const size_t ra = (size_t)(std::lower_bound(rest.begin(), rest.end(), G.lo * stride) - rest.begin());
-        const size_t rb = g + 1 < ng ? (size_t)(std::lower_bound(rest.begin(), rest.end(), G.hi * stride) - rest.begin()) : rest.size();
+        return 0;
+        };
+        if (overlap && G.hi > G.lo && rb > ra && (size_t)(G.hi - G.lo) + (rb - ra) <= (size_t)batch_slots(c))
+            return two_phase_group_overlapped(c, lane, movie, first, G.lo, G.hi, rest, ra, rb, stride, sync, between, v_x, v_y,
+                                              remodelling, speed, stats);
+        if (int rc = two_phase_part(c, movie, first, (size_t)G.lo, (size_t)G.hi, false, stride, sync, v_x, v_y, remodelling, speed, stats)) return rc;
+        if (int rc = between()) return rc;
         return two_phase_part(c, movie, rest, ra, rb, true, stride, sync, v_x, v_y, remodelling, speed, stats);
     };
     int rc = 0;
@@ -2066,7 +2212,7 @@
 }
 
 static int solve_stack_two_phase(vof_ctx* c, const double* movie, int P, double* v_x, double* v_y, double* remodelling,
-                                 double* speed, vof_pair_stats* stats, int stride, int lanes) {
+                                 double* speed, vof_pair_stats* stats, int stride, int lanes, bool allow_overlap) {
     const size_t len = 3 * c->L[0].npts;
     const int B = c->B;
     std::vector<int> first, rest;
@@ -2083,16 +2229,24 @@
     GroupSync sync;
     sync.usable.assign((size_t)n1, 0);
     int rc = LANES_NO_THREAD;
+    const bool overlap_wanted = allow_overlap && tail_overlap_wanted(c);
     if (lanes > 1) {
         const std::vector<LaneGroup> groups = plan_groups(c, n1, lanes, lane_groups_wanted());
         sync.state.assign(groups.size(), 0);
         for (size_t g = 0; g < groups.size(); ++g)
             if (!c->group_ev[g]) HIPCHK(hipEventCreateWithFlags(&c->group_ev[g], hipEventDisableTiming));
+        const bool overlap = overlap_wanted && (int)groups.size() == lanes && P <= B;
+        std::vector<int> slots;
+        if (overlap)
+            for (int g = 0; g < lanes; ++g) slots.push_back((g + 1 < lanes ? groups[g + 1].lo * stride : P) - groups[g].lo * stride);
         rc = run_lanes(c, lanes, [&](vof_ctx* L, int i) {
-            return two_phase_lane(L, i, groups, c->group_ev, sync, movie, first, rest, stride, v_x, v_y, remodelling, speed, stats);
-        }, true);
-    }
-    if (rc == LANES_NO_THREAD) {
+            return two_phase_lane(L, i, groups, c->group_ev, sync, movie, first, rest, stride, overlap, v_x, v_y, remodelling, speed, stats);
+        }, true, overlap ? &slots : nullptr);
+    }
+    if (rc == LANES_NO_THREAD && overlap_wanted && !rest.empty() && P <= B) {
+        rc = two_phase_group_overlapped(c, 0, movie, first, 0, n1, rest, 0, rest.size(), stride, sync, [] { return 0; }, v_x, v_y,
+                                        remodelling, speed, stats);
+    } else if (rc == LANES_NO_THREAD) {
         for (int phase = 0; phase < 2; ++phase) {
             const std::vector<int>& list = phase ? rest : first;
             if ((rc = two_phase_part(c, movie, list, 0, list.size(), phase == 1, stride, sync, v_x, v_y, remodelling, speed, stats))) return rc;
@@ -2141,7 +2295,7 @@
     if (!stats && prm.preconditioner == 2) { local.resize((size_t)P); stats = local.data(); }
     if (stride > 1 && P >= 2 * stride && (double)(P / stride) * (double)c->Ni * (double)c->Nj >= 16e6) {
         const int lanes = allow_lanes ? lanes_for(c, (P + stride - 1) / stride) : 1;
-        if (int rc = solve_stack_two_phase(c, frames, P, v_x, v_y, remodelling, speed, stats, stride, lanes)) return rc;
+        if (int rc = solve_stack_two_phase(c, frames, P, v_x, v_y, remodelling, speed, stats, stride, lanes, allow_lanes)) return rc;
     } else {
         auto plain = [&](vof_ctx* L, int a, int b) -> int {
             for (int k0 = a; k0 < b; k0 += batch_slots(L)) {
@@ -2748,6 +2902,13 @@
         if (level < 0 || l == level) { n += c->prof_n[kid][l]; ms += c->prof_ms[kid][l]; }
     if (launches) *launches = n;
     if (total_ms) *total_ms = ms;
+    return 0;
+}
+
+int vof_debug_tail_overlap(vof_ctx* c, int64_t* groups_overlapped, int64_t* queued_early) {
+    if (!c) return -1;
+    if (groups_overlapped) *groups_overlapped = c->tail_preludes;
+    if (queued_early) *queued_early = c->tail_early;
     return 0;
 }
 
diff --git a/profiles/round_overlap.py b/profiles/round_overlap.py
--- a/profiles/round_overlap.py
+++ b/profiles/round_overlap.py
@@ -34,6 +34,9 @@
     return sum(max(0, min(e, b) - max(s, a)) for a, b in cover)
 
 
+SETUP = ("k_galerkin", "k_coarse_build", "k_coarse_invert", "k_rhs_norm")
+
+
 def main():
     ap = argparse.ArgumentParser()
     ap.add_argument("trace")
@@ -60,22 +63,28 @@
         rounds[q] = rs
     dense = {q: merged([(r["start"], r["end"]) for r in rs if r["share"] is not None and not r["straggler"]])
              for q, rs in rounds.items()}
+    setup = {q: [(s, e) for s, e, name in ks if any(k in name for k in SETUP)] for q, ks in per_queue.items()}
+    tot_beside = tot_inside = 0
     tot_span = tot_sum = tot_cov = 0
     n_str = 0
     if not a.quiet:
-        print("| queue | round | start ms | wall span ms | summed kernel ms | launches | k_update_xr ms | share of the queue's longest | straggler | covered ms |")
-        print("|---|---:|---:|---:|---:|---:|---:|---:|---|---:|")
+        print("| queue | round | start ms | wall span ms | summed kernel ms | launches | k_update_xr ms | share of the queue's longest | straggler | covered ms | set-up beside ms | set-up inside ms |")
+        print("|---|---:|---:|---:|---:|---:|---:|---:|---|---:|---:|---:|")
     for q in sorted(rounds):
         cover = merged([iv for p, ivs in dense.items() if p != q for iv in ivs])
         for i, r in enumerate(rounds[q]):
             span = r["end"] - r["start"]
             cov = overlap(r["start"], r["end"], cover) if r["straggler"] else 0
+            beside = inside = 0
             if r["straggler"]:
+                beside = overlap(r["start"], r["end"], merged([iv for p, ivs in setup.items() if p != q for iv in ivs]))
+                inside = overlap(r["start"], r["end"], setup[q])
+                tot_beside += beside; tot_inside += inside
                 tot_span += span; tot_sum += r["sum"]; tot_cov += cov; n_str += 1
             if not a.quiet:
                 upd = "tail" if r["upd"] is None else f"{r['upd'] / 1e6:.3f}"
                 share = "" if r["share"] is None else f"{100 * r['share']:.1f} %"
-                tail = f"yes | {cov / 1e6:.2f}" if r["straggler"] else " | "
+                tail = f"yes | {cov / 1e6:.2f} | {beside / 1e6:.2f} | {inside / 1e6:.2f}" if r["straggler"] else " | | | "
                 print(f"| {q} | {i} | {(r['start'] - t0) / 1e6:.1f} | {span / 1e6:.2f} | {r['sum'] / 1e6:.2f} | {len(r['iv'])} | {upd} | {share} | {tail} |")
     k = a.steps
     all_iv = [(s, e) for ks in per_queue.values() for s, e, _ in ks]
@@ -88,6 +97,8 @@
     print(f"| summed kernel time of the straggler rounds, ms | {tot_sum / 1e6 / k:.2f} |")
     print(f"| of the wall span: covered by a dense round of another queue, ms | {tot_cov / 1e6 / k:.2f} |")
     print(f"| of the wall span: not covered, ms | {(tot_span - tot_cov) / 1e6 / k:.2f} |")
+    print(f"| of the wall span: a set-up kernel runs on another queue, ms | {tot_beside / 1e6 / k:.2f} |")
+    print(f"| set-up kernels on the straggler round's own queue inside its span, ms | {tot_inside / 1e6 / k:.2f} |")
     print(f"| first to last solver kernel, ms (all steps, with the gaps between them) | {span_all / 1e6:.1f} |")
 
 
```

New measurement: 1355 frame-pairs/s (median of 2 runs). No clear change (-0.3%).
